# clovaai/assembled-cnn

Measured on AMD Instinct MI355X. Metric: images/sec Assemble-ResNet-50 224^2 bf16 train, higher is better.
Workload: dtype bf16; 1 GPU; Assemble-ResNet-50 (BigLittle + SK + anti_alias sconv k=3 + resnet_d) bf16 train; per_gpu_batch=256, global_batch=256, image=224x224x3, num_classes=1001, parallelism=dp1

## Files before the change

### assembled_cnn_amd/build.py

```python
from __future__ import annotations

import concurrent.futures
import os
import shutil
import subprocess
import sys

HERE = os.path.dirname(os.path.abspath(__file__))
CSRC = os.path.join(HERE, 'csrc')
OBJ_DIR = os.path.join(CSRC, '_obj')
LIB_PATH = os.path.join(HERE, 'libasm_hip.so')
SOURCES = ['conv_igemm.hip', 'conv_igemm8.hip', 'conv_gemm1.hip', 'conv_dgrad_s2.hip', 'conv_wgrad.hip', 'bn.hip', 'pool.hip', 'sk_se.hip', 'sk_fused.hip', 'dense_small.hip', 'misc.hip', 'extra.hip', 'input.hip', 'autoaugment.hip', 'jpeg.hip', 'plan.hip', 'tape.hip', 'collective.hip', 'retrieval.hip']
HEADERS = [os.path.join(CSRC, 'common.h'), os.path.join(CSRC, 'igemm_common.h'), os.path.join(CSRC, 'jpeg_entropy.h'), os.path.join(CSRC, 'jpeg_parallel.h'), os.path.join(HERE, '..', 'include', 'asm_hip.h'),
           os.path.join(HERE, '..', 'include', 'asm_hip_debug.h')]
ARCH = 'gfx950'
CFLAGS = ['--offload-arch=' + ARCH, '-O3', '-std=c++17', '-fPIC', '-fno-gpu-rdc', '-Wall', '-Wno-unused-function']


def _hipcc() -> str:
  exe = shutil.which('hipcc') or '/opt/rocm/bin/hipcc'
  if not os.path.exists(exe):
    raise RuntimeError('hipcc not found: cannot build libasm_hip.so')
  return exe


def _stale(target: str, deps) -> bool:
  if not os.path.exists(target):
    return True
  t = os.path.getmtime(target)
  return any(os.path.getmtime(d) > t for d in deps)


def _compile(src: str) -> str:
  obj = os.path.join(OBJ_DIR, os.path.splitext(src)[0] + '.o')
  path = os.path.join(CSRC, src)
  if _stale(obj, [path] + HEADERS):
    cmd = [_hipcc()] + CFLAGS + ['-c', path, '-o', obj]
    r = subprocess.run(cmd, capture_output=True, text=True)
    if r.returncode != 0:
      raise RuntimeError('hipcc failed for %s:\n%s\n%s' % (src, r.stdout, r.stderr))
  return obj


def build(force: bool = False, verbose: bool = False) -> str:
  os.makedirs(OBJ_DIR, exist_ok=True)
  if force:
    for f in os.listdir(OBJ_DIR):
      os.remove(os.path.join(OBJ_DIR, f))
  with concurrent.futures.ThreadPoolExecutor(max_workers=min(8, len(SOURCES))) as ex:
    objs = list(ex.map(_compile, SOURCES))
  if force or _stale(LIB_PATH, objs):
    tmp = LIB_PATH + '.tmp.%d' % os.getpid()
    cmd = [_hipcc(), '--offload-arch=' + ARCH, '-shared', '-fPIC', '-o', tmp] + objs
    r = subprocess.run(cmd, capture_output=True, text=True)
    if r.returncode != 0:
      if os.path.exists(tmp):
        os.remove(tmp)
      raise RuntimeError('link failed:\n%s\n%s' % (r.stdout, r.stderr))
    os.replace(tmp, LIB_PATH)
  if verbose:
    print('built', LIB_PATH)
  return LIB_PATH


if __name__ == '__main__':
  build(force='--force' in sys.argv, verbose=True)
```

### assembled_cnn_amd/csrc/bn.hip

```cpp
#include "common.h"
#include <stdlib.h>


#define BN_LD_RED(p) (*(p))
#define BN_ST_BWD(v, p) __builtin_nontemporal_store(v, p)
#define BN_ST_FWD(v, p) __builtin_nontemporal_store(v, p)

namespace {

struct RowTiling {
  int vcols;
  int vcb;
  int rpb;
  int rows_per_block;
  int blocks;
  int slices;
  int vc_slice;
};

RowTiling make_tiling(int M, int C) {
  RowTiling t;
  t.vcols = C / 8;
  const int want = 8;
  int sl = t.vcols / 8;
// ... 312 lines not shown
      const unsigned m = fd_div((unsigned)i, fd_vcols);
      body(i, m, (int)((unsigned)i - m * (unsigned)vcols), k);
    }
  } else {
    for (size_t i = i0; i < nvec; i += stride) {
      const unsigned m = fd_div((unsigned)i, fd_vcols);
      const int vc = (int)((unsigned)i - m * (unsigned)vcols);
      load_coef(vc);
      body(i, m, vc, k);
    }
  }
}

template <int RES, bool RELU>
__global__ __launch_bounds__(256) void bn_apply_kernel(size_t nvec, int C, FastDiv fd_vcols,
                                                       const bf16_t* __restrict__ x, bf16_t* __restrict__ y,
                                                       const float* __restrict__ scale,
                                                       const float* __restrict__ shift,
                                                       const bf16_t* __restrict__ res, FastDiv fd_w, FastDiv fd_h,
                                                       int H, int W, uint8_t* __restrict__ mask) {
  const float* const coef[2] = {scale, shift};
  for_each_vec<2>(nvec, C, fd_vcols, coef, [&](size_t i, unsigned m, int vc, const float (&k)[2][8]) {
    float f[8];
    unpack8(__builtin_nontemporal_load(reinterpret_cast<const u32x4*>(x + i * 8)), f);
#pragma unroll
    for (int e = 0; e < 8; ++e) f[e] = f[e] * k[0][e] + k[1][e];
    if (RES != 0) {
      size_t ri;
      if (RES == 1) {
        ri = i * 8;
      } else {
        const unsigned nh = fd_div(m, fd_w);
        const unsigned w = m - nh * (unsigned)W;
        const unsigned n = fd_div(nh, fd_h);
        const unsigned h = nh - n * (unsigned)H;
        ri = ((((size_t)n * (H >> 1) + (h >> 1)) * (W >> 1) + (w >> 1)) * (C >> 3) + vc) * 8;
      }
      float r[8];
      unpack8(*reinterpret_cast<const u32x4*>(res + ri), r);
#pragma unroll
      for (int e = 0; e < 8; ++e) f[e] += r[e];
    }
    if (RELU) {
      if (mask) mask[i] = (uint8_t)relu_mask8(f);
#pragma unroll
      for (int e = 0; e < 8; ++e) f[e] = fmaxf(f[e], 0.f);
    }
    BN_ST_FWD(pack8(f), reinterpret_cast<u32x4*>(y + i * 8));
  });
}

__device__ __forceinline__ float bwd_dx(float A, float dz, float B, float x, float C) {
  return __builtin_fmaf(A, dz, B * x) + C;
}

template <int RELU, bool WRITE_DZ>
__global__ __launch_bounds__(256) void bn_bwd_apply_kernel(size_t nvec, int C, FastDiv fd_vcols,
                                                           const bf16_t* __restrict__ dy, const bf16_t* __restrict__ x,
                                                           const bf16_t* __restrict__ yout, const float* __restrict__ cA,
                                                           const float* __restrict__ cB,
                                                           const float* __restrict__ cC, bf16_t* __restrict__ dx,
                                                           bf16_t* __restrict__ dz) {
  const float* const coef[3] = {cA, cB, cC};
  for_each_vec<3>(nvec, C, fd_vcols, coef, [&](size_t i, unsigned, int, const float (&k)[3][8]) {
    float g[8], fx[8];
    unpack8(__builtin_nontemporal_load(reinterpret_cast<const u32x4*>(dy + i * 8)), g);
    unpack8(__builtin_nontemporal_load(reinterpret_cast<const u32x4*>(x + i * 8)), fx);
    if (RELU == 1) {
      float fy[8];
      unpack8(*reinterpret_cast<const u32x4*>(yout + i * 8), fy);
#pragma unroll
      for (int e = 0; e < 8; ++e) g[e] = fy[e] > 0.f ? g[e] : 0.f;
    } else if (RELU == 2) {
      mask8(g, reinterpret_cast<const uint8_t*>(yout)[i]);
    }
    if (WRITE_DZ) *reinterpret_cast<u32x4*>(dz + i * 8) = pack8(g);
    float o[8];
#pragma unroll
    for (int e = 0; e < 8; ++e) o[e] = bwd_dx(k[0][e], g[e], k[1][e], fx[e], k[2][e]);
    BN_ST_BWD(pack8(o), reinterpret_cast<u32x4*>(dx + i * 8));
  });
}

struct BwdRow2 {
  const bf16_t* __restrict__ dy;
  const bf16_t* __restrict__ xa;
  const bf16_t* __restrict__ xb;
  const uint8_t* __restrict__ mask;
  const float* __restrict__ mean_a;
  const float* __restrict__ invstd_a;
  const float* __restrict__ mean_b;
  const float* __restrict__ invstd_b;
  float* __restrict__ pa;
  float* __restrict__ pb;
  int C;
  float ma[8], ia[8], mb[8], ib[8];
  struct Loaded { u32x4 vg, va, vb; unsigned mk; };
  __device__ __forceinline__ void setup(int vc) {
#pragma unroll
    for (int e = 0; e < 8; ++e) {
      ma[e] = mean_a[vc * 8 + e];
      ia[e] = invstd_a[vc * 8 + e];
      mb[e] = mean_b[vc * 8 + e];
      ib[e] = invstd_b[vc * 8 + e];
    }
  }
  __device__ __forceinline__ void load(Loaded& ld, size_t off, size_t mi) const {
    ld.vg = BN_LD_RED(reinterpret_cast<const u32x4*>(dy + off));
    ld.va = BN_LD_RED(reinterpret_cast<const u32x4*>(xa + off));
    ld.vb = BN_LD_RED(reinterpret_cast<const u32x4*>(xb + off));
    ld.mk = mask[mi];
  }
  __device__ __forceinline__ void accum(const Loaded& ld, float (&acc)[3][8]) const {
    float g[8], fa[8], fb[8];
    unpack8(ld.vg, g);
    unpack8(ld.va, fa);
    unpack8(ld.vb, fb);
    mask8(g, ld.mk);
#pragma unroll
    for (int e = 0; e < 8; ++e) {
      acc[0][e] += g[e];
      acc[1][e] += g[e] * ((fa[e] - ma[e]) * ia[e]);
      acc[2][e] += g[e] * ((fb[e] - mb[e]) * ib[e]);
    }
  }
  __device__ __forceinline__ void store(int rblk, int which, int ch, float v) const {
    if (which == 0) {
      pa[((size_t)rblk * 2 + 0) * C + ch] = v;
      pb[((size_t)rblk * 2 + 0) * C + ch] = v;
    } else if (which == 1) {
      pa[((size_t)rblk * 2 + 1) * C + ch] = v;
    } else {
      pb[((size_t)rblk * 2 + 1) * C + ch] = v;
    }
  }
};

__global__ __launch_bounds__(256) void bn_bwd_reduce2_kernel(const bf16_t* __restrict__ dy, const bf16_t* __restrict__ xa,
                                                             const bf16_t* __restrict__ xb, const uint8_t* __restrict__ mask,
                                                             int M, int C, const float* __restrict__ mean_a,
                                                             const float* __restrict__ invstd_a, const float* __restrict__ mean_b,
                                                             const float* __restrict__ invstd_b, RowTiling t,
                                                             float* __restrict__ pa, float* __restrict__ pb) {
  row_reduce<3>(BwdRow2{dy, xa, xb, mask, mean_a, invstd_a, mean_b, invstd_b, pa, pb, C}, M, C, t);
}

__global__ __launch_bounds__(256) void bn_bwd_apply2_kernel(size_t nvec, int C, FastDiv fd_vcols,
                                                            const bf16_t* __restrict__ dy, const bf16_t* __restrict__ xa,
                                                            const bf16_t* __restrict__ xb, const uint8_t* __restrict__ mask,
                                                            const float* __restrict__ co, bf16_t* __restrict__ dxa,
                                                            bf16_t* __restrict__ dxb) {
  const float* const coef[6] = {co, co + (size_t)C, co + (size_t)2 * C, co + (size_t)3 * C, co + (size_t)4 * C, co + (size_t)5 * C};
  for_each_vec<6>(nvec, C, fd_vcols, coef, [&](size_t i, unsigned, int, const float (&k)[6][8]) {
    float g[8], fa[8], fb[8];
    unpack8(__builtin_nontemporal_load(reinterpret_cast<const u32x4*>(dy + i * 8)), g);
    unpack8(__builtin_nontemporal_load(reinterpret_cast<const u32x4*>(xa + i * 8)), fa);
    unpack8(__builtin_nontemporal_load(reinterpret_cast<const u32x4*>(xb + i * 8)), fb);
    mask8(g, mask[i]);
    float oa[8], ob[8];
#pragma unroll
    for (int e = 0; e < 8; ++e) {
      oa[e] = bwd_dx(k[0][e], g[e], k[1][e], fa[e], k[2][e]);
      ob[e] = bwd_dx(k[3][e], g[e], k[4][e], fb[e], k[5][e]);
    }
    BN_ST_BWD(pack8(oa), reinterpret_cast<u32x4*>(dxa + i * 8));
    BN_ST_BWD(pack8(ob), reinterpret_cast<u32x4*>(dxb + i * 8));
// ... 267 lines not shown
  ASM_LAUNCH(bn_finalize_kernel, dim3(cdiv(C, 16)), dim3(16 * FL), 0, (hipStream_t)stream, stats_partial,
                     blocks, M, C, gamma, beta, eps, momentum, moving_mean, moving_var, mean, invstd, scale, shift);
  ASM_CHECK_LAUNCH("bn_finalize");
  return ASM_OK;
}

extern "C" int asm_bn_infer_coeffs(int C, const float* gamma, const float* beta, const float* moving_mean,
                                   const float* moving_var, float eps, float* scale, float* shift, void* stream) {
  ASM_REQUIRE(C > 0 && gamma && beta && moving_mean && moving_var && scale && shift, "bn_infer_coeffs: bad arguments");
  ASM_LAUNCH(bn_infer_coeffs_kernel, dim3(cdiv(C, 256)), dim3(256), 0, (hipStream_t)stream, C, gamma, beta,
                     moving_mean, moving_var, eps, scale, shift);
  ASM_CHECK_LAUNCH("bn_infer_coeffs");
  return ASM_OK;
}

extern "C" int asm_bn_apply(const void* x, void* y, int M, int C, const float* scale, const float* shift,
                            const void* residual, int res_mode, int relu, int H, int W, uint8_t* relu_mask_out,
                            void* stream) {
  ASM_REQUIRE(x && y && scale && shift && M > 0 && C > 0 && C % 8 == 0, "bn_apply: bad arguments");
  ASM_REQUIRE(res_mode >= 0 && res_mode <= 2 && (res_mode == 0 || residual), "bn_apply: bad residual mode");
  ASM_REQUIRE((size_t)M * (C / 8) < 0x7fffffffull, "bn_apply: tensor too large");
  if (res_mode == 2)
    ASM_REQUIRE(H > 0 && W > 0 && H % 2 == 0 && W % 2 == 0 && M % (H * W) == 0, "bn_apply: bad upsample geometry");
  const FastDiv fw = make_fastdiv((unsigned)(W > 0 ? W : 1)), fh = make_fastdiv((unsigned)(H > 0 ? H : 1));
  static constexpr decltype(&bn_apply_kernel<0, false>) kernels[3][2] = {
      {bn_apply_kernel<0, false>, bn_apply_kernel<0, true>},
      {bn_apply_kernel<1, false>, bn_apply_kernel<1, true>},
      {bn_apply_kernel<2, false>, bn_apply_kernel<2, true>}};
  launch_vecs(kernels[res_mode][relu != 0], stream, M, C, (const bf16_t*)x, (bf16_t*)y, scale, shift, (const bf16_t*)residual,
              fw, fh, H, W, relu_mask_out);
  ASM_CHECK_LAUNCH("bn_apply");
  return ASM_OK;
}

extern "C" int asm_bn_bwd_reduce(const void* dy, const void* x, const void* yout, int relu, int M, int C,
                                 const float* mean, const float* invstd, float* partial, void* stream) {
  ASM_REQUIRE(dy && x && mean && invstd && partial && M > 0 && C > 0 && C % 8 == 0, "bn_bwd_reduce: bad arguments");
  ASM_REQUIRE(relu >= 0 && relu <= 2 && (!relu || yout), "bn_bwd_reduce: relu mask needs the forward output / bitmask");
  RowTiling t = make_tiling(M, C);
  ASM_LAUNCH(bn_bwd_reduce_kernel, dim3(t.blocks * t.slices), dim3(256), 0, (hipStream_t)stream, (const bf16_t*)dy,
                     (const bf16_t*)x, (const bf16_t*)yout, relu, M, C, mean, invstd, t, partial);
  ASM_CHECK_LAUNCH("bn_bwd_reduce");
  return ASM_OK;
}

extern "C" int asm_bn_bwd_finalize(const float* partial, int blocks, int M, int C, const float* gamma,
                                   const float* mean, const float* invstd, float* dgamma, float* dbeta,
                                   float* coefA, float* coefB, float* coefC, void* stream) {
  ASM_REQUIRE(partial && gamma && mean && invstd && dgamma && dbeta && coefA && coefB && coefC && blocks > 0,
              "bn_bwd_finalize: bad arguments");
  ASM_LAUNCH(bn_bwd_finalize_kernel, dim3(cdiv(C, 16)), dim3(16 * FL), 0, (hipStream_t)stream, partial, blocks,
                     M, C, gamma, mean, invstd, dgamma, dbeta, coefA, coefB, coefC, 0);
  ASM_CHECK_LAUNCH("bn_bwd_finalize");
  return ASM_OK;
}

extern "C" int asm_bn_bwd_finalize_raw(const float* partial, int blocks, int M, int C, const float* gamma,
                                       const float* mean, const float* invstd, float* dgamma, float* dbeta,
                                       float* coefA, float* coefB, float* coefC, void* stream) {
  ASM_REQUIRE(partial && gamma && mean && invstd && dgamma && dbeta && coefA && coefB && coefC && blocks > 0,
              "bn_bwd_finalize_raw: bad arguments");
  ASM_LAUNCH(bn_bwd_finalize_kernel, dim3(cdiv(C, 16)), dim3(16 * FL), 0, (hipStream_t)stream, partial, blocks,
                     M, C, gamma, mean, invstd, dgamma, dbeta, coefA, coefB, coefC, 1);
  ASM_CHECK_LAUNCH("bn_bwd_finalize_raw");
  return ASM_OK;
}

extern "C" int asm_bn_bwd_apply(const void* dy, const void* x, const void* yout, int relu, int M, int C,
                                const float* coefA, const float* coefB, const float* coefC, void* dx,
                                void* dz_out, void* stream) {
  ASM_REQUIRE(dy && x && dx && coefA && coefB && coefC && M > 0 && C > 0 && C % 8 == 0, "bn_bwd_apply: bad arguments");
  ASM_REQUIRE(relu >= 0 && relu <= 2 && (!relu || yout), "bn_bwd_apply: relu mask needs the forward output / bitmask");
  ASM_REQUIRE((size_t)M * (C / 8) < 0x7fffffffull, "bn_bwd_apply: tensor too large");
  static constexpr decltype(&bn_bwd_apply_kernel<0, false>) kernels[3][2] = {
      {bn_bwd_apply_kernel<0, false>, bn_bwd_apply_kernel<0, true>},
      {bn_bwd_apply_kernel<1, false>, bn_bwd_apply_kernel<1, true>},
      {bn_bwd_apply_kernel<2, false>, bn_bwd_apply_kernel<2, true>}};
  launch_vecs(kernels[relu][dz_out != nullptr], stream, M, C, (const bf16_t*)dy, (const bf16_t*)x, (const bf16_t*)yout, coefA,
              coefB, coefC, (bf16_t*)dx, (bf16_t*)dz_out);
  ASM_CHECK_LAUNCH("bn_bwd_apply");
  return ASM_OK;
}

extern "C" int asm_bn_small_max_rows(void) { return SMALL_BN_MAX_ROWS; }

extern "C" int asm_bn_small_fwd(const void* x, void* y, int M, int C, const float* gamma, const float* beta, float eps,
                                float momentum, float* moving_mean, float* moving_var, float* mean, float* invstd,
                                int relu, uint8_t* relu_mask_out, void* stream) {
  ASM_REQUIRE(x && y && gamma && beta && mean && invstd && M > 0 && M <= SMALL_BN_MAX_ROWS && C > 0 && C % 8 == 0,
              "bn_small_fwd: bad arguments (M=%d C=%d)", M, C);
  ASM_REQUIRE((moving_mean == nullptr) == (moving_var == nullptr), "bn_small_fwd: moving stats must both be given");
  const dim3 grid(cdiv(C, 64)), block(256);
  if (relu)
    ASM_LAUNCH(bn_small_fwd_kernel<true>, grid, block, 0, (hipStream_t)stream, (const bf16_t*)x, (bf16_t*)y, M, C,
                       gamma, beta, eps, momentum, moving_mean, moving_var, mean, invstd, relu_mask_out);
  else
    ASM_LAUNCH(bn_small_fwd_kernel<false>, grid, block, 0, (hipStream_t)stream, (const bf16_t*)x, (bf16_t*)y, M, C,
                       gamma, beta, eps, momentum, moving_mean, moving_var, mean, invstd, nullptr);
  ASM_CHECK_LAUNCH("bn_small_fwd");
  return ASM_OK;
}

extern "C" int asm_bn_small_bwd(const void* dy, const void* x, const uint8_t* relu_mask, int M, int C,
                                const float* gamma, const float* mean, const float* invstd, float* dgamma,
                                float* dbeta, void* dx, void* stream) {
  ASM_REQUIRE(dy && x && gamma && mean && invstd && dgamma && dbeta && dx && M > 0 && M <= SMALL_BN_MAX_ROWS && C > 0 &&
                  C % 8 == 0, "bn_small_bwd: bad arguments (M=%d C=%d)", M, C);
  const dim3 grid(cdiv(C, 64)), block(256);
  if (relu_mask)
    ASM_LAUNCH(bn_small_bwd_kernel<2>, grid, block, 0, (hipStream_t)stream, (const bf16_t*)dy, (const bf16_t*)x,
                       relu_mask, M, C, gamma, mean, invstd, dgamma, dbeta, (bf16_t*)dx);
  else
    ASM_LAUNCH(bn_small_bwd_kernel<0>, grid, block, 0, (hipStream_t)stream, (const bf16_t*)dy, (const bf16_t*)x,
                       nullptr, M, C, gamma, mean, invstd, dgamma, dbeta, (bf16_t*)dx);
  ASM_CHECK_LAUNCH("bn_small_bwd");
  return ASM_OK;
}

extern "C" int asm_bn_bwd_reduce2(const void* dy, const void* xa, const void* xb, const uint8_t* relu_mask, int M, int C,
                                  const float* mean_a, const float* invstd_a, const float* mean_b, const float* invstd_b,
                                  float* partial_a, float* partial_b, void* stream) {
  ASM_REQUIRE(dy && xa && xb && relu_mask && mean_a && invstd_a && mean_b && invstd_b && partial_a && partial_b && M > 0 &&
                  C > 0 && C % 8 == 0, "bn_bwd_reduce2: bad arguments");
  RowTiling t = make_tiling(M, C);
  ASM_LAUNCH(bn_bwd_reduce2_kernel, dim3(t.blocks * t.slices), dim3(256), 0, (hipStream_t)stream, (const bf16_t*)dy,
                     (const bf16_t*)xa, (const bf16_t*)xb, relu_mask, M, C, mean_a, invstd_a, mean_b, invstd_b, t, partial_a,
                     partial_b);
  ASM_CHECK_LAUNCH("bn_bwd_reduce2");
  return ASM_OK;
}

extern "C" int asm_bn_bwd_apply2(const void* dy, const void* xa, const void* xb, const uint8_t* relu_mask, int M, int C,
                                 const float* coef6, void* dxa, void* dxb, void* stream) {
  ASM_REQUIRE(dy && xa && xb && relu_mask && coef6 && dxa && dxb && M > 0 && C > 0 && C % 8 == 0, "bn_bwd_apply2: bad arguments");
  ASM_REQUIRE((size_t)M * (C / 8) < 0x7fffffffull, "bn_bwd_apply2: tensor too large");
  launch_vecs(bn_bwd_apply2_kernel, stream, M, C, (const bf16_t*)dy, (const bf16_t*)xa, (const bf16_t*)xb, relu_mask, coef6,
              (bf16_t*)dxa, (bf16_t*)dxb);
  ASM_CHECK_LAUNCH("bn_bwd_apply2");
  return ASM_OK;
}

extern "C" int asm_bn_apply2(const void* xa, const void* xb, void* y, int M, int C, const float* scale_a,
                             const float* shift_a, const float* scale_b, const float* shift_b, int relu,
                             uint8_t* relu_mask_out, void* stream) {
  ASM_REQUIRE(xa && xb && y && scale_a && shift_a && scale_b && shift_b && M > 0 && C > 0 && C % 8 == 0, "bn_apply2: bad arguments");
  ASM_REQUIRE((size_t)M * (C / 8) < 0x7fffffffull, "bn_apply2: tensor too large");
  launch_vecs(relu ? bn_apply2_kernel<true> : bn_apply2_kernel<false>, stream, M, C, (const bf16_t*)xa, (const bf16_t*)xb,
              (bf16_t*)y, scale_a, shift_a, scale_b, shift_b, relu ? relu_mask_out : nullptr);
  ASM_CHECK_LAUNCH("bn_apply2");
  return ASM_OK;
}
```

### assembled_cnn_amd/csrc/pool.hip

```cpp
#include "common.h"

namespace {

inline unsigned grid_for(size_t nvec) {
  size_t b = cdivz(nvec, 256);
  return (unsigned)(b ? b : 1);
}

__device__ __forceinline__ u32x4 ldv(const bf16_t* p, size_t elem_off) {
  return *reinterpret_cast<const u32x4*>(p + elem_off);
}

struct Pix {
  int n, h, w, vc;
};
__device__ __forceinline__ Pix decode(size_t i64, int H, int W, int vcols) {
  const unsigned i = (unsigned)i64;
  Pix p;
  unsigned m = i / (unsigned)vcols;
  p.vc = (int)(i - m * (unsigned)vcols);
  unsigned q = m / (unsigned)W;
  p.w = (int)(m - q * (unsigned)W);
  const unsigned n = q / (unsigned)H;
  p.h = (int)(q - n * (unsigned)H);
  p.n = (int)n;
  return p;
}

__global__ __launch_bounds__(256) void maxpool_fwd_kernel(const bf16_t* __restrict__ x, bf16_t* __restrict__ y,
                                                          uint8_t* __restrict__ amax, int N, int H, int W, int C,
                                                          int Ho, int Wo, int pad_h, int pad_w) {
  const int vcols = C >> 3;
  const size_t nvec = (size_t)N * Ho * Wo * vcols;
  const size_t i = (size_t)blockIdx.x * 256 + threadIdx.x;
  if (i >= nvec) return;
  const Pix p = decode(i, Ho, Wo, vcols);
  float best[8];
  int bidx[8];
#pragma unroll
  for (int e = 0; e < 8; ++e) {
    best[e] = -INFINITY;
    bidx[e] = 0;
  }
  for (int r = 0; r < 3; ++r) {
    const int ih = p.h * 2 + r - pad_h;
    if ((unsigned)ih >= (unsigned)H) continue;
    for (int s = 0; s < 3; ++s) {
      const int iw = p.w * 2 + s - pad_w;
      if ((unsigned)iw >= (unsigned)W) continue;
      float f[8];
      unpack8(ldv(x, (((size_t)p.n * H + ih) * W + iw) * C + p.vc * 8), f);
#pragma unroll
      for (int e = 0; e < 8; ++e)
        if (f[e] > best[e]) {
          best[e] = f[e];
          bidx[e] = r * 3 + s;
        }
    }
  }
  *reinterpret_cast<u32x4*>(y + i * 8) = pack8(best);
  if (amax) {
    unsigned lo = 0, hi = 0;
#pragma unroll
    for (int e = 0; e < 4; ++e) {
      lo |= (unsigned)bidx[e] << (8 * e);
      hi |= (unsigned)bidx[e + 4] << (8 * e);
    }
    u32x2 v = {lo, hi};
    *reinterpret_cast<u32x2*>(amax + i * 8) = v;
  }
}

__global__ __launch_bounds__(256) void maxpool_bwd_kernel(const bf16_t* __restrict__ dy,
                                                          const uint8_t* __restrict__ amax, bf16_t* __restrict__ dx,
                                                          int N, int H, int W, int C, int Ho, int Wo, int pad_h,
                                                          int pad_w) {
  const int vcols = C >> 3;
  const size_t nvec = (size_t)N * H * W * vcols;
  const size_t i = (size_t)blockIdx.x * 256 + threadIdx.x;
  if (i >= nvec) return;
  const Pix p = decode(i, H, W, vcols);
  float acc[8];
#pragma unroll
// ... 48 lines not shown
      ++cnt;
    }
  }
  const float inv = 1.0f / (float)(count_valid ? cnt : k * k);
#pragma unroll
  for (int e = 0; e < 8; ++e) acc[e] *= inv;
  *reinterpret_cast<u32x4*>(y + i * 8) = pack8(acc);
}

__device__ __forceinline__ int valid_taps(int o, int stride, int pad, int k, int L) {
  int c = 0;
  for (int r = 0; r < k; ++r) c += ((unsigned)(o * stride + r - pad) < (unsigned)L);
  return c;
}

__global__ __launch_bounds__(256) void avgpool_bwd_kernel(const bf16_t* __restrict__ dy, bf16_t* dx,
                                                          int N, int H, int W, int C, int k, int stride, int pad,
                                                          int Ho, int Wo, int count_valid, const bf16_t* addend) {
  const int vcols = C >> 3;
  const size_t nvec = (size_t)N * H * W * vcols;
  const size_t i = (size_t)blockIdx.x * 256 + threadIdx.x;
  if (i >= nvec) return;
  const Pix p = decode(i, H, W, vcols);
  const int sh = stride >> 1, msk = stride - 1;
  const float inv_full = 1.0f / (float)(k * k);
  float acc[8];
#pragma unroll
  for (int e = 0; e < 8; ++e) acc[e] = 0.f;
  const bf16_t* src = dy + (size_t)p.n * Ho * Wo * C + p.vc * 8;
  for (int r = 0; r < k; ++r) {
    const int th = p.h + pad - r;
    const int ho = th >> sh;
    if (th < 0 || (th & msk) || ho >= Ho) continue;
    for (int s = 0; s < k; ++s) {
      const int tw = p.w + pad - s;
      const int wo = tw >> sh;
      if (tw < 0 || (tw & msk) || wo >= Wo) continue;
      float g[8];
      unpack8(ldv(src, (size_t)(ho * Wo + wo) * C), g);
      const float inv = count_valid
                            ? 1.0f / (float)(valid_taps(ho, stride, pad, k, H) * valid_taps(wo, stride, pad, k, W))
                            : inv_full;
#pragma unroll
      for (int e = 0; e < 8; ++e) acc[e] += g[e] * inv;
    }
  }
  if (addend) {
    float f[8];
    unpack8(ldv(addend, i * 8), f);
#pragma unroll
    for (int e = 0; e < 8; ++e) acc[e] += f[e];
  }
  *reinterpret_cast<u32x4*>(dx + i * 8) = pack8(acc);
}

template <bool MASKED>
__global__ __launch_bounds__(256) void upsample_bwd_kernel(const bf16_t* __restrict__ dy, const uint8_t* __restrict__ mask,
                                                           bf16_t* __restrict__ dx, int N, int Hs, int Ws, int C) {
  const int vcols = C >> 3;
  const size_t nvec = (size_t)N * Hs * Ws * vcols;
  const size_t i = (size_t)blockIdx.x * 256 + threadIdx.x;
  if (i >= nvec) return;
  const Pix p = decode(i, Hs, Ws, vcols);
  float acc[8];
#pragma unroll
  for (int e = 0; e < 8; ++e) acc[e] = 0.f;
  const int H = Hs * 2, W = Ws * 2;
#pragma unroll
  for (int r = 0; r < 2; ++r)
#pragma unroll
    for (int s = 0; s < 2; ++s) {
      float g[8];
      const size_t pix = ((size_t)p.n * H + p.h * 2 + r) * W + p.w * 2 + s;
      unpack8(ldv(dy, pix * C + p.vc * 8), g);
      if (MASKED) {
        const unsigned mk = mask[pix * vcols + p.vc];
#pragma unroll
        for (int e = 0; e < 8; ++e) g[e] = ((mk >> e) & 1u) ? g[e] : 0.f;
      }
#pragma unroll
      for (int e = 0; e < 8; ++e) acc[e] += g[e];
    }
  *reinterpret_cast<u32x4*>(dx + i * 8) = pack8(acc);
}

struct BlurCoef {
  float a[8];
};
inline BlurCoef blur_coef(int k) {
  static const int tri[8][7] = {{0}, {1}, {1, 1}, {1, 2, 1}, {1, 3, 3, 1}, {1, 4, 6, 4, 1}, {1, 5, 10, 10, 5, 1},
                                {1, 6, 15, 20, 15, 6, 1}};
  BlurCoef c;
  int sum = 0;
  for (int i = 0; i < k; ++i) sum += tri[k][i];
  for (int i = 0; i < 8; ++i) c.a[i] = i < k ? (float)tri[k][i] / (float)sum : 0.f;
  return c;
}
__device__ __forceinline__ int reflect(int i, int L) {
  if (i < 0) i = -i;
  if (i >= L) i = 2 * (L - 1) - i;
  return i;
}

__global__ __launch_bounds__(256) void blur_fwd_kernel(const bf16_t* __restrict__ x, bf16_t* __restrict__ y, int N,
                                                       int H, int W, int C, int k, int stride, int Ho, int Wo,
                                                       BlurCoef cf) {
  const int vcols = C >> 3;
  const size_t nvec = (size_t)N * Ho * Wo * vcols;
  const size_t i = (size_t)blockIdx.x * 256 + threadIdx.x;
  if (i >= nvec) return;
  const Pix p = decode(i, Ho, Wo, vcols);
  const int pad = (k - 1) / 2;
  float acc[8];
#pragma unroll
  for (int e = 0; e < 8; ++e) acc[e] = 0.f;
  for (int r = 0; r < k; ++r) {
    const int ih = reflect(p.h * stride + r - pad, H);
    for (int s = 0; s < k; ++s) {
      const int iw = reflect(p.w * stride + s - pad, W);
      float f[8];
      unpack8(ldv(x, (((size_t)p.n * H + ih) * W + iw) * C + p.vc * 8), f);
      const float wgt = cf.a[r] * cf.a[s];
#pragma unroll
      for (int e = 0; e < 8; ++e) acc[e] += f[e] * wgt;
    }
  }
  *reinterpret_cast<u32x4*>(y + i * 8) = pack8(acc);
}

__device__ __forceinline__ int padded_sources(int h, int L, int pad, int* hp) {
  int n = 0;
  hp[n++] = h + pad;
  if (h >= 1 && h <= pad) hp[n++] = pad - h;
  if (h <= L - 2 && h >= L - 1 - pad) hp[n++] = pad + 2 * (L - 1) - h;
  return n;
}

__global__ __launch_bounds__(256) void blur_bwd_kernel(const bf16_t* __restrict__ dy, bf16_t* __restrict__ dx, int N,
                                                       int H, int W, int C, int k, int stride, int Ho, int Wo,
                                                       BlurCoef cf) {
  const int vcols = C >> 3;
  const size_t nvec = (size_t)N * H * W * vcols;
  const size_t i = (size_t)blockIdx.x * 256 + threadIdx.x;
  if (i >= nvec) return;
  const Pix p = decode(i, H, W, vcols);
  const int pad = (k - 1) / 2;
  float acc[8];
#pragma unroll
  for (int e = 0; e < 8; ++e) acc[e] = 0.f;
  int hps[3], wps[3];
  const int nh = padded_sources(p.h, H, pad, hps);
  const int nw = padded_sources(p.w, W, pad, wps);
  for (int a = 0; a < nh; ++a)
    for (int r = 0; r < k; ++r) {
      const int th = hps[a] - r;
      if (th < 0 || th % stride) continue;
      const int ho = th / stride;
      if (ho >= Ho) continue;
      for (int b = 0; b < nw; ++b)
        for (int s = 0; s < k; ++s) {
          const int tw = wps[b] - s;
          if (tw < 0 || tw % stride) continue;
          const int wo = tw / stride;
          if (wo >= Wo) continue;
          float g[8];
          unpack8(ldv(dy, (((size_t)p.n * Ho + ho) * Wo + wo) * C + p.vc * 8), g);
          const float wgt = cf.a[r] * cf.a[s];
#pragma unroll
          for (int e = 0; e < 8; ++e) acc[e] += g[e] * wgt;
        }
    }
  *reinterpret_cast<u32x4*>(dx + i * 8) = pack8(acc);
}

__global__ __launch_bounds__(256) void blur3s2_bwd_kernel(const bf16_t* __restrict__ dy, bf16_t* __restrict__ dx, int N,
                                                          int Hh, int Wh, int C, float a0, float a1, float a2) {
  const int vcols = C >> 3;
  const size_t nq = (size_t)N * Hh * Wh * vcols;
  const size_t q = (size_t)blockIdx.x * 256 + threadIdx.x;
  if (q >= nq) return;
  const Pix p = decode(q, Hh, Wh, vcols);
  const bool hv = p.h + 1 < Hh, wv = p.w + 1 < Wh;
  float g[2][2][8];
#pragma unroll
  for (int a = 0; a < 2; ++a)
#pragma unroll
    for (int b = 0; b < 2; ++b) {
      const bool ok = (a == 0 || hv) && (b == 0 || wv);
      const size_t off = (((size_t)p.n * Hh + p.h + (ok ? a : 0)) * Wh + p.w + (ok ? b : 0)) * C + p.vc * 8;
      unpack8(ldv(dy, off), g[a][b]);
    }
  const int src_odd[3] = {1, 0, 0};
  const float wgt_odd[3] = {a0, a2, a0};
  const bool okh[3] = {hv, true, p.h == 0}, okw[3] = {wv, true, p.w == 0};
  const int W2 = 2 * Wh;
#pragma unroll
  for (int u = 0; u < 2; ++u)
#pragma unroll
    for (int v = 0; v < 2; ++v) {
      float acc[8];
#pragma unroll
      for (int e = 0; e < 8; ++e) acc[e] = 0.f;
#pragma unroll
      for (int th = 0; th < (u ? 3 : 1); ++th) {
        const int sh = u ? src_odd[th] : 0;
        const float wh = u ? wgt_odd[th] : a1;
        if (u && !okh[th]) continue;
#pragma unroll
        for (int tw = 0; tw < (v ? 3 : 1); ++tw) {
          const int sw = v ? src_odd[tw] : 0;
          const float ww = v ? wgt_odd[tw] : a1;
          if (v && !okw[tw]) continue;
          const float wgt = wh * ww;
#pragma unroll
          for (int e = 0; e < 8; ++e) acc[e] += g[sh][sw][e] * wgt;
        }
      }
      const size_t off = (((size_t)p.n * 2 * Hh + 2 * p.h + u) * W2 + 2 * p.w + v) * C + p.vc * 8;
      *reinterpret_cast<u32x4*>(dx + off) = pack8(acc);
    }
}

template <bool TWO_BRANCH, int NT>
__global__ __launch_bounds__(NT) void gap_fwd_kernel(const bf16_t* __restrict__ x, bf16_t* __restrict__ y, int HW,
                                                     int Cin, int Cout, int vcb) {
  __shared__ float red[NT][9];
  const int vcols = Cout >> 3;
  const int vcl = threadIdx.x % vcb;
  const int rl = threadIdx.x / vcb;
  const int nrl = NT / vcb;
  const int vc = blockIdx.x * vcb + vcl;
  const int n = blockIdx.y;
  float acc[8];
#pragma unroll
  for (int e = 0; e < 8; ++e) acc[e] = 0.f;
  if (vc < vcols && rl < nrl) {
    constexpr int U = 4;
    const bf16_t* base = x + (size_t)n * HW * Cin + vc * 8;
    int r = rl;
    for (; r + (U - 1) * nrl < HW; r += U * nrl) {
      u32x4 v[U], w[U];
#pragma unroll
      for (int u = 0; u < U; ++u) {
        const size_t off = (size_t)(r + u * nrl) * Cin;
        v[u] = ldv(base, off);
        if (TWO_BRANCH) w[u] = ldv(base, off + Cout);
      }
#pragma unroll
      for (int u = 0; u < U; ++u) {
        float f[8];
        unpack8(v[u], f);
#pragma unroll
        for (int e = 0; e < 8; ++e) acc[e] += f[e];
        if (TWO_BRANCH) {
          unpack8(w[u], f);
#pragma unroll
          for (int e = 0; e < 8; ++e) acc[e] += f[e];
        }
      }
    }
    for (; r < HW; r += nrl) {
      const size_t off = (size_t)r * Cin;
      float f[8];
      unpack8(ldv(base, off), f);
#pragma unroll
      for (int e = 0; e < 8; ++e) acc[e] += f[e];
      if (TWO_BRANCH) {
        unpack8(ldv(base, off + Cout), f);
#pragma unroll
        for (int e = 0; e < 8; ++e) acc[e] += f[e];
      }
    }
  }
#pragma unroll
  for (int e = 0; e < 8; ++e) red[threadIdx.x][e] = acc[e];
  __syncthreads();
  if (rl == 0 && vc < vcols) {
    float o[8];
    const float inv = 1.0f / (float)HW;
#pragma unroll
    for (int e = 0; e < 8; ++e) {
      float t = 0.f;
      for (int r = 0; r < nrl; ++r) t += red[r * vcb + vcl][e];
      o[e] = t * inv;
    }
    *reinterpret_cast<u32x4*>(y + (size_t)n * Cout + vc * 8) = pack8(o);
  }
}

__global__ __launch_bounds__(256) void gap_bwd_kernel(const bf16_t* __restrict__ dy, bf16_t* __restrict__ dx, int N,
                                                      int HW, int C) {
  const int vcols = C >> 3;
  const size_t nvec = (size_t)N * HW * vcols;
  const size_t i = (size_t)blockIdx.x * 256 + threadIdx.x;
  if (i >= nvec) return;
  const unsigned iu = (unsigned)i;
  const int vc = (int)(iu % (unsigned)vcols);
  const int n = (int)(iu / ((unsigned)HW * (unsigned)vcols));
  float g[8];
  unpack8(ldv(dy, (size_t)n * C + vc * 8), g);
// ... 163 lines not shown
```

### assembled_cnn_amd/csrc/sk_fused.hip

```cpp
#include "common.h"

namespace {

__device__ __forceinline__ u32x4 ldv(const bf16_t* p, size_t off) { return *reinterpret_cast<const u32x4*>(p + off); }
__device__ __forceinline__ float rbf(float x) { return bf2f(f2bf(x)); }

struct Coef8 {
  float sc[8], sh[8];
};
__device__ __forceinline__ void load_coef(const float* __restrict__ scale, const float* __restrict__ shift, int ch0, Coef8& k) {
  const f32x4 s0 = *reinterpret_cast<const f32x4*>(scale + ch0), s1 = *reinterpret_cast<const f32x4*>(scale + ch0 + 4);
  const f32x4 h0 = *reinterpret_cast<const f32x4*>(shift + ch0), h1 = *reinterpret_cast<const f32x4*>(shift + ch0 + 4);
#pragma unroll
  for (int e = 0; e < 4; ++e) {
    k.sc[e] = s0[e]; k.sc[e + 4] = s1[e];
    k.sh[e] = h0[e]; k.sh[e + 4] = h1[e];
  }
}
__device__ __forceinline__ void bnrelu8(const u32x4& vy, const Coef8& k, float* f) {
  float y[8];
  unpack8(vy, y);
#pragma unroll
  for (int e = 0; e < 8; ++e) f[e] = rbf(fmaxf(y[e] * k.sc[e] + k.sh[e], 0.f));
}

__device__ __forceinline__ void gate8(const float* __restrict__ att, int n, int F, int c0, float* a0) {
#pragma unroll
  for (int e = 0; e < 8; ++e) {
    const float l0 = att[(size_t)n * 2 * F + c0 + e];
    const float l1 = att[(size_t)n * 2 * F + F + c0 + e];
    a0[e] = 1.0f / (1.0f + __expf(l1 - l0));
  }
}

template <int NT>
__device__ __forceinline__ void lane_sum8(float (*red)[9], const float* v, float* out, int vcb, int vcl, int nrl, bool leader) {
  if ((vcb & (vcb - 1)) == 0 && vcb <= 64) {
    float w[8];
#pragma unroll
    for (int e = 0; e < 8; ++e) w[e] = v[e];
    for (int off = vcb; off < 64; off <<= 1) {
#pragma unroll
      for (int e = 0; e < 8; ++e) w[e] += __shfl_xor(w[e], off, 64);
    }
    const int wave = threadIdx.x >> 6, lane = threadIdx.x & 63;
    __syncthreads();
    if (lane < vcb) {
#pragma unroll
      for (int e = 0; e < 8; ++e) red[wave * vcb + lane][e] = w[e];
    }
    __syncthreads();
    if (leader) {
#pragma unroll
      for (int e = 0; e < 8; ++e) {
        float t = 0.f;
#pragma unroll
        for (int r = 0; r < NT / 64; ++r) t += red[r * vcb + vcl][e];
        out[e] = t;
      }
    }
    return;
  }
  __syncthreads();
#pragma unroll
  for (int e = 0; e < 8; ++e) red[threadIdx.x][e] = v[e];
  __syncthreads();
  if (leader) {
#pragma unroll
    for (int e = 0; e < 8; ++e) {
      float t = 0.f;
      for (int r = 0; r < nrl; ++r) t += red[r * vcb + vcl][e];
      out[e] = t;
    }
  }
}

__device__ __forceinline__ void bnrelu8m(const u32x4& vy, const Coef8& k, float* f, float* m, float* my) {
  float y[8];
  unpack8(vy, y);
#pragma unroll
  for (int e = 0; e < 8; ++e) {
    const float t = y[e] * k.sc[e] + k.sh[e];
    f[e] = rbf(fmaxf(t, 0.f));
    m[e] = t > 0.f ? 1.f : 0.f;
    my[e] = t > 0.f ? y[e] : 0.f;
  }
}

template <int NT, bool ST>
__global__ __launch_bounds__(NT, NT == 256 ? 4 : 1) void sk_gap_bn_kernel(const bf16_t* __restrict__ y, const float* __restrict__ scale,
                                                       const float* __restrict__ shift, bf16_t* __restrict__ s, int HW,
                                                       int F, int vcb, const float* __restrict__ mean,
                                                       const float* __restrict__ invstd, float* __restrict__ stats) {
  __shared__ float red[NT][9];
  const int vcols = F >> 3;
  const int vcl = threadIdx.x % vcb, rl = threadIdx.x / vcb, nrl = NT / vcb;
  const int vc = blockIdx.x * vcb + vcl;
  const int n = blockIdx.y;
  float acc[8], c0[8], x0[8], c1[8], x1[8];
#pragma unroll
  for (int e = 0; e < 8; ++e) acc[e] = c0[e] = x0[e] = c1[e] = x1[e] = 0.f;
  if (vc < vcols && rl < nrl) {
    Coef8 k0, k1;
    load_coef(scale, shift, vc * 8, k0);
    load_coef(scale, shift, F + vc * 8, k1);
    auto consume = [&](const u32x4& v, const u32x4& w) {
      if (ST) {
        float f[8], m[8], my[8];
        bnrelu8m(v, k0, f, m, my);
#pragma unroll
        for (int e = 0; e < 8; ++e) { acc[e] += f[e]; c0[e] += m[e]; x0[e] += my[e]; }
        bnrelu8m(w, k1, f, m, my);
#pragma unroll
        for (int e = 0; e < 8; ++e) { acc[e] += f[e]; c1[e] += m[e]; x1[e] += my[e]; }
      } else {
        float f0[8], f1[8];
        bnrelu8(v, k0, f0);
        bnrelu8(w, k1, f1);
#pragma unroll
        for (int e = 0; e < 8; ++e) acc[e] += f0[e] + f1[e];
      }
    };
    constexpr int U = ST ? 2 : 4;
    const bf16_t* base = y + (size_t)n * HW * 2 * F + vc * 8;
    int r = rl;
    for (; r + (U - 1) * nrl < HW; r += U * nrl) {
      u32x4 v[U], w[U];
#pragma unroll
      for (int u = 0; u < U; ++u) {
        const size_t off = (size_t)(r + u * nrl) * 2 * F;
        v[u] = ldv(base, off);
        w[u] = ldv(base, off + F);
      }
#pragma unroll
      for (int u = 0; u < U; ++u) consume(v[u], w[u]);
    }
    for (; r < HW; r += nrl) {
      const size_t off = (size_t)r * 2 * F;
      consume(ldv(base, off), ldv(base, off + F));
    }
  }
  const bool leader = rl == 0 && vc < vcols;
  float o[8];
  lane_sum8<NT>(red, acc, o, vcb, vcl, nrl, leader);
  if (leader) {
    const float inv = 1.0f / (float)HW;
#pragma unroll
    for (int e = 0; e < 8; ++e) o[e] *= inv;
    *reinterpret_cast<u32x4*>(s + (size_t)n * F + vc * 8) = pack8(o);
  }
  if (ST) {
    float* st = stats + (size_t)n * 4 * F;
    const float* src[4] = {c0, c1, x0, x1};
#pragma unroll
    for (int q = 0; q < 4; ++q) {
      lane_sum8<NT>(red, src[q], o, vcb, vcl, nrl, leader);
      if (leader) {
        float* dst = st + (q >> 1) * 2 * F + (q & 1) * F + vc * 8;
        *reinterpret_cast<f32x4*>(dst) = f32x4{o[0], o[1], o[2], o[3]};
        *reinterpret_cast<f32x4*>(dst + 4) = f32x4{o[4], o[5], o[6], o[7]};
      }
    }
  }
}

__global__ __launch_bounds__(256) void sk_select_bn_fwd_kernel(const bf16_t* __restrict__ y, const float* __restrict__ scale,
                                                               const float* __restrict__ shift,
                                                               const float* __restrict__ att, bf16_t* __restrict__ v,
                                                               int HW, int F, int rpb, int rows_per_chunk) {
  const int fv = F >> 3;
  const int vc = threadIdx.x % fv, rr = threadIdx.x / fv;
  if (rr >= rpb) return;
  const int n = blockIdx.y;
  Coef8 k0, k1;
  load_coef(scale, shift, vc * 8, k0);
  load_coef(scale, shift, F + vc * 8, k1);
  float a0[8];
  gate8(att, n, F, vc * 8, a0);
  const int r_begin = blockIdx.x * rows_per_chunk;
  const int r_end = min(HW, r_begin + rows_per_chunk);
  constexpr int U = 2;
  for (int r = r_begin + rr; r < r_end; r += U * rpb) {
    u32x4 y0[U], y1[U];
#pragma unroll
    for (int q = 0; q < U; ++q) {
      const int rq = r + q * rpb;
      const size_t m = (size_t)n * HW + (rq < r_end ? rq : r);
      y0[q] = ldv(y, m * 2 * F + vc * 8);
      y1[q] = ldv(y, m * 2 * F + F + vc * 8);
    }
#pragma unroll
    for (int q = 0; q < U; ++q) {
      const int rq = r + q * rpb;
      if (rq >= r_end) break;
      float f0[8], f1[8], o[8];
      bnrelu8(y0[q], k0, f0);
      bnrelu8(y1[q], k1, f1);
#pragma unroll
      for (int e = 0; e < 8; ++e) o[e] = a0[e] * f0[e] + (1.0f - a0[e]) * f1[e];
      *reinterpret_cast<u32x4*>(v + ((size_t)n * HW + rq) * F + vc * 8) = pack8(o);
    }
  }
}

template <int NT, bool ST>
__global__ __launch_bounds__(NT, NT == 256 ? 4 : 1) void sk_bn_bwd_att_kernel(const bf16_t* __restrict__ y, const float* __restrict__ scale,
                                                           const float* __restrict__ shift, const bf16_t* __restrict__ dv,
                                                           const float* __restrict__ att, bf16_t* __restrict__ datt,
                                                           int HW, int F, int vcb, const float* __restrict__ mean,
                                                           const float* __restrict__ invstd, float* __restrict__ stats) {
  __shared__ float red[NT][9];
  const int vcols = F >> 3;
  const int vcl = threadIdx.x % vcb, rl = threadIdx.x / vcb, nrl = NT / vcb;
  const int vc = blockIdx.x * vcb + vcl;
  const int n = blockIdx.y;
  float acc[8], g0[8], x0[8], g1[8], x1[8];
#pragma unroll
  for (int e = 0; e < 8; ++e) acc[e] = g0[e] = x0[e] = g1[e] = x1[e] = 0.f;
  if (vc < vcols && rl < nrl) {
    Coef8 k0, k1;
    load_coef(scale, shift, vc * 8, k0);
    load_coef(scale, shift, F + vc * 8, k1);
    auto consume = [&](const u32x4& v0, const u32x4& v1, const u32x4& vg) {
      float g[8];
      unpack8(vg, g);
      if (ST) {
        float f[8], m[8], my[8];
        bnrelu8m(v0, k0, f, m, my);
#pragma unroll
        for (int e = 0; e < 8; ++e) { acc[e] += f[e] * g[e]; g0[e] += m[e] * g[e]; x0[e] += my[e] * g[e]; }
        bnrelu8m(v1, k1, f, m, my);
#pragma unroll
        for (int e = 0; e < 8; ++e) { acc[e] -= f[e] * g[e]; g1[e] += m[e] * g[e]; x1[e] += my[e] * g[e]; }
      } else {
        float f0[8], f1[8];
        bnrelu8(v0, k0, f0);
        bnrelu8(v1, k1, f1);
#pragma unroll
        for (int e = 0; e < 8; ++e) acc[e] += (f0[e] - f1[e]) * g[e];
      }
    };
    constexpr int U = ST ? 1 : 2;
    int r = rl;
    for (; r + (U - 1) * nrl < HW; r += U * nrl) {
      u32x4 v0[U], v1[U], vg[U];
#pragma unroll
      for (int u = 0; u < U; ++u) {
        const size_t m = (size_t)n * HW + r + u * nrl;
        v0[u] = ldv(y, m * 2 * F + vc * 8);
        v1[u] = ldv(y, m * 2 * F + F + vc * 8);
        vg[u] = ldv(dv, m * F + vc * 8);
      }
#pragma unroll
      for (int u = 0; u < U; ++u) consume(v0[u], v1[u], vg[u]);
    }
    for (; r < HW; r += nrl) {
      const size_t m = (size_t)n * HW + r;
      consume(ldv(y, m * 2 * F + vc * 8), ldv(y, m * 2 * F + F + vc * 8), ldv(dv, m * F + vc * 8));
    }
  }
  const bool leader = rl == 0 && vc < vcols;
  float o[8];
  lane_sum8<NT>(red, acc, o, vcb, vcl, nrl, leader);
  if (leader) {
    float a0[8], d0[8], d1[8];
    gate8(att, n, F, vc * 8, a0);
#pragma unroll
    for (int e = 0; e < 8; ++e) {
      d0[e] = a0[e] * (1.0f - a0[e]) * o[e];
      d1[e] = -d0[e];
    }
    *reinterpret_cast<u32x4*>(datt + (size_t)n * 2 * F + vc * 8) = pack8(d0);
    *reinterpret_cast<u32x4*>(datt + (size_t)n * 2 * F + F + vc * 8) = pack8(d1);
  }
  if (ST) {
    float* st = stats + (size_t)n * 4 * F;
    const float* src[4] = {g0, g1, x0, x1};
#pragma unroll
    for (int q = 0; q < 4; ++q) {
      lane_sum8<NT>(red, src[q], o, vcb, vcl, nrl, leader);
      if (leader) {
        float* dst = st + (q >> 1) * 2 * F + (q & 1) * F + vc * 8;
        *reinterpret_cast<f32x4*>(dst) = f32x4{o[0], o[1], o[2], o[3]};
        *reinterpret_cast<f32x4*>(dst + 4) = f32x4{o[4], o[5], o[6], o[7]};
      }
    }
  }
}

struct SkBnGeom {
  int HW, F, vcols, rpb, rows_per_chunk, chunks;
};

__device__ __forceinline__ void sk_thread_setup(const SkBnGeom& g, int n, int vc, const float* __restrict__ att,
                                                const bf16_t* __restrict__ ds, float* ab, float* u) {
  const int fv = g.F >> 3;
  const int b = vc >= fv ? 1 : 0;
  const int c0 = (vc - b * fv) * 8;
  float a0[8], q[8];
  gate8(att, n, g.F, c0, a0);
  unpack8(ldv(ds, (size_t)n * g.F + c0), q);
  const float inv = 1.0f / (float)g.HW;
#pragma unroll
  for (int e = 0; e < 8; ++e) {
    ab[e] = b ? (1.0f - a0[e]) : a0[e];
    u[e] = q[e] * inv;
  }
}

__global__ __launch_bounds__(256) void sk_bn_bwd_reduce_kernel(const bf16_t* __restrict__ dv, const float* __restrict__ att,
                                                               const bf16_t* __restrict__ ds, const bf16_t* __restrict__ y,
                                                               const float* __restrict__ scale,
                                                               const float* __restrict__ shift,
                                                               const float* __restrict__ mean,
                                                               const float* __restrict__ invstd, SkBnGeom g,
                                                               float* __restrict__ partial) {
  __shared__ float red[4096];
  const int tid = threadIdx.x;
  const int vc = tid % g.vcols;
  const int rr = tid / g.vcols;
  const bool active = rr < g.rpb;
  const int n = blockIdx.y;
  const int C2 = 2 * g.F;
  const int fv = g.F >> 3;
  const int cv = vc >= fv ? vc - fv : vc;
  float acc[2][8];
#pragma unroll
  for (int e = 0; e < 8; ++e) acc[0][e] = acc[1][e] = 0.f;
  if (active) {
    Coef8 k;
    load_coef(scale, shift, vc * 8, k);
    float mu[8], is[8], ab[8], u[8];
#pragma unroll
    for (int e = 0; e < 8; ++e) {
      mu[e] = mean[vc * 8 + e];
      is[e] = invstd[vc * 8 + e];
    }
    sk_thread_setup(g, n, vc, att, ds, ab, u);
    const int r_begin = blockIdx.x * g.rows_per_chunk;
    const int r_end = min(g.HW, r_begin + g.rows_per_chunk);
    constexpr int U = 2;
    for (int r = r_begin + rr; r < r_end; r += U * g.rpb) {
      u32x4 vy[U], vg[U];
#pragma unroll
      for (int q = 0; q < U; ++q) {
        const int rq = r + q * g.rpb;
        const size_t m = (size_t)n * g.HW + (rq < r_end ? rq : r);
        vy[q] = *reinterpret_cast<const u32x4*>(y + m * C2 + vc * 8);
        vg[q] = ldv(dv, m * g.F + cv * 8);
      }
#pragma unroll
      for (int q = 0; q < U; ++q) {
        if (r + q * g.rpb >= r_end) break;
        float fy[8], fg[8];
        unpack8(vy[q], fy);
        unpack8(vg[q], fg);
#pragma unroll
        for (int e = 0; e < 8; ++e) {
          const float dz = (fy[e] * k.sc[e] + k.sh[e] > 0.f) ? (ab[e] * fg[e] + u[e]) : 0.f;
          acc[0][e] += dz;
          acc[1][e] += dz * ((fy[e] - mu[e]) * is[e]);
        }
      }
    }
  }
  const size_t prow = (size_t)n * g.chunks + blockIdx.x;
  row_lanes_sum<2>(red, acc, active, vc, rr, g.rpb, g.vcols * 8,
                   [&](int which, int col, float v) { partial[(prow * 2 + which) * C2 + col] = v; });
}

__global__ __launch_bounds__(1024) void sk_bn_bwd_finalize_kernel(const float* __restrict__ gst, const float* __restrict__ mst,
                                                                  const float* __restrict__ att, const bf16_t* __restrict__ ds,
                                                                  int N, int HW, int F, const float* __restrict__ gamma,
                                                                  const float* __restrict__ mean,
                                                                  const float* __restrict__ invstd, float* dgamma,
                                                                  float* dbeta, float* coefA, float* coefB, float* coefC) {
  __shared__ double red[2][64][16];
  const int cx = threadIdx.x & 15, ry = threadIdx.x >> 4;
  const int C2 = 2 * F;
  const int ch = blockIdx.x * 16 + cx;
  double s0 = 0.0, s1 = 0.0;
  if (ch < C2) {
    const int b = ch >= F ? 1 : 0, c = ch - b * F;
    const float inv = 1.0f / (float)HW;
    for (int n = ry; n < N; n += 64) {
      const float l0 = att[(size_t)n * C2 + c], l1 = att[(size_t)n * C2 + F + c];
      const float a0 = 1.0f / (1.0f + __expf(l1 - l0));
      const float ab = b ? (1.0f - a0) : a0;
      const float u = bf2f(ds[(size_t)n * F + c]) * inv;
      const float* gs = gst + (size_t)n * 2 * C2;
      const float* ms = mst + (size_t)n * 2 * C2;
      const double g0 = gs[ch], m0 = ms[ch];
      const double w = (double)ab * g0 + (double)u * m0;
      s0 += w;
      s1 += (double)ab * (double)gs[C2 + ch] + (double)u * (double)ms[C2 + ch];
      s1 -= (double)mean[ch] * w;
    }
    s1 *= (double)invstd[ch];
  }
  fl_stage(red, ry, cx, s0, s1);
  if (ry == 0 && ch < C2) {
    double db, dg;
    fl_sum2(red, cx, db, dg);
    dbeta[ch] = (float)db;
    dgamma[ch] = (float)dg;
    bn_bwd_coefs(gamma[ch], invstd[ch], mean[ch], db, dg, (double)N * (double)HW, coefA[ch], coefB[ch], coefC[ch]);
  }
}

__global__ __launch_bounds__(256) void sk_bn_bwd_apply_kernel(const bf16_t* __restrict__ dv, const float* __restrict__ att,
                                                              const bf16_t* __restrict__ ds, const bf16_t* __restrict__ y,
                                                              const float* __restrict__ scale,
                                                              const float* __restrict__ shift, const float* __restrict__ cA,
                                                              const float* __restrict__ cB, const float* __restrict__ cC,
                                                              bf16_t* __restrict__ dy, SkBnGeom g) {
  const int tid = threadIdx.x;
  const int vc = tid % g.vcols;
  const int rr = tid / g.vcols;
  if (rr >= g.rpb) return;
  const int n = blockIdx.y;
  const int C2 = 2 * g.F;
  const int fv = g.F >> 3;
  const int cv = vc >= fv ? vc - fv : vc;
  Coef8 k;
  load_coef(scale, shift, vc * 8, k);
  float ab[8], u[8], kA[8], kB[8], kC[8];
#pragma unroll
  for (int e = 0; e < 8; ++e) {
    kA[e] = cA[vc * 8 + e];
    kB[e] = cB[vc * 8 + e];
    kC[e] = cC[vc * 8 + e];
  }
  sk_thread_setup(g, n, vc, att, ds, ab, u);
  const int r_begin = blockIdx.x * g.rows_per_chunk;
  const int r_end = min(g.HW, r_begin + g.rows_per_chunk);
  constexpr int U = 2;
  for (int r = r_begin + rr; r < r_end; r += U * g.rpb) {
    u32x4 vy[U], vg[U];
#pragma unroll
    for (int q = 0; q < U; ++q) {
      const int rq = r + q * g.rpb;
      const size_t m = (size_t)n * g.HW + (rq < r_end ? rq : r);
      vy[q] = __builtin_nontemporal_load(reinterpret_cast<const u32x4*>(y + m * C2 + vc * 8));
      vg[q] = ldv(dv, m * g.F + cv * 8);
    }
#pragma unroll
    for (int q = 0; q < U; ++q) {
      const int rq = r + q * g.rpb;
      if (rq >= r_end) break;
      float fy[8], fg[8], o[8];
      unpack8(vy[q], fy);
      unpack8(vg[q], fg);
#pragma unroll
      for (int e = 0; e < 8; ++e) {
        const float dz = (fy[e] * k.sc[e] + k.sh[e] > 0.f) ? (ab[e] * fg[e] + u[e]) : 0.f;
        o[e] = kA[e] * dz + kB[e] * fy[e] + kC[e];
      }
      const size_t m = (size_t)n * g.HW + rq;
      __builtin_nontemporal_store(pack8(o), reinterpret_cast<u32x4*>(dy + m * C2 + vc * 8));
    }
  }
}

int image_pass_vcb(int N, int F) {
  const int vcols = F / 8;
  int groups = cdiv(1024, N > 0 ? N : 1);
  if (groups < 1) groups = 1;
  int vcb = 32;
  while (vcb > 8 && cdiv(vcols, vcb) < groups) vcb >>= 1;
  return vcols < vcb ? vcols : vcb;
}

SkBnGeom make_geom(int N, int HW, int F) {
  SkBnGeom g;
  g.HW = HW;
  g.F = F;
  g.vcols = 2 * F / 8;
  g.rpb = 256 / g.vcols;
  int chunks = 1024 / N;
  if (chunks < 1) chunks = 1;
  int rows = cdiv(HW, chunks);
  rows = cdiv(rows, g.rpb) * g.rpb;
  if (rows < g.rpb * 4) rows = g.rpb * 4;
  g.rows_per_chunk = rows;
  g.chunks = cdiv(HW, rows);
  return g;
}

}

#define SKF_OK(name)                                                                                        \
  ASM_REQUIRE(N > 0 && HW > 0 && F > 0 && F % 8 == 0 && 2 * F / 8 <= 256, name ": bad shape (N=%d HW=%d F=%d)", N, HW, F); \
  ASM_REQUIRE((size_t)N * HW * (2 * F / 8) < 0x7fffffffull, name ": tensor too large for 32-bit indexing")

static int sk_gap_bn_impl(const void* y, const float* scale, const float* shift, void* s, int N, int HW, int F,
                          const float* mean, const float* invstd, float* stats, void* stream) {
  SKF_OK("sk_gap_bn");
  ASM_REQUIRE(y && scale && shift && s, "sk_gap_bn: null pointer");
  const int vcb = image_pass_vcb(N, F);
  const dim3 grid(cdiv(F / 8, vcb), N);
  hipStream_t st = (hipStream_t)stream;
#define LAUNCH_GAP(NT, ST)                                                                                       \
  ASM_LAUNCH((sk_gap_bn_kernel<NT, ST>), grid, dim3(NT), 0, st, (const bf16_t*)y, scale, shift, (bf16_t*)s, HW, F, \
                     vcb, mean, invstd, stats)
  if (stats) { if (HW >= 512) LAUNCH_GAP(1024, true); else LAUNCH_GAP(256, true); }
  else { if (HW >= 512) LAUNCH_GAP(1024, false); else LAUNCH_GAP(256, false); }
#undef LAUNCH_GAP
  ASM_CHECK_LAUNCH("sk_gap_bn");
  return ASM_OK;
}

extern "C" int asm_sk_gap_bn(const void* y, const float* scale, const float* shift, void* s, int N, int HW, int F,
                             void* stream) {
  return sk_gap_bn_impl(y, scale, shift, s, N, HW, F, nullptr, nullptr, nullptr, stream);
}

extern "C" int asm_sk_gap_bn_stats(const void* y, const float* scale, const float* shift, const float* mean,
                                   const float* invstd, void* s, float* mask_stats, int N, int HW, int F, void* stream) {
  ASM_REQUIRE(mean && invstd && mask_stats, "sk_gap_bn_stats: null pointer");
  return sk_gap_bn_impl(y, scale, shift, s, N, HW, F, mean, invstd, mask_stats, stream);
}

extern "C" int asm_sk_select_bn_fwd(const void* y, const float* scale, const float* shift, const float* att, void* v,
                                    int N, int HW, int F, void* stream) {
  SKF_OK("sk_select_bn_fwd");
  ASM_REQUIRE(y && scale && shift && att && v, "sk_select_bn_fwd: null pointer");
  const int fv = F / 8, rpb = 256 / fv;
  int chunks = 2048 / N;
  if (chunks < 1) chunks = 1;
  int rows = cdiv(HW, chunks);
  rows = cdiv(rows, rpb) * rpb;
  if (rows < rpb * 4) rows = rpb * 4;
  ASM_LAUNCH(sk_select_bn_fwd_kernel, dim3(cdiv(HW, rows), N), dim3(256), 0, (hipStream_t)stream,
                     (const bf16_t*)y, scale, shift, att, (bf16_t*)v, HW, F, rpb, rows);
  ASM_CHECK_LAUNCH("sk_select_bn_fwd");
  return ASM_OK;
}

static int sk_att_impl(const void* y, const float* scale, const float* shift, const void* dv, const float* att, void* datt,
                       int N, int HW, int F, const float* mean, const float* invstd, float* stats, void* stream) {
  SKF_OK("sk_select_bn_bwd_att");
  ASM_REQUIRE(y && scale && shift && dv && att && datt, "sk_select_bn_bwd_att: null pointer");
  const int vcb = image_pass_vcb(N, F);
  const dim3 grid(cdiv(F / 8, vcb), N);
  hipStream_t st = (hipStream_t)stream;
#define LAUNCH_ATT(NT, ST)                                                                                          \
  ASM_LAUNCH((sk_bn_bwd_att_kernel<NT, ST>), grid, dim3(NT), 0, st, (const bf16_t*)y, scale, shift, (const bf16_t*)dv, \
                     att, (bf16_t*)datt, HW, F, vcb, mean, invstd, stats)
  if (stats) { if (HW >= 512) LAUNCH_ATT(1024, true); else LAUNCH_ATT(256, true); }
  else { if (HW >= 512) LAUNCH_ATT(1024, false); else LAUNCH_ATT(256, false); }
#undef LAUNCH_ATT
  ASM_CHECK_LAUNCH("sk_select_bn_bwd_att");
  return ASM_OK;
}

extern "C" int asm_sk_select_bn_bwd_att(const void* y, const float* scale, const float* shift, const void* dv,
                                        const float* att, void* datt, int N, int HW, int F, void* stream) {
  return sk_att_impl(y, scale, shift, dv, att, datt, N, HW, F, nullptr, nullptr, nullptr, stream);
}

extern "C" int asm_sk_select_bn_bwd_att_stats(const void* y, const float* scale, const float* shift, const float* mean,
                                              const float* invstd, const void* dv, const float* att, void* datt,
                                              float* grad_stats, int N, int HW, int F, void* stream) {
  ASM_REQUIRE(mean && invstd && grad_stats, "sk_select_bn_bwd_att_stats: null pointer");
  return sk_att_impl(y, scale, shift, dv, att, datt, N, HW, F, mean, invstd, grad_stats, stream);
}

extern "C" int asm_sk_bn_bwd_finalize(const float* grad_stats, const float* mask_stats, const float* att, const void* ds,
                                      int N, int HW, int F, const float* gamma, const float* mean, const float* invstd,
                                      float* dgamma, float* dbeta, float* coefA, float* coefB, float* coefC, void* stream) {
  SKF_OK("sk_bn_bwd_finalize");
  ASM_REQUIRE(grad_stats && mask_stats && att && ds && gamma && mean && invstd && dgamma && dbeta && coefA && coefB && coefC,
              "sk_bn_bwd_finalize: null pointer");
  ASM_LAUNCH(sk_bn_bwd_finalize_kernel, dim3(cdiv(2 * F, 16)), dim3(1024), 0, (hipStream_t)stream, grad_stats,
                     mask_stats, att, (const bf16_t*)ds, N, HW, F, gamma, mean, invstd, dgamma, dbeta, coefA, coefB, coefC);
  ASM_CHECK_LAUNCH("sk_bn_bwd_finalize");
  return ASM_OK;
}

extern "C" int asm_sk_bn_bwd_blocks(int N, int HW, int F) {
  if (N <= 0 || HW <= 0 || F <= 0 || F % 8 || 2 * F / 8 > 256) return ASM_EINVAL;
  return N * make_geom(N, HW, F).chunks;
}

extern "C" int asm_sk_bn_bwd_reduce(const void* dv, const float* att, const void* ds, const void* y, const float* scale,
                                    const float* shift, const float* mean, const float* invstd, int N, int HW, int F,
                                    float* partial, void* stream) {
  SKF_OK("sk_bn_bwd_reduce");
  ASM_REQUIRE(dv && att && ds && y && scale && shift && mean && invstd && partial, "sk_bn_bwd_reduce: null pointer");
  const SkBnGeom g = make_geom(N, HW, F);
  ASM_LAUNCH(sk_bn_bwd_reduce_kernel, dim3(g.chunks, N), dim3(256), 0, (hipStream_t)stream, (const bf16_t*)dv, att,
                     (const bf16_t*)ds, (const bf16_t*)y, scale, shift, mean, invstd, g, partial);
  ASM_CHECK_LAUNCH("sk_bn_bwd_reduce");
  return ASM_OK;
}

extern "C" int asm_sk_bn_bwd_apply(const void* dv, const float* att, const void* ds, const void* y, const float* scale,
                                   const float* shift, const float* coefA, const float* coefB, const float* coefC,
                                   void* dy, int N, int HW, int F, void* stream) {
  SKF_OK("sk_bn_bwd_apply");
  ASM_REQUIRE(dv && att && ds && y && scale && shift && coefA && coefB && coefC && dy, "sk_bn_bwd_apply: null pointer");
  const SkBnGeom g = make_geom(N, HW, F);
  ASM_LAUNCH(sk_bn_bwd_apply_kernel, dim3(g.chunks, N), dim3(256), 0, (hipStream_t)stream,
                     (const bf16_t*)dv, att, (const bf16_t*)ds, (const bf16_t*)y, scale, shift, coefA, coefB, coefC,
                     (bf16_t*)dy, g);
  ASM_CHECK_LAUNCH("sk_bn_bwd_apply");
  return ASM_OK;
}
```

### assembled_cnn_amd/lib.py

```python
from __future__ import annotations

import ctypes as C
import os

HERE = os.path.dirname(os.path.abspath(__file__))
LIB_PATH = os.environ.get('ASM_HIP_LIB') or os.path.join(HERE, 'libasm_hip.so')

ASM_OK, ASM_EINVAL, ASM_ENOTSUP, ASM_EHIP = 0, -1, -2, -3
ABI_VERSION = 11


class AsmError(RuntimeError):
  pass


class ImageDesc(C.Structure):
  _fields_ = [('src_offset', C.c_int64), ('Hs', C.c_int32), ('Ws', C.c_int32),
              ('crop_y', C.c_int32), ('crop_x', C.c_int32), ('crop_h', C.c_int32), ('crop_w', C.c_int32),
              ('resize_h', C.c_int32), ('resize_w', C.c_int32), ('out_y', C.c_int32), ('out_x', C.c_int32),
              ('flip', C.c_int32), ('reserved', C.c_int32)]


assert C.sizeof(ImageDesc) == 56

# ... 66 lines not shown
  _fields_ = [('n_entries', C.c_int32), ('trainable_tensors', C.c_int32), ('trainable_elems', C.c_int64),
              ('forward_macs_per_image', C.c_int64), ('wgrad_workspace_bytes', C.c_int64)]


class Tuning(C.Structure):
  _fields_ = [(n, C.c_int32) for n in (
      'igemm_mode', 'igemm_tile', 'igemm_pfa', 'dgrad_parity', 'wgrad_halo', 'wgrad_big', 'wgrad_splits', 'bn_rows', 'igemm3',
      'gemm1', 'wgrad_ring', 'igemm8', 'dense_small')]


TUNING_ENV = {'ASM_IGEMM_MODE': 'igemm_mode', 'ASM_IGEMM_TILE': 'igemm_tile', 'ASM_IGEMM_PFA': 'igemm_pfa',
              'ASM_DGRAD_PARITY': 'dgrad_parity', 'ASM_WGRAD_HALO': 'wgrad_halo', 'ASM_WGRAD_BIG': 'wgrad_big',
              'ASM_WGRAD_SPLITS': 'wgrad_splits', 'ASM_BN_ROWS': 'bn_rows', 'ASM_IGEMM3': 'igemm3', 'ASM_GEMM1': 'gemm1',
              'ASM_WGRAD_RING': 'wgrad_ring', 'ASM_IGEMM8': 'igemm8', 'ASM_DENSE_SMALL': 'dense_small'}


def apply_env_tuning(lib) -> 'Tuning':
  t = Tuning()
  lib.asm_tuning_defaults(C.byref(t))
  for env, field in TUNING_ENV.items():
    v = os.environ.get(env)
    if v not in (None, ''):
      setattr(t, field, int(v))
  check_code = lib.asm_set_tuning(C.byref(t))
  if check_code != ASM_OK:
    raise ValueError('asm_set_tuning rejected the ASM_* overrides: %s' % (lib.asm_last_error() or b'').decode())
  return t


ASM_F32, ASM_BF16, ASM_F16 = 0, 1, 2
ASM_DGRAD_MASKED, ASM_DGRAD_POOLED, ASM_DGRAD_BNRED = 1, 2, 4
CONV_DGRAD_S2 = 5
CONV_DENSE = 6
ASM_AA_SCONV, ASM_AA_PROJ = 1, 2
POOL_TYPES = {'gap': 0, 'gem': 1, 'flatten': 2}
(PLAN_CONV, PLAN_BN, PLAN_DENSE, PLAN_MAXPOOL, PLAN_AVGPOOL, PLAN_BLURPOOL, PLAN_GAP, PLAN_GEM, PLAN_FLATTEN, PLAN_SK_GAP,
 PLAN_SK_SELECT, PLAN_SE_SCALE, PLAN_ADD) = range(13)

_P, _I, _F, _Z = C.c_void_p, C.c_int, C.c_float, C.c_size_t
_D = C.POINTER(ConvDesc)

SIGNATURES = {
    'asm_last_error': (C.c_char_p, []),
    'asm_abi_version': (_I, []),
    'asm_launch_count': (C.c_ulonglong, []),
    'asm_stream_join': (_I, [_P, _P]),
    'asm_memcpy_async': (_I, [_P, _P, _Z, _P]),
    'asm_allreduce_bucket': (_I, [_P, _Z, _I, _P, _P, _P]),
    'asm_tape_begin': (_I, []),
    'asm_tape_mark': (_I, []),
    'asm_tape_end': (_I, []),
    'asm_tape_info': (_I, [_I, C.POINTER(C.c_int64 * 6)]),
    'asm_tape_replay': (_I, [_I, _I]),
    'asm_tape_free': (_I, [_I]),
    'asm_tuning_defaults': (None, [C.POINTER(Tuning)]),
    'asm_set_tuning': (_I, [C.POINTER(Tuning)]),
    'asm_get_tuning': (None, [C.POINTER(Tuning)]),
    'asm_conv2d_fprop': (_I, [_D, _P, _P, _P, _P, _P]),
    'asm_conv2d_stats_blocks': (_I, [_D]),
    'asm_conv2d_dgrad': (_I, [_D, _P, _P, _P, _P, _P]),
    'asm_conv2d_dgrad_masked': (_I, [_D, _P, _P, _P, _P, _P, _P]),
    'asm_conv2d_dgrad_pooled': (_I, [_D, _P, _P, _P, _P, _P, _I, _I, _I, _I, _I, _I, _P, _P]),
    'asm_conv2d_dgrad_bnred_blocks': (_I, [_D]),
    'asm_conv2d_dgrad_bnred': (_I, [_D, _P, _P, _P, _P, _P, _P, _P, _P, _P]),
    'asm_conv2d_dgrad_kernel': (_I, [_D, _I]),
    'asm_conv2d_wgrad_workspace_bytes': (_Z, [_D]),
    'asm_conv2d_wgrad': (_I, [_D, _P, _P, _P, _P, _Z, _P]),
    'asm_filter_transpose': (_I, [_P, _P, _I, _I, _I, _I, _I, _P]),
    'asm_filter_transpose_batched': (_I, [_P, _P, _P, _I, C.c_longlong, _P]),
    'asm_filter_transpose_tiled': (_I, [_P, _P, _P, _I, _I, _P]),
    'asm_stem_pack_filter': (_I, [_P, _P, _I, _I, _P]),
    'asm_stem_unpack_grad': (_I, [_P, _P, _I, _I, _P]),
    'asm_stem_pad_input': (_I, [_P, _I, _P, _I, _I, _I, _P]),
    'asm_bn_stats_blocks': (_I, [_I, _I]),
    'asm_bn_stats': (_I, [_P, _I, _I, _P, _P]),
    'asm_bn_partials_compact': (_I, [_P, _I, _I, _P, _I, _P]),
    'asm_bn_finalize': (_I, [_P, _I, _I, _I, _P, _P, _F, _F, _P, _P, _P, _P, _P, _P, _P]),
    'asm_bn_infer_coeffs': (_I, [_I, _P, _P, _P, _P, _F, _P, _P, _P]),
    'asm_bn_apply': (_I, [_P, _P, _I, _I, _P, _P, _P, _I, _I, _I, _I, _P, _P]),
    'asm_bn_bwd_reduce': (_I, [_P, _P, _P, _I, _I, _I, _P, _P, _P, _P]),
    'asm_bn_bwd_finalize': (_I, [_P, _I, _I, _I, _P, _P, _P, _P, _P, _P, _P, _P, _P]),
    'asm_bn_bwd_finalize_raw': (_I, [_P, _I, _I, _I, _P, _P, _P, _P, _P, _P, _P, _P, _P]),
    'asm_bn_bwd_apply': (_I, [_P, _P, _P, _I, _I, _I, _P, _P, _P, _P, _P, _P]),
    'asm_maxpool3x3s2_fwd': (_I, [_P, _P, _P, _I, _I, _I, _I, _P]),
    'asm_maxpool3x3s2_bwd': (_I, [_P, _P, _P, _I, _I, _I, _I, _P]),
    'asm_avgpool_fwd': (_I, [_P, _P, _I, _I, _I, _I, _I, _I, _I, _I, _I, _I, _P]),
    'asm_avgpool_bwd': (_I, [_P, _P, _I, _I, _I, _I, _I, _I, _I, _I, _I, _I, _P, _P]),
    'asm_upsample2x_bwd': (_I, [_P, _P, _I, _I, _I, _I, _P]),
    'asm_upsample2x_bwd_masked': (_I, [_P, _P, _P, _I, _I, _I, _I, _P]),
    'asm_blurpool_fwd': (_I, [_P, _P, _I, _I, _I, _I, _I, _I, _P]),
    'asm_blurpool_bwd': (_I, [_P, _P, _I, _I, _I, _I, _I, _I, _P]),
    'asm_gap_fwd': (_I, [_P, _P, _I, _I, _I, _P]),
    'asm_gap_bwd': (_I, [_P, _P, _I, _I, _I, _P]),
    'asm_sk_gap': (_I, [_P, _P, _I, _I, _I, _P]),
    'asm_sk_select_fwd': (_I, [_P, _P, _P, _I, _I, _I, _P]),
    'asm_sk_select_bwd_att': (_I, [_P, _P, _P, _P, _I, _I, _I, _P]),
    'asm_sk_select_bwd_f': (_I, [_P, _P, _P, _P, _I, _I, _I, _P]),
    'asm_sk_gap_bn': (_I, [_P, _P, _P, _P, _I, _I, _I, _P]),
    'asm_sk_select_bn_fwd': (_I, [_P, _P, _P, _P, _P, _I, _I, _I, _P]),
    'asm_sk_select_bn_bwd_att': (_I, [_P, _P, _P, _P, _P, _P, _I, _I, _I, _P]),
    'asm_sk_bn_bwd_blocks': (_I, [_I, _I, _I]),
    'asm_sk_bn_bwd_reduce': (_I, [_P, _P, _P, _P, _P, _P, _P, _P, _I, _I, _I, _P, _P]),
    'asm_sk_bn_bwd_apply': (_I, [_P, _P, _P, _P, _P, _P, _P, _P, _P, _P, _I, _I, _I, _P]),
    'asm_sk_gap_bn_stats': (_I, [_P, _P, _P, _P, _P, _P, _P, _I, _I, _I, _P]),
    'asm_sk_select_bn_bwd_att_stats': (_I, [_P, _P, _P, _P, _P, _P, _P, _P, _P, _I, _I, _I, _P]),
    'asm_sk_bn_bwd_finalize': (_I, [_P, _P, _P, _P, _I, _I, _I, _P, _P, _P, _P, _P, _P, _P, _P, _P]),
    'asm_se_scale_fwd': (_I, [_P, _P, _P, _I, _I, _I, _P]),
    'asm_se_scale_bwd_e': (_I, [_P, _P, _P, _P, _I, _I, _I, _P]),
    'asm_se_scale_bwd_x': (_I, [_P, _P, _P, _P, _I, _I, _I, _P]),
    'asm_relu_fwd': (_I, [_P, _P, _Z, _P]),
    'asm_relu_bwd': (_I, [_P, _P, _P, _Z, _P]),
    'asm_add_bf16': (_I, [_P, _P, _P, _Z, _P]),
    'asm_mask_apply': (_I, [_P, _P, _P, _Z, _P]),
    'asm_bias_add_f32': (_I, [_P, _P, _I, _I, _I, _P]),
    'asm_bias_grad_bf16': (_I, [_P, _I, _I, _I, _P, _P]),
    'asm_cast_f32_to_bf16': (_I, [_P, _P, _Z, _P]),
    'asm_cast_bf16_to_f32': (_I, [_P, _P, _Z, _P]),
    'asm_softmax_ce': (_I, [_P, _I, _P, _P, _I, _I, _F, _F, _F, _P, _P, _I, _P]),
    'asm_onehot': (_I, [_P, _P, _I, _I, _P]),
    'asm_softmax_rows': (_I, [_P, _P, _I, _I, _F, _P]),
    'asm_mean_f32': (_I, [_P, _I, _P, _P]),
    'asm_mixup_meansub': (_I, [_P, _I, _I, _I, _I, _I, _P, _P, _P, _P]),
    'asm_mixup_labels': (_I, [_P, _I, _I, _I, _P, _P, _P, _P]),
    'asm_sigmoid_ce': (_I, [_P, _I, _P, _I, _I, _F, _P, _P, _P, _I, _P]),
    'asm_gem_fwd': (_I, [_P, _P, _P, _I, _I, _I, _F, _P]),
    'asm_gem_bwd': (_I, [_P, _P, _P, _P, _I, _I, _I, _F, _P]),
    'asm_dropblock_mask': (_I, [_P, _F, _I, _I, _I, _I, _P, _P, _P]),
    'asm_dropblock_mask_dev': (_I, [_P, _P, _I, _I, _I, _I, _P, _P, _P]),
    'asm_dropblock_apply': (_I, [_P, _P, _P, _P, _I, _P, _I, _I, _P]),
    'asm_eval_rows': (_I, [_P, _I, _P, _I, _I, _P, _P, _P, _P, _P]),
    'asm_eval_accumulate': (_I, [_P, _P, _P, _I, _P, _P]),
    'asm_embed_sqnorm': (_I, [_P, _I, _I, _I, _P, _P]),
    'asm_retrieval_topk_workspace_bytes': (_Z, [_I, _I, _I]),
    'asm_retrieval_topk': (_I, [_P, _I, _P, _I, _P, _P, _I, _I, _I, _I, _I, _I, _P, _P, _P, _Z, _P]),
    'asm_topk_merge': (_I, [_P, _P, _I, _I, _I, _P, _P, _P]),
    'asm_retrieval_topk_wide_workspace_bytes': (_Z, [_I, _I, _I]),
    'asm_retrieval_topk_wide': (_I, [_P, _I, _P, _I, _P, _P, _I, _I, _I, _I, _I, _I, _P, _P, _P, _Z, _P]),
    'asm_topk_merge_wide': (_I, [_P, _P, _I, _I, _I, _P, _P, _P]),
    'asm_recall_accumulate': (_I, [_P, _I, _I, _P, _P, _I, _I, _P, _I, _P, _P]),
    'asm_sgd_momentum': (_I, [_P, _P, _P, _P, _Z, _F, _F, _F, _F, _P]),
    'asm_conv2d_fprop_bn': (_I, [_P, _P, _P, _P, _P, _P, _P, _I, _P]),
    'asm_bn_apply2': (_I, [_P, _P, _P, _I, _I, _P, _P, _P, _P, _I, _P, _P]),
    'asm_bn_bwd_reduce2': (_I, [_P, _P, _P, _P, _I, _I, _P, _P, _P, _P, _P, _P, _P]),
    'asm_bn_bwd_apply2': (_I, [_P, _P, _P, _P, _I, _I, _P, _P, _P, _P]),
    'asm_bn_small_max_rows': (_I, []),
    'asm_bn_small_fwd': (_I, [_P, _P, _I, _I, _P, _P, _F, _F, _P, _P, _P, _P, _I, _P, _P]),
    'asm_bn_small_bwd': (_I, [_P, _P, _P, _I, _I, _P, _P, _P, _P, _P, _P, _P]),
    'asm_dense_small': (_I, [_P, _I, _P, _I, _I, _I, _I, _P, _I, _I, _P, _P]),
    'asm_dense_small_wgrad': (_I, [_P, _I, _P, _I, _I, _I, _I, _P, _I, _P]),
    'asm_resize_crop_flip': (_I, [_P, C.c_int64, _P, _I, _I, _I, _I, _P, _P]),
    'asm_autoaugment_workspace_bytes': (_I, [_I, _I, _I, C.POINTER(C.c_int64)]),
    'asm_autoaugment': (_I, [_P, _P, _I, _I, _I, _I, _P, _P, C.c_int64, _P]),
    'asm_jpeg_decode_workspace_bytes': (_I, [C.c_int64, C.POINTER(C.c_int64)]),
    'asm_jpeg_decode': (_I, [_P, C.c_int64, _P, _P, _P, _I, _I, C.c_int64, _I, _I, _P, C.c_int64, _P, _P, C.c_int64, _I, _P]),
    'asm_jpeg_decode_parallel_workspace_bytes': (_I, [C.c_int64, C.c_int64, C.POINTER(C.c_int64)]),
    'asm_jpeg_decode_parallel': (_I, [_P, C.c_int64, _P, _P, _P, _P, _I, _I, C.c_int64, _I, C.c_int64, _I, _I, _P, C.c_int64, _P,
                                      _P, _P, C.c_int64, _I, _P]),
    'asm_jpeg_decode_progressive': (_I, [_P, C.c_int64, _P, _P, _P, _P, _P, _I, _I, _I, _I, C.c_int64, _I, _I, _P, C.c_int64, _P,
                                         _P, C.c_int64, _I, _P]),
    'asm_model_plan': (_I, [C.POINTER(ModelCfg), _I, _I, _I, C.POINTER(PlanEntry), _I, C.POINTER(PlanSummary)]),
}

DEBUG_SIGNATURES = {
    'asm_conv2d_fprop_naive': (_I, [_D, _P, _P, _P, _P]),
    'asm_conv2d_dgrad_naive': (_I, [_D, _P, _P, _P, _P]),
    'asm_conv2d_wgrad_naive': (_I, [_D, _P, _P, _P, _P]),
    'asm_debug_tr_probe': (_I, [_P, _P]),
    'asm_conv2d_wgrad_plan': (_I, [_D, C.POINTER(C.c_int32 * 6)]),
    'asm_debug_last_conv_kernel': (_I, []),
    'asm_debug_retrieval_topk_wide_counted': (_I, [_P, _I, _P, _I, _P, _P, _I, _I, _I, _I, _I, _I, _P, _P, _P, _Z, _P, _P]),
}

_lib = None


def load(path: str = LIB_PATH) -> C.CDLL:
  global _lib
  if _lib is not None:
    return _lib
  if not os.path.exists(path):
    raise AsmError('%s not found -- build it with `python -m assembled_cnn_amd.build` '
                   '(there is no CPU fallback)' % path)
  import torch
  lib = C.CDLL(path)
  ver = getattr(lib, 'asm_abi_version', None)
  if ver is None:
    raise AsmError('%s does not export asm_abi_version: not a libasm_hip.so' % path)
  ver.restype, ver.argtypes = C.c_int, []
# ... 27 lines not shown
```

### assembled_cnn_amd/nn.py

```python
from __future__ import annotations

import math
from collections import OrderedDict
from typing import Callable, Dict, List, NamedTuple, Optional, Tuple

import numpy as np
import torch

from . import ops

BN_EPS = 1e-5


def dual_bn_on() -> bool:
  return ops.knob('ASM_BN_DUAL', '1') != '0'


def lazy_dz_on() -> bool:
  return ops.knob('ASM_LAZY_DZ', '1') != '0'


def defer_bn_on() -> bool:
  return ops.knob('ASM_BN_DEFER', '1') != '0'

# ... 172 lines not shown
    self.finalized = True
    self.refresh_shadows()

  def _view(self, arena, name):
    sp = self.specs[name]
    return arena[sp.offset:sp.offset + sp.numel].view(sp.shape)

  def w(self, name):
    return self._view(self.w32, name)

  def g(self, name):
    return self._view(self.g32, name)

  def m(self, name):
    return self._view(self.m32, name)

  def wb(self, name):
    return self._view(self.w16, name)

  def st(self, name):
    shape, _, off = self.state_specs[name]
    n = int(np.prod(shape))
    return self.state[off:off + n].view(shape)

  def refresh_shadows(self):
    ops.cast_f32_to_bf16(self.w32, self.w16)
    self.refresh_derived()

  def alloc_wt(self, name, K, RS, Cn, ldk) -> dict:
    ws = dict(name=name, K=K, RS=RS, C=Cn, ldk=ldk, offset=-1)
    self.wt_specs.append(ws)
    return ws

  def wt_view(self, ws) -> torch.Tensor:
    n = ws['C'] * ws['RS'] * ws['ldk']
    return self.wt16[ws['offset']:ws['offset'] + n]

  def refresh_derived(self):
    if self.wt_specs:
      ops.filter_transpose_tiled(self.w16, self.wt16, self._wt_table, len(self.wt_specs), self._wt_tiles)
    for fn in self.derived:
      fn()

  def num_params(self) -> int:
    return sum(sp.numel for sp in self.specs.values())


def variance_scaling_init(shape_krsc):
  k, r, s, c = shape_krsc
  std = math.sqrt(1.0 / (r * s * c)) / .87962566103423978

  def init(rng):
    out = rng.standard_normal(size=shape_krsc)
    bad = np.abs(out) > 2.0
    while bad.any():
      out[bad] = rng.standard_normal(size=int(bad.sum()))
      bad = np.abs(out) > 2.0
    return out * std
  return init


def glorot_uniform_init(shape_kc):
  k, c = shape_kc
  limit = math.sqrt(6.0 / (k + c))
  return lambda rng: rng.uniform(-limit, limit, size=shape_kc)


def const_init(shape, value):
  return lambda rng: np.full(shape, value, dtype=np.float32)


class SavedBN(NamedTuple):
  y: torch.Tensor
  M: int
  C: int
  gamma: torch.Tensor
  mean: torch.Tensor
  invstd: torch.Tensor
  bn: "BatchNorm"
  scale: torch.Tensor
  shift: torch.Tensor


class RedCtx(NamedTuple):
  y: torch.Tensor
  mask: Optional[torch.Tensor]


class Var(object):
  __slots__ = ('_data', 'shape', '_grad', 'grad_mask', 'grad_owned', 'needs_grad', 'deferred', 'bn_ctx', 'red_ctx', 'red',
               'pre_dy', 'pool_grad')

  def __init__(self, data, shape=None, needs_grad=True):
    self._data = data
    self.shape = tuple(data.shape) if data is not None else tuple(shape)
    self.needs_grad = needs_grad
    self._grad = self.grad_mask = self.pool_grad = self.red = self.pre_dy = None
    self.grad_owned = False
    self.deferred = self.bn_ctx = self.red_ctx = None

  @property
  def data(self):
    if self.bn_pending():
      s = self.deferred
      self._data = ops.bn_apply(s.y, s.M, s.C, s.scale, s.shift, None, 0, False)
    return self._data

  def bn_pending(self) -> bool:
    return self._data is None and self.deferred is not None

  @data.setter
  def data(self, t):
    self._data = t

  @property
  def grad(self):
    if self.grad_mask is not None:
      self.set_grad(ops.mask_apply(self._grad, self.grad_mask), True)
    if self.pool_grad is not None:
      pg, self.pool_grad = self.pool_grad, None
      self._add_scattered(*pg)
    return self._grad

  @grad.setter
  def grad(self, g):
    self.set_grad(g, False)

  def set_grad(self, g, owned: bool, red_part=None):
    self._grad, self.grad_mask, self.grad_owned = g, None, owned
    self.red = (red_part, g) if red_part is not None else None

  def add_grad(self, g, owned: bool, mask=None):
    self.red = None
    if mask is not None:
      if self._grad is None:
        self._grad, self.grad_mask, self.grad_owned = g, mask, False
        return
      g, owned = ops.mask_apply(g, mask), True
    cur = self.grad
    if cur is None:
      self.set_grad(g, owned)
    elif self.grad_owned:
      ops.add_bf16(cur, g, out=cur)
    else:
      self.set_grad(ops.add_bf16(cur, g), True)

  def add_pooled_grad(self, dp, k, stride, pad, count_valid, keep_pooled: bool):
    self.red = None
    if keep_pooled and self.pool_grad is None:
      self.pool_grad = (dp, k, stride, pad, count_valid)
    else:
      self.grad
      self._add_scattered(dp, k, stride, pad, count_valid)

  def _add_scattered(self, dp, k, stride, pad, count_valid):
    self.red = None
    if self._grad is None:
      self._grad = ops.avgpool_bwd(dp, self.shape, k, stride, pad, count_valid)
    elif self.grad_owned:
      ops.avgpool_bwd(dp, self.shape, k, stride, pad, count_valid, addend=self._grad)
    else:
      self._grad = ops.add_bf16(self._grad, ops.avgpool_bwd(dp, self.shape, k, stride, pad, count_valid))
    self.grad_owned = True

  def take_masked_grad(self):
    if self.pool_grad is not None:
      self.grad
    return self._grad, self.grad_mask

  def take_pool_grad(self, d):
    if self.pool_grad is None or not ops.dgrad_pool_ok(d):
      return None
    pg, self.pool_grad = self.pool_grad, None
    return pg

  def take_red(self, g, relu_mask):
    red, self.red = self.red, None
    ok = red is not None and red[1] is g and self.red_ctx is not None and self.red_ctx.mask is relu_mask
    return red[0] if ok else None

  def park_dy(self, dy):
    self.pre_dy = dy

  def take_dy(self):
    dy, self.pre_dy = self.pre_dy, None
    return dy

  def no_grad_yet(self) -> bool:
    return self._grad is None and self.pre_dy is None

  def held(self):
    return self._grad, self.grad_mask, self.pre_dy, self.pool_grad


def accum_grad(v: Var, g: torch.Tensor, owned: bool, mask: Optional[torch.Tensor] = None):
  if v.needs_grad:
    v.add_grad(g, owned, mask)


class Ctx(object):

  def __init__(self, arena: ParamArena, training: bool, dry: bool, bn_momentum: float, device,
               record_tape: bool, layers: Optional[list] = None):
    self.arena = arena
    self.layers = layers if layers is not None else []
    self._cursor = 0
    self.dlogits = None
    self.uniforms = None
    self.db_static = None
    self.rng = None
    self.training = training
    self.dry = dry
    self.bn_momentum = bn_momentum
    self.device = device
    self.tape: Optional[List[Callable[[], None]]] = [] if (record_tape and not dry) else None
    self.taps: "OrderedDict[str, torch.Tensor]" = OrderedDict()
    self._scope: List[str] = []
    self._counters: Dict[Tuple[str, str], int] = {}

  def next_uniform(self, shape):
    if self.uniforms is not None:
      u = next(self.uniforms)
      if tuple(u.shape) != tuple(shape):
        raise ValueError('dropblock uniform has shape %s, expected %s' % (tuple(u.shape), tuple(shape)))
      return u.contiguous()
    return torch.rand(shape, generator=self.rng, device=self.device, dtype=torch.float32)

  def layer(self, factory):
    if self.dry:
      obj = factory()
      self.layers.append(obj)
      return obj
    obj = self.layers[self._cursor]
    self._cursor += 1
    return obj

  def unique(self, base: str) -> str:
    key = ('/'.join(self._scope), base)
    n = self._counters.get(key, 0)
    self._counters[key] = n + 1
    return base if n == 0 else '%s_%d' % (base, n)

  def push_scope(self, default_name: str):
    self._scope.append(self.unique(default_name))

  def pop_scope(self):
    self._scope.pop()

  def full_name(self, layer: str, var: str) -> str:
    return '/'.join(['resnet_model'] + self._scope + [layer, var])

  def record(self, fn: Callable[[], None]):
    if self.tape is not None:
      self.tape.append(fn)

  def tap(self, name: str, v: Var):
    if not self.dry:
      self.taps[name] = v.data

  def backward(self):
    for fn in reversed(self.tape):
      fn()
    self.tape = []


class ConvKernel(object):

  def __init__(self, ctx: Ctx, k: int, cin: int, cout: int, layer_name: Optional[str] = None,
               dense: bool = False, stem: bool = False, need_dgrad: bool = True):
    layer = ctx.unique('dense' if dense else 'conv2d') if layer_name is None else layer_name
    self.name = ctx.full_name(layer, 'kernel')
    self.k, self.cin, self.cout = k, cin, cout
    self.stem = stem
    self.stem_len = _round_up(4 * k, 8)
# ... 161 lines not shown
  out_shape = (N, d.Ho, d.Wo, conv.cout)
  if ctx.dry:
    return Var(None, out_shape)
  a = ctx.arena
  M = N * d.Ho * d.Wo
  Cn = conv.cout
  gamma, beta = a.w(bn.gamma), a.w(bn.beta)
  rm = res_mode if residual is not None else 0
  form = conv_bn_form(ctx, conv, d, M, relu, residual, rm, tap_pre)
  small = form.stats == 'small'
  res_t = residual.data if (residual is not None and form.apply != 'dual') else None
  out_t = mask_t = mean = invstd = None
  if small:
    y, _ = conv.fprop(d, x.data, False)
    out_t, mask_t, mean, invstd = ops.bn_small_fwd(y, M, Cn, gamma, beta, BN_EPS, ctx.bn_momentum, a.st(bn.mm),
                                                   a.st(bn.mv), relu, want_mask=form.want_mask)
  elif form.stats == 'batch':
    y, part = conv.fprop(d, x.data, True)
    mean, invstd, scale, shift = ops.bn_finalize(part, M, Cn, gamma, beta, BN_EPS, ctx.bn_momentum,
                                                 a.st(bn.mm), a.st(bn.mv))
  elif form.fold:
    scale, shift = ops.bn_infer_coeffs(Cn, gamma, beta, a.st(bn.mm), a.st(bn.mv), BN_EPS)
    return Var(conv.fprop_bn(d, x.data, scale, shift, res_t if rm == 1 else None, relu))
  else:
    y, _ = conv.fprop(d, x.data, False)
    scale, shift = ops.bn_infer_coeffs(Cn, gamma, beta, a.st(bn.mm), a.st(bn.mv), BN_EPS)
  if tap_pre is not None:
    ctx.taps[tap_pre] = y
  if form.apply == 'dual':
    sc = residual.deferred
    out_t, mask_t = _with_mask(ops.bn_apply_dual(y, sc.y, M, Cn, scale, shift, sc.scale, sc.shift, relu,
                                                 want_mask=form.want_mask), form.want_mask)
  elif form.apply == 'own':
    out_t, mask_t = _with_mask(ops.bn_apply(y, M, Cn, scale, shift, res_t, rm, relu, d.Ho, d.Wo, want_mask=form.want_mask),
                               form.want_mask)
  out = Var(out_t, out_shape)
  if form.apply == 'defer' or form.save_bn:
    saved = SavedBN(y, M, Cn, gamma, mean, invstd, bn, scale, shift)
    if form.apply == 'defer':
      out.deferred = saved
    if form.save_bn:
      out.bn_ctx = saved
  if form.offer_red:
    out.red_ctx = RedCtx(y, mask_t)

  if ctx.tape is not None:
    x_t = x.data

    def bwd():
      dy = out.take_dy()
      if dy is not None:
        a.notify_grad(bn.gamma)
        conv_input_grad(conv, d, x, x_t, dy, want_red=False)
        return
      dout, in_mask = out.take_masked_grad()
      if dout is None:
        raise RuntimeError('conv_bn backward: no gradient reached this layer')
      bmask, brelu = mask_t, relu
      if in_mask is not None:
        if relu or small or residual is not None:
          dout = out.grad
        else:
          bmask, brelu = in_mask, True
      sc = residual.bn_ctx if (residual is not None and rm == 1) else None
      if residual is None:
        route = 'none'
      elif not relu:
        route = 'dout'
      elif not (lazy_dz_on() and (residual.needs_grad if rm == 1 else rm == 2)):
        route = 'dz'
      elif sc is not None and residual.no_grad_yet() and sc.M == M and sc.C == Cn and dual_bn_on():
        route = 'dual'
      else:
        route = 'lazy'
      dz = None
      if small:
        dy = ops.bn_small_bwd(dout, y, bmask, M, Cn, gamma, mean, invstd, a.g(bn.gamma), a.g(bn.beta))
      elif route == 'dual':
        dy, dy_sc = ops.bn_bwd_dual(dout, y, sc.y, mask_t, M, Cn,
                                    (gamma, mean, invstd, a.g(bn.gamma), a.g(bn.beta)),
                                    (sc.gamma, sc.mean, sc.invstd, a.g(sc.bn.gamma), a.g(sc.bn.beta)))
        residual.park_dy(dy_sc)
      else:
        dy, dz = ops.bn_bwd(dout, y, bmask, brelu, M, Cn, gamma, mean, invstd, a.g(bn.gamma), a.g(bn.beta),
                            route == 'dz', raw_part=out.take_red(dout, bmask))
      a.notify_grad(bn.gamma)
      if route in ('lazy', 'dz', 'dout'):
        g, g_mask, owned = (dout, mask_t, False) if route == 'lazy' else (dz, None, True) if route == 'dz' else (dout, None, False)
        if rm == 2:
          g, g_mask, owned = ops.upsample2x_bwd(g, g_mask), None, True
        accum_grad(residual, g, owned, mask=g_mask)
      conv_input_grad(conv, d, x, x_t, dy)
      out.grad = None
    bwd.relu_mask = mask_t
    ctx.record(bwd)
  return out


def conv_input_grad(conv: ConvKernel, d, x: Var, x_t: torch.Tensor, dy: torch.Tensor, want_red: bool = True):
  pool = x.take_pool_grad(d) if (conv.kpad == conv.cout and x.needs_grad) else None
  xg, xmask = x.take_masked_grad()
  dx, part = conv.backward_red(d, x_t, dy, x.needs_grad, xg, xmask, pool, x.red_ctx if want_red else None)
  if dx is not None:
    x.set_grad(dx, True, part)


def conv_plain(ctx: Ctx, x: Var, conv: ConvKernel, out_f32: bool, ldy: int = 0):
  N, H, W, _ = x.shape
  d = conv.desc(N, H, W, 1, out_f32=out_f32, ldy=ldy)
  if ctx.dry:
    return None, None, (N, d.Ho, d.Wo, ldy if ldy else conv.cout)
  y, _ = conv.fprop(d, x.data, False)
  x_t = x.data

  def bwd(dy: torch.Tensor):
    dd = ops.make_conv_desc(d.N, d.H, d.W, d.C, d.K, d.R, d.S, d.stride, pad=d.pad, Ho=d.Ho, Wo=d.Wo,
                            ldy=ldy if (ldy and ldy != conv.cout) else 0)
    conv_input_grad(conv, dd, x, x_t, dy, want_red=False)
  return y, bwd, tuple(y.shape)


class SKUnit(object):

  def __init__(self, ctx: Ctx, cin: int, filters: int, r: int = 2, L: int = 32):
    self.filters = filters
    self.conv = ConvKernel(ctx, 3, cin, filters * 2)
    self.bn = BatchNorm(ctx, filters * 2)
    self.d = max(int(filters / r), L)
    ctx.push_scope('sk_block')
    self.fc1 = ConvKernel(ctx, 1, filters, self.d, layer_name='sk_fc_1')
    self.bn1 = BatchNorm(ctx, self.d)
    self.fc2 = ConvKernel(ctx, 1, self.d, filters * 2, layer_name='sk_fc_2')
    ctx.pop_scope()

  def __call__(self, ctx: Ctx, x: Var, stride: int) -> Var:
    if ctx.training and not ctx.dry and 2 * self.filters <= 2048 and ops.knob('ASM_SK_FUSED', '1') != '0':
      return self._call_fused(ctx, x, stride)
    F_ = self.filters
    f = conv_bn(ctx, x, self.conv, self.bn, stride, relu=True)
    N, H, W, _ = f.shape
    if ctx.dry:
      return Var(None, (N, H, W, F_))
    s = Var(ops.sk_gap(f.data, F_))
    z = conv_bn(ctx, s, self.fc1, self.bn1, 1, relu=True)
    att, fc2_bwd, _ = conv_plain(ctx, z, self.fc2, out_f32=True)
    v_t = ops.sk_select_fwd(f.data, att, F_)
    v = Var(v_t)
    if ctx.tape is not None:
      bwd_z = ctx.tape.pop()
      bwd_f = ctx.tape.pop()
      f_t = f.data

      def bwd():
        dv = v.grad
        datt = ops.sk_select_bwd_att(f_t, dv, att, F_)
        fc2_bwd(datt)
        bwd_z()
        df = ops.sk_select_bwd_f(dv, att, s.grad, F_)
        s.grad = None
        accum_grad(f, df, True)
        bwd_f()
        v.grad = None
      ctx.record(bwd)
    return v


  def _call_fused(self, ctx: Ctx, x: Var, stride: int) -> Var:
    F_ = self.filters
    conv, bn, a = self.conv, self.bn, ctx.arena
    N, H, W, _ = x.shape
    d = conv.desc(N, H, W, stride)
    M, C2 = N * d.Ho * d.Wo, 2 * F_
    gamma, beta = a.w(bn.gamma), a.w(bn.beta)
    y, part = conv.fprop(d, x.data, True)
    mean, invstd, scale, shift = ops.bn_finalize(part, M, C2, gamma, beta, BN_EPS, ctx.bn_momentum, a.st(bn.mm),
                                                 a.st(bn.mv))
    factor = ctx.tape is not None and ops.knob('ASM_SK_FACTOR', '1') == '1'
    if factor:
      s_t, mask_stats = ops.sk_gap_bn(y, scale, shift, F_, mean, invstd)
      s = Var(s_t)
    else:
      s = Var(ops.sk_gap_bn(y, scale, shift, F_))
    z = conv_bn(ctx, s, self.fc1, self.bn1, 1, relu=True)
    att, fc2_bwd, _ = conv_plain(ctx, z, self.fc2, out_f32=True)
    v = Var(ops.sk_select_bn_fwd(y, scale, shift, att, F_))
    if ctx.tape is not None:
      bwd_z = ctx.tape.pop()
      x_t = x.data

      def bwd():
        dv = v.grad
        if dv is None:
          raise RuntimeError('sk unit backward: no gradient reached this layer')
        if factor:
          datt, grad_stats = ops.sk_select_bn_bwd_att(y, scale, shift, dv, att, F_, mean, invstd)
        else:
          datt, grad_stats = ops.sk_select_bn_bwd_att(y, scale, shift, dv, att, F_), None
        fc2_bwd(datt)
        bwd_z()
        dy = ops.sk_bn_bwd(dv, att, s.grad, y, scale, shift, gamma, mean, invstd, a.g(bn.gamma), a.g(bn.beta), F_,
                           grad_stats, mask_stats if factor else None)
        s.grad = None
        a.notify_grad(bn.gamma)
        conv_input_grad(conv, d, x, x_t, dy)
        v.grad = None
      ctx.record(bwd)
    return v


class SEUnit(object):

  def __init__(self, ctx: Ctx, c: int, ratio: int = 16):
    self.c = c
    ctx.push_scope('se_block')
    self.fc1 = ConvKernel(ctx, 1, c, c // ratio, layer_name='seblock_dense_1')
    self.fc2 = ConvKernel(ctx, 1, c // ratio, c, layer_name='seblock_dense_2')
    ctx.pop_scope()

  def __call__(self, ctx: Ctx, x: Var) -> Var:
    if ctx.dry:
      return Var(None, x.shape)
    sq = Var(ops.gap_fwd(x.data))
    e1_t, fc1_bwd, _ = conv_plain(ctx, sq, self.fc1, out_f32=False)
    e1r = Var(ops.relu_fwd(e1_t))
    e_t, fc2_bwd, _ = conv_plain(ctx, e1r, self.fc2, out_f32=True)
    y = Var(ops.se_scale_fwd(x.data, e_t))
    if ctx.tape is not None:
      x_t = x.data

      def bwd():
        dy = y.grad
        de = ops.se_scale_bwd_e(x_t, dy, e_t)
        fc2_bwd(de)
        fc1_bwd(ops.relu_bwd(e1r.grad, e1r.data))
        accum_grad(x, ops.se_scale_bwd_x(dy, e_t, sq.grad), True)
        e1r.grad = sq.grad = y.grad = None
      ctx.record(bwd)
    return y


def max_pool_3x3_s2_same(ctx: Ctx, x: Var) -> Var:
  N, H, W, Cn = x.shape
  if ctx.dry:
    return Var(None, (N, (H + 1) // 2, (W + 1) // 2, Cn))
  y_t, am = ops.maxpool3x3s2_fwd(x.data)
  y = Var(y_t)
  if ctx.tape is not None:
    def bwd():
      accum_grad(x, ops.maxpool3x3s2_bwd(y.grad, am, x.shape), True)
      y.grad = None
    ctx.record(bwd)
  return y


def avg_pool(ctx: Ctx, x: Var, k: int, stride: int, pad: int, count_valid: bool) -> Var:
  N, H, W, Cn = x.shape
  if count_valid:
    Ho, Wo = H, W
  else:
    Ho, Wo = (H + (k - 1) - k) // stride + 1, (W + (k - 1) - k) // stride + 1
  if ctx.dry:
    return Var(None, (N, Ho, Wo, Cn))
  y = Var(ops.avgpool_fwd(x.data, k, stride, pad, Ho, Wo, count_valid))
  if ctx.tape is not None:
    def bwd():
      if y.grad is None:
        raise RuntimeError('avg_pool backward: no gradient reached this layer')
      if x.needs_grad:
        x.add_pooled_grad(y.grad, k, stride, pad, count_valid,
                          stride in (1, 2) and stride <= k <= 2 * stride and ops.knob('ASM_POOL_FUSE', '1') != '0')
      y.grad = None
    ctx.record(bwd)
  return y


def blur_pool(ctx: Ctx, x: Var, k: int, stride: int) -> Var:
  N, H, W, Cn = x.shape
  if k == 1:
    raise NotImplementedError('anti_alias_filter_size=1 hard-codes NCHW slicing in the reference (blocks.py:79-84)')
  if ctx.dry:
    return Var(None, (N, ops.blur_out_size(H, k, stride), ops.blur_out_size(W, k, stride), Cn))
  y = Var(ops.blurpool_fwd(x.data, k, stride))
  if ctx.tape is not None:
    def bwd():
      accum_grad(x, ops.blurpool_bwd(y.grad, x.shape, k, stride), True)
      y.grad = None
    ctx.record(bwd)
  return y


def global_avg_pool(ctx: Ctx, x: Var) -> Var:
  N, H, W, Cn = x.shape
  if ctx.dry:
    return Var(None, (N, 1, 1, Cn))
  y = Var(ops.gap_fwd(x.data))
  if ctx.tape is not None:
    def bwd():
      accum_grad(x, ops.gap_bwd(y.grad, x.shape), True)
      y.grad = None
    ctx.record(bwd)
  return y


def gem_pool(ctx: Ctx, x: Var, p: float = 3.0) -> Var:
  N, H, W, Cn = x.shape
  if ctx.dry:
    return Var(None, (N, 1, 1, Cn))
  y_t, ssum = ops.gem_fwd(x.data, p)
  y = Var(y_t)
  if ctx.tape is not None:
    x_t = x.data

    def bwd():
      accum_grad(x, ops.gem_bwd(x_t, y.grad, ssum, p), True)
      y.grad = None
    ctx.record(bwd)
  return y


def flatten_pool(ctx: Ctx, x: Var) -> Var:
  N, H, W, Cn = x.shape
  if ctx.dry:
    return Var(None, (N, 1, 1, H * W * Cn))
  y = Var(x.data.view(N, 1, 1, H * W * Cn))
  if ctx.tape is not None:
    def bwd():
      accum_grad(x, y.grad.view(N, H, W, Cn), False)
      y.grad = None
    ctx.record(bwd)
  return y


DROPBLOCK_SIZE = 7


def dropblock_gamma(gamma_scale: float, keep_prob: float, H: int, W: int) -> float:
  bs = DROPBLOCK_SIZE
  return gamma_scale * (1. - keep_prob) * (W * H) / (bs ** 2) / ((W - bs + 1) * (H - bs + 1))


class DropBlockState(object):
  CAP = 256
  RING = 16

  def __init__(self, device):
    self.device = torch.device(device)
    self.slots = []
    self.gamma = torch.zeros((self.CAP,), dtype=torch.float32, device=self.device)
    self.known = False
    self._i = 0
    self._kp = 1.0
    self._pin = None
    self._pin_ev = None
    self._k = 0

  def begin(self, keep_prob: float, uniforms, rng):
    self._i = 0
    self._kp = float(keep_prob)
    self._given = list(uniforms) if uniforms is not None else None
    self._rng = rng
    if not self.known:
      self.slots = []
      return
    n = len(self.slots)
# ... 89 lines not shown
```

### assembled_cnn_amd/ops.py

```python
from __future__ import annotations

import ctypes as C
import os
from typing import Optional, Tuple

import torch

from . import lib as _lib
from .lib import ConvDesc, check

_L = None
_IS_DOUBLE = False


def set_library(obj, is_double: bool = False):
  global _L, _IS_DOUBLE
  _L = obj
  _IS_DOUBLE = is_double


def L():
  global _L
  if _L is None:
    _L = _lib.load()
# ... 301 lines not shown


def filter_transpose_tiled(w_arena, wt_arena, table, nlayers, total_tiles):
  check(L().asm_filter_transpose_tiled(_ptr(w_arena), _ptr(wt_arena), _ptr(table), nlayers, total_tiles, _stream()),
        'filter_transpose_tiled')


def stem_pack_filter(w32: torch.Tensor, wp: torch.Tensor, K: int, ksize: int):
  check(L().asm_stem_pack_filter(_ptr(w32), _ptr(wp), K, ksize, _stream()), 'stem_pack_filter')


def stem_unpack_grad(dwp: torch.Tensor, dw: torch.Tensor, K: int, ksize: int):
  check(L().asm_stem_unpack_grad(_ptr(dwp), _ptr(dw), K, ksize, _stream()), 'stem_unpack_grad')


def stem_pad_input(x: torch.Tensor) -> torch.Tensor:
  N, H, W, c = x.shape
  if c != 3:
    raise ValueError('stem input must have 3 channels')
  if x.dtype not in (F32, BF16):
    raise ValueError('stem input dtype must be float32 or bfloat16')
  xp = empty((N, H + 6, W + 6, 4), BF16, x)
  check(L().asm_stem_pad_input(_ptr(x), 1 if x.dtype == F32 else 0, _ptr(xp), N, H, W, _stream()), 'stem_pad_input')
  return xp


def bn_stats(x2d: torch.Tensor, M: int, Cn: int) -> torch.Tensor:
  blocks = L().asm_bn_stats_blocks(M, Cn)
  if blocks <= 0:
    raise ValueError('bn_stats: bad shape')
  part = empty((blocks, 2, Cn), F32, x2d)
  check(L().asm_bn_stats(_ptr(x2d), M, Cn, _ptr(part), _stream()), 'bn_stats')
  return part


def _compact(part: torch.Tensor, Cn: int) -> torch.Tensor:
  blocks = part.shape[0]
  if blocks <= 1024:
    return part
  per = -(-blocks // 32)
  groups = -(-blocks // per)
  out = empty((groups, 2, Cn), F32, part)
  check(L().asm_bn_partials_compact(_ptr(part), blocks, Cn, _ptr(out), groups, _stream()), 'bn_partials_compact')
  return out


def bn_finalize(part, M, Cn, gamma, beta, eps, momentum, mm, mv):
  ev = _bn_ev(part.numel() * 4.0)
  part = _compact(part, Cn)
  co = empty((4, Cn), F32, part)
  check(L().asm_bn_finalize(_ptr(part), part.shape[0], M, Cn, _ptr(gamma), _ptr(beta), eps, momentum,
                            _ptr(mm), _ptr(mv), _ptr(co[0]), _ptr(co[1]), _ptr(co[2]), _ptr(co[3]),
                            _stream()), 'bn_finalize')
  if ev is not None:
    ev.record()
  return co[0], co[1], co[2], co[3]


def bn_infer_coeffs(Cn, gamma, beta, mm, mv, eps):
  co = empty((2, Cn), F32, gamma)
  check(L().asm_bn_infer_coeffs(Cn, _ptr(gamma), _ptr(beta), _ptr(mm), _ptr(mv), eps, _ptr(co[0]), _ptr(co[1]),
                                _stream()), 'bn_infer_coeffs')
  return co[0], co[1]


def bn_apply(x, M, Cn, scale, shift, residual=None, res_mode=0, relu=False, H=0, W=0, want_mask=False):
  y = torch.empty_like(x)
  mask = empty((M, Cn // 8), torch.uint8, x) if (want_mask and relu) else None
  ev = _bn_ev(M * Cn * (4.0 + (2.0 if res_mode == 1 else 0.5 if res_mode == 2 else 0.0) + (0.125 if mask is not None else 0.0)))
  check(L().asm_bn_apply(_ptr(x), _ptr(y), M, Cn, _ptr(scale), _ptr(shift), _ptr(residual), res_mode,
                         1 if relu else 0, H, W, _ptr(mask), _stream()), 'bn_apply')
  if ev is not None:
    ev.record()
  return (y, mask) if want_mask else y


def _bn_bwd_coeffs(part, M, Cn, gamma, mean, invstd, dgamma, dbeta, co, raw=False):
  part = _compact(part, Cn)
  fin, what = (L().asm_bn_bwd_finalize_raw, 'bn_bwd_finalize_raw') if raw else (L().asm_bn_bwd_finalize, 'bn_bwd_finalize')
  check(fin(_ptr(part), part.shape[0], M, Cn, _ptr(gamma), _ptr(mean), _ptr(invstd), _ptr(dgamma), _ptr(dbeta),
            _ptr(co[0]), _ptr(co[1]), _ptr(co[2]), _stream()), what)


def bn_bwd(dy, x, yout, relu, M, Cn, gamma, mean, invstd, dgamma, dbeta, want_dz, raw_part=None):
  rk = 0 if not relu else (2 if yout.dtype == torch.uint8 else 1)
  red_bytes = 0.0 if raw_part is not None else (4.0 + (0.125 if rk == 2 else 2.0 if rk == 1 else 0.0))
  ev = _bn_ev(M * Cn * (red_bytes + 4.0 + 2.0 + (2.0 if want_dz else 0.0) + (0.125 if rk == 2 else 2.0 if rk == 1 else 0.0)))
  co = empty((3, Cn), F32, dy)
  part = raw_part
  if part is None:
    part = empty((L().asm_bn_stats_blocks(M, Cn), 2, Cn), F32, dy)
    check(L().asm_bn_bwd_reduce(_ptr(dy), _ptr(x), _ptr(yout if relu else None), rk, M, Cn,
                                _ptr(mean), _ptr(invstd), _ptr(part), _stream()), 'bn_bwd_reduce')
  _bn_bwd_coeffs(part, M, Cn, gamma, mean, invstd, dgamma, dbeta, co, raw=raw_part is not None)
  dx = torch.empty_like(x)
  dz = torch.empty_like(x) if want_dz else None
  check(L().asm_bn_bwd_apply(_ptr(dy), _ptr(x), _ptr(yout if relu else None), rk, M, Cn,
                             _ptr(co[0]), _ptr(co[1]), _ptr(co[2]), _ptr(dx), _ptr(dz), _stream()), 'bn_bwd_apply')
  if ev is not None:
    ev.record()
  return dx, dz


def bn_apply_dual(xa, xb, M, Cn, scale_a, shift_a, scale_b, shift_b, relu, want_mask=False):
  y = torch.empty_like(xa)
  mask = empty((M, Cn // 8), torch.uint8, xa) if (want_mask and relu) else None
  ev = _bn_ev(M * Cn * (6.0 + (0.125 if mask is not None else 0.0)))
  check(L().asm_bn_apply2(_ptr(xa), _ptr(xb), _ptr(y), M, Cn, _ptr(scale_a), _ptr(shift_a), _ptr(scale_b), _ptr(shift_b),
                          1 if relu else 0, _ptr(mask), _stream()), 'bn_apply2')
  if ev is not None:
    ev.record()
  return (y, mask) if want_mask else y


def bn_bwd_dual(dy, xa, xb, mask, M, Cn, bn_a, bn_b):
  ev = _bn_ev(M * Cn * (2 * 6.0 + 4.0 + 2 * 0.125))
  blocks = L().asm_bn_stats_blocks(M, Cn)
  pa, pb = empty((blocks, 2, Cn), F32, dy), empty((blocks, 2, Cn), F32, dy)
  check(L().asm_bn_bwd_reduce2(_ptr(dy), _ptr(xa), _ptr(xb), _ptr(mask), M, Cn, _ptr(bn_a[1]), _ptr(bn_a[2]),
                               _ptr(bn_b[1]), _ptr(bn_b[2]), _ptr(pa), _ptr(pb), _stream()), 'bn_bwd_reduce2')
  co = empty((6, Cn), F32, dy)
  for i, (part, (gamma, mean, invstd, dgamma, dbeta)) in enumerate(((pa, bn_a), (pb, bn_b))):
    _bn_bwd_coeffs(part, M, Cn, gamma, mean, invstd, dgamma, dbeta, co[3 * i:3 * i + 3])
  dxa, dxb = torch.empty_like(xa), torch.empty_like(xb)
  check(L().asm_bn_bwd_apply2(_ptr(dy), _ptr(xa), _ptr(xb), _ptr(mask), M, Cn, _ptr(co), _ptr(dxa), _ptr(dxb), _stream()),
        'bn_bwd_apply2')
  if ev is not None:
    ev.record()
  return dxa, dxb


_SMALL_BN_ROWS = None


def bn_small_ok(M: int) -> bool:
  global _SMALL_BN_ROWS
  if _SMALL_BN_ROWS is None:
    _SMALL_BN_ROWS = int(L().asm_bn_small_max_rows())
  return M <= _SMALL_BN_ROWS


def bn_small_fwd(x, M, Cn, gamma, beta, eps, momentum, mm, mv, relu, want_mask):
  y = torch.empty_like(x)
  co = empty((2, Cn), F32, x)
  mask = empty((M, Cn // 8), torch.uint8, x) if (want_mask and relu) else None
  check(L().asm_bn_small_fwd(_ptr(x), _ptr(y), M, Cn, _ptr(gamma), _ptr(beta), eps, momentum, _ptr(mm), _ptr(mv),
                             _ptr(co[0]), _ptr(co[1]), 1 if relu else 0, _ptr(mask), _stream()), 'bn_small_fwd')
  return y, mask, co[0], co[1]


def bn_small_bwd(dy, x, mask, M, Cn, gamma, mean, invstd, dgamma, dbeta):
  dx = torch.empty_like(x)
  check(L().asm_bn_small_bwd(_ptr(dy), _ptr(x), _ptr(mask), M, Cn, _ptr(gamma), _ptr(mean), _ptr(invstd),
                             _ptr(dgamma), _ptr(dbeta), _ptr(dx), _stream()), 'bn_small_bwd')
  return dx


def maxpool3x3s2_fwd(x):
  N, H, W, Cn = x.shape
  Ho, Wo = (H + 1) // 2, (W + 1) // 2
  y = empty((N, Ho, Wo, Cn), BF16, x)
  am = empty((N, Ho, Wo, Cn), torch.uint8, x)
  check(L().asm_maxpool3x3s2_fwd(_ptr(x), _ptr(y), _ptr(am), N, H, W, Cn, _stream()), 'maxpool_fwd')
  return y, am


def maxpool3x3s2_bwd(dy, am, in_shape):
  N, H, W, Cn = in_shape
  dx = empty(in_shape, BF16, dy)
  check(L().asm_maxpool3x3s2_bwd(_ptr(dy), _ptr(am), _ptr(dx), N, H, W, Cn, _stream()), 'maxpool_bwd')
  return dx


def avgpool_fwd(x, k, stride, pad, Ho, Wo, count_valid):
  N, H, W, Cn = x.shape
  y = empty((N, Ho, Wo, Cn), BF16, x)
  check(L().asm_avgpool_fwd(_ptr(x), _ptr(y), N, H, W, Cn, k, stride, pad, Ho, Wo, 1 if count_valid else 0,
                            _stream()), 'avgpool_fwd')
# ... 20 lines not shown


def blur_out_size(n, k, stride):
  return (n + 2 * ((k - 1) // 2) - k) // stride + 1


def blurpool_fwd(x, k, stride):
  N, H, W, Cn = x.shape
  y = empty((N, blur_out_size(H, k, stride), blur_out_size(W, k, stride), Cn), BF16, x)
  check(L().asm_blurpool_fwd(_ptr(x), _ptr(y), N, H, W, Cn, k, stride, _stream()), 'blurpool_fwd')
  return y


def blurpool_bwd(dy, in_shape, k, stride):
  N, H, W, Cn = in_shape
  dx = empty(in_shape, BF16, dy)
  check(L().asm_blurpool_bwd(_ptr(dy), _ptr(dx), N, H, W, Cn, k, stride, _stream()), 'blurpool_bwd')
  return dx


def gap_fwd(x):
  N, H, W, Cn = x.shape
  y = empty((N, 1, 1, Cn), BF16, x)
  check(L().asm_gap_fwd(_ptr(x), _ptr(y), N, H * W, Cn, _stream()), 'gap_fwd')
  return y


def gap_bwd(dy, in_shape):
  N, H, W, Cn = in_shape
  dx = empty(in_shape, BF16, dy)
  check(L().asm_gap_bwd(_ptr(dy), _ptr(dx), N, H * W, Cn, _stream()), 'gap_bwd')
  return dx


def sk_gap(f, F_):
  N, H, W, _ = f.shape
  s = empty((N, 1, 1, F_), BF16, f)
  check(L().asm_sk_gap(_ptr(f), _ptr(s), N, H * W, F_, _stream()), 'sk_gap')
  return s


def sk_select_fwd(f, att, F_):
  N, H, W, _ = f.shape
  v = empty((N, H, W, F_), BF16, f)
  check(L().asm_sk_select_fwd(_ptr(f), _ptr(att), _ptr(v), N, H * W, F_, _stream()), 'sk_select_fwd')
  return v


def sk_select_bwd_att(f, dv, att, F_):
  N, H, W, _ = f.shape
  datt = empty((N, 1, 1, 2 * F_), BF16, f)
  check(L().asm_sk_select_bwd_att(_ptr(f), _ptr(dv), _ptr(att), _ptr(datt), N, H * W, F_, _stream()),
        'sk_select_bwd_att')
  return datt


def sk_select_bwd_f(dv, att, ds, F_):
  N, H, W, _ = dv.shape
  df = empty((N, H, W, 2 * F_), BF16, dv)
  check(L().asm_sk_select_bwd_f(_ptr(dv), _ptr(att), _ptr(ds), _ptr(df), N, H * W, F_, _stream()), 'sk_select_bwd_f')
  return df


def sk_gap_bn(y, scale, shift, F_, mean=None, invstd=None):
  N, H, W, _ = y.shape
  s = empty((N, 1, 1, F_), BF16, y)
  if mean is not None:
    st = empty((N, 2, 2 * F_), F32, y)
    check(L().asm_sk_gap_bn_stats(_ptr(y), _ptr(scale), _ptr(shift), _ptr(mean), _ptr(invstd), _ptr(s), _ptr(st), N, H * W,
                                  F_, _stream()), 'sk_gap_bn_stats')
    return s, st
  check(L().asm_sk_gap_bn(_ptr(y), _ptr(scale), _ptr(shift), _ptr(s), N, H * W, F_, _stream()), 'sk_gap_bn')
  return s


def sk_select_bn_fwd(y, scale, shift, att, F_):
  N, H, W, _ = y.shape
  v = empty((N, H, W, F_), BF16, y)
  check(L().asm_sk_select_bn_fwd(_ptr(y), _ptr(scale), _ptr(shift), _ptr(att), _ptr(v), N, H * W, F_, _stream()),
        'sk_select_bn_fwd')
  return v


def sk_select_bn_bwd_att(y, scale, shift, dv, att, F_, mean=None, invstd=None):
  N, H, W, _ = y.shape
  datt = empty((N, 1, 1, 2 * F_), BF16, y)
  if mean is not None:
    st = empty((N, 2, 2 * F_), F32, y)
    check(L().asm_sk_select_bn_bwd_att_stats(_ptr(y), _ptr(scale), _ptr(shift), _ptr(mean), _ptr(invstd), _ptr(dv), _ptr(att),
                                             _ptr(datt), _ptr(st), N, H * W, F_, _stream()), 'sk_select_bn_bwd_att_stats')
    return datt, st
  check(L().asm_sk_select_bn_bwd_att(_ptr(y), _ptr(scale), _ptr(shift), _ptr(dv), _ptr(att), _ptr(datt), N, H * W, F_,
                                     _stream()), 'sk_select_bn_bwd_att')
  return datt


def sk_bn_bwd(dv, att, ds, y, scale, shift, gamma, mean, invstd, dgamma, dbeta, F_, grad_stats=None, mask_stats=None):
  N, H, W, C2 = y.shape
  HW, M = H * W, N * H * W
  co = empty((3, C2), F32, y)
  if grad_stats is not None and mask_stats is not None:
    ev = _bn_ev(M * (2.0 * C2 + 2.0 * F_ + 2.0 * C2))
    check(L().asm_sk_bn_bwd_finalize(_ptr(grad_stats), _ptr(mask_stats), _ptr(att), _ptr(ds), N, HW, F_, _ptr(gamma),
                                     _ptr(mean), _ptr(invstd), _ptr(dgamma), _ptr(dbeta), _ptr(co[0]), _ptr(co[1]),
                                     _ptr(co[2]), _stream()), 'sk_bn_bwd_finalize')
  else:
    blocks = L().asm_sk_bn_bwd_blocks(N, HW, F_)
    if blocks <= 0:
      raise ValueError('sk_bn_bwd: bad shape')
    ev = _bn_ev(M * (2 * (2.0 * C2 + 2.0 * F_) + 2.0 * C2))
    part = empty((blocks, 2, C2), F32, y)
    check(L().asm_sk_bn_bwd_reduce(_ptr(dv), _ptr(att), _ptr(ds), _ptr(y), _ptr(scale), _ptr(shift), _ptr(mean),
                                   _ptr(invstd), N, HW, F_, _ptr(part), _stream()), 'sk_bn_bwd_reduce')
    _bn_bwd_coeffs(part, M, C2, gamma, mean, invstd, dgamma, dbeta, co)
  dy = torch.empty_like(y)
  check(L().asm_sk_bn_bwd_apply(_ptr(dv), _ptr(att), _ptr(ds), _ptr(y), _ptr(scale), _ptr(shift), _ptr(co[0]),
                                _ptr(co[1]), _ptr(co[2]), _ptr(dy), N, HW, F_, _stream()), 'sk_bn_bwd_apply')
  if ev is not None:
    ev.record()
  return dy


def se_scale_fwd(x, e):
  N, H, W, Cn = x.shape
  y = torch.empty_like(x)
  check(L().asm_se_scale_fwd(_ptr(x), _ptr(e), _ptr(y), N, H * W, Cn, _stream()), 'se_scale_fwd')
  return y


def se_scale_bwd_e(x, dy, e):
  N, H, W, Cn = x.shape
  de = empty((N, 1, 1, Cn), BF16, x)
  check(L().asm_se_scale_bwd_e(_ptr(x), _ptr(dy), _ptr(e), _ptr(de), N, H * W, Cn, _stream()), 'se_scale_bwd_e')
  return de


def se_scale_bwd_x(dy, e, dsq):
  N, H, W, Cn = dy.shape
  dx = torch.empty_like(dy)
  check(L().asm_se_scale_bwd_x(_ptr(dy), _ptr(e), _ptr(dsq), _ptr(dx), N, H * W, Cn, _stream()), 'se_scale_bwd_x')
  return dx


def relu_fwd(x):
  y = torch.empty_like(x)
  check(L().asm_relu_fwd(_ptr(x), _ptr(y), x.numel(), _stream()), 'relu_fwd')
  return y


def relu_bwd(dy, y):
  dx = torch.empty_like(dy)
  check(L().asm_relu_bwd(_ptr(dy), _ptr(y), _ptr(dx), dy.numel(), _stream()), 'relu_bwd')
  return dx


def mask_apply(dy, mask):
  dx = torch.empty_like(dy)
  check(L().asm_mask_apply(_ptr(dy), _ptr(mask), _ptr(dx), dy.numel(), _stream()), 'mask_apply')
  return dx


def add_bf16(a, b, out=None):
  if out is None:
    out = torch.empty_like(a)
  check(L().asm_add_bf16(_ptr(a), _ptr(b), _ptr(out), a.numel(), _stream()), 'add_bf16')
  return out


def bias_add_f32(y, bias, M, Cn, ldy):
  check(L().asm_bias_add_f32(_ptr(y), _ptr(bias), M, Cn, ldy, _stream()), 'bias_add')


def bias_grad_bf16(dz, M, Cn, ld, dbias):
  check(L().asm_bias_grad_bf16(_ptr(dz), M, Cn, ld, _ptr(dbias), _stream()), 'bias_grad')


def cast_f32_to_bf16(x, y):
  check(L().asm_cast_f32_to_bf16(_ptr(x), _ptr(y), x.numel(), _stream()), 'cast')


def cast_bf16_to_f32(x, y):
  check(L().asm_cast_bf16_to_f32(_ptr(x), _ptr(y), x.numel(), _stream()), 'cast_bf16_to_f32')


def softmax_ce(logits, ld, targets, teacher, B, Cn, label_smoothing, kd_temp, loss_scale, ld_out, want_grad=True):
  loss_rows = empty((B,), F32, logits)
  dlogits = empty((B, 1, 1, ld_out), BF16, logits) if want_grad else None
  check(L().asm_softmax_ce(_ptr(logits), ld, _ptr(targets), _ptr(teacher), B, Cn, label_smoothing, kd_temp,
                           loss_scale, _ptr(loss_rows), _ptr(dlogits), ld_out, _stream()), 'softmax_ce')
  return loss_rows, dlogits


def onehot(labels_i32, B, Cn):
  out = empty((B, Cn), F32, labels_i32)
  check(L().asm_onehot(_ptr(labels_i32), _ptr(out), B, Cn, _stream()), 'onehot')
  return out


# ... 275 lines not shown
```

### include/asm_hip.h

```cpp
#ifndef ASM_HIP_H_
#define ASM_HIP_H_

#include <stddef.h>
#include <stdint.h>

#ifdef __cplusplus
extern "C" {
#endif

#define ASM_OK 0
#define ASM_EINVAL (-1)
#define ASM_ENOTSUP (-2)
#define ASM_EHIP (-3)

#define ASM_ABI_VERSION 11

const char* asm_last_error(void);
int asm_abi_version(void);
unsigned long long asm_launch_count(void);

int asm_stream_join(void* dst_stream, void* src_stream);
int asm_memcpy_async(void* dst, const void* src, size_t bytes, void* stream);

int asm_allreduce_bucket(void* buf, size_t count, int dtype, void* nccl_comm, void* comm_stream, void* producer_stream);
// ... 19 lines not shown
  int32_t igemm8;
  int32_t dense_small;
} asm_tuning;
void asm_tuning_defaults(asm_tuning* t);
int asm_set_tuning(const asm_tuning* t);
void asm_get_tuning(asm_tuning* t);

typedef struct asm_conv_desc {
  int32_t N, H, W, C;
  int32_t K, R, S;
  int32_t stride, pad;
  int32_t Ho, Wo;
  int64_t x_img_pitch;
  int32_t x_row_pitch;
  int32_t x_pix_pitch;
  int32_t ldy;
  int32_t out_f32;
} asm_conv_desc;

int asm_conv2d_fprop(const asm_conv_desc* d, const void* x, const void* w, void* y,
                     float* stats_partial, void* stream);
int asm_conv2d_stats_blocks(const asm_conv_desc* d);

int asm_conv2d_fprop_bn(const asm_conv_desc* d, const void* x, const void* w, void* y, const float* scale,
                        const float* shift, const void* residual, int relu, void* stream);

int asm_conv2d_dgrad(const asm_conv_desc* d, const void* dy, const void* wt, const void* addend, void* dx,
                     void* stream);

int asm_conv2d_dgrad_masked(const asm_conv_desc* d, const void* dy, const void* wt, const void* addend,
                            const uint8_t* addend_mask, void* dx, void* stream);
int asm_conv2d_dgrad_pooled(const asm_conv_desc* d, const void* dy, const void* wt, const void* addend,
                            const uint8_t* addend_mask, const void* pool_dy, int pool_k, int pool_stride, int pool_pad,
                            int pool_Ho, int pool_Wo, int count_valid, void* dx, void* stream);

int asm_conv2d_dgrad_bnred_blocks(const asm_conv_desc* d);
int asm_conv2d_dgrad_bnred(const asm_conv_desc* d, const void* dy, const void* wt, const void* addend,
                           const uint8_t* addend_mask, const void* bn_y, const uint8_t* bn_relu_mask, float* partial,
                           void* dx, void* stream);

#define ASM_DGRAD_MASKED 1
#define ASM_DGRAD_POOLED 2
#define ASM_DGRAD_BNRED 4
int asm_conv2d_dgrad_kernel(const asm_conv_desc* d, int variant);

size_t asm_conv2d_wgrad_workspace_bytes(const asm_conv_desc* d);
int asm_conv2d_wgrad(const asm_conv_desc* d, const void* x, const void* dy, float* dw,
                     void* workspace, size_t workspace_bytes, void* stream);

int asm_filter_transpose(const void* w_krsc, void* w_crsk, int K, int R, int S, int C, int ldk, void* stream);

int asm_filter_transpose_batched(const void* w_arena, void* wt_arena, const int32_t* table, int nlayers,
                                 long long total_elems, void* stream);
int asm_filter_transpose_tiled(const void* w_arena, void* wt_arena, const int32_t* table, int nlayers,
                               int total_tiles, void* stream);

int asm_stem_pack_filter(const float* w_krsc3, void* w_packed, int K, int ksize, void* stream);
int asm_stem_unpack_grad(const float* dw_packed, float* dw_krsc3, int K, int ksize, void* stream);
int asm_stem_pad_input(const void* x, int x_is_f32, void* xp, int N, int H, int W, void* stream);

int asm_bn_stats_blocks(int M, int C);
int asm_bn_stats(const void* x, int M, int C, float* stats_partial, void* stream);
int asm_bn_partials_compact(const float* partial, int blocks, int C, float* out, int groups, void* stream);
int asm_bn_finalize(const float* stats_partial, int blocks, int M, int C, const float* gamma,
                    const float* beta, float eps, float momentum, float* moving_mean,
                    float* moving_var, float* mean, float* invstd, float* scale, float* shift,
                    void* stream);
int asm_bn_infer_coeffs(int C, const float* gamma, const float* beta, const float* moving_mean,
                        const float* moving_var, float eps, float* scale, float* shift, void* stream);
int asm_bn_apply(const void* x, void* y, int M, int C, const float* scale, const float* shift,
                 const void* residual, int res_mode, int relu, int H, int W, uint8_t* relu_mask_out,
                 void* stream);
int asm_bn_bwd_reduce(const void* dy, const void* x, const void* yout, int relu, int M, int C,
                      const float* mean, const float* invstd, float* partial, void* stream);
int asm_bn_bwd_finalize(const float* partial, int blocks, int M, int C, const float* gamma,
                        const float* mean, const float* invstd, float* dgamma, float* dbeta,
                        float* coefA, float* coefB, float* coefC, void* stream);
int asm_bn_bwd_finalize_raw(const float* partial, int blocks, int M, int C, const float* gamma,
                            const float* mean, const float* invstd, float* dgamma, float* dbeta,
                            float* coefA, float* coefB, float* coefC, void* stream);
int asm_bn_bwd_apply(const void* dy, const void* x, const void* yout, int relu, int M, int C,
                     const float* coefA, const float* coefB, const float* coefC, void* dx,
                     void* dz_out, void* stream);

int asm_bn_apply2(const void* xa, const void* xb, void* y, int M, int C, const float* scale_a, const float* shift_a,
                  const float* scale_b, const float* shift_b, int relu, uint8_t* relu_mask_out, void* stream);
int asm_bn_bwd_reduce2(const void* dy, const void* xa, const void* xb, const uint8_t* relu_mask, int M, int C,
                       const float* mean_a, const float* invstd_a, const float* mean_b, const float* invstd_b,
                       float* partial_a, float* partial_b, void* stream);
int asm_bn_bwd_apply2(const void* dy, const void* xa, const void* xb, const uint8_t* relu_mask, int M, int C,
                      const float* coef6, void* dxa, void* dxb, void* stream);

int asm_bn_small_max_rows(void);
int asm_bn_small_fwd(const void* x, void* y, int M, int C, const float* gamma, const float* beta, float eps,
                     float momentum, float* moving_mean, float* moving_var, float* mean, float* invstd, int relu,
                     uint8_t* relu_mask_out, void* stream);
int asm_bn_small_bwd(const void* dy, const void* x, const uint8_t* relu_mask, int M, int C, const float* gamma,
                     const float* mean, const float* invstd, float* dgamma, float* dbeta, void* dx, void* stream);

int asm_dense_small(const void* p, int ldp, const void* q, int ldq, int M, int N, int K, void* out, int ldo,
                    int out_f32, const void* addend, void* stream);
int asm_dense_small_wgrad(const void* x, int ldx, const void* dy, int ldy, int M, int Cin, int Cout, float* dw, int ldw,
                          void* stream);

int asm_maxpool3x3s2_fwd(const void* x, void* y, uint8_t* argmax, int N, int H, int W, int C, void* stream);
int asm_maxpool3x3s2_bwd(const void* dy, const uint8_t* argmax, void* dx, int N, int H, int W, int C, void* stream);
int asm_avgpool_fwd(const void* x, void* y, int N, int H, int W, int C, int k, int stride, int pad,
                    int Ho, int Wo, int count_valid, void* stream);
int asm_avgpool_bwd(const void* dy, void* dx, int N, int H, int W, int C, int k, int stride, int pad,
                    int Ho, int Wo, int count_valid, const void* addend, void* stream);
int asm_upsample2x_bwd(const void* dy, void* dx, int N, int Hs, int Ws, int C, void* stream);
int asm_upsample2x_bwd_masked(const void* dy, const uint8_t* relu_mask, void* dx, int N, int Hs, int Ws, int C,
                              void* stream);
int asm_blurpool_fwd(const void* x, void* y, int N, int H, int W, int C, int k, int stride, void* stream);
int asm_blurpool_bwd(const void* dy, void* dx, int N, int H, int W, int C, int k, int stride, void* stream);
int asm_gap_fwd(const void* x, void* y, int N, int HW, int C, void* stream);
int asm_gap_bwd(const void* dy, void* dx, int N, int HW, int C, void* stream);

int asm_sk_gap(const void* f, void* s, int N, int HW, int F, void* stream);
int asm_sk_select_fwd(const void* f, const float* att, void* v, int N, int HW, int F, void* stream);
int asm_sk_select_bwd_att(const void* f, const void* dv, const float* att, void* datt, int N, int HW, int F, void* stream);
int asm_sk_select_bwd_f(const void* dv, const float* att, const void* ds, void* df, int N, int HW, int F, void* stream);
int asm_sk_gap_bn(const void* y, const float* scale, const float* shift, void* s, int N, int HW, int F, void* stream);
int asm_sk_select_bn_fwd(const void* y, const float* scale, const float* shift, const float* att, void* v, int N,
                         int HW, int F, void* stream);
int asm_sk_select_bn_bwd_att(const void* y, const float* scale, const float* shift, const void* dv, const float* att,
                             void* datt, int N, int HW, int F, void* stream);
int asm_sk_bn_bwd_blocks(int N, int HW, int F);
int asm_sk_bn_bwd_reduce(const void* dv, const float* att, const void* ds, const void* y, const float* scale,
                         const float* shift, const float* mean, const float* invstd, int N, int HW, int F,
                         float* partial, void* stream);
int asm_sk_bn_bwd_apply(const void* dv, const float* att, const void* ds, const void* y, const float* scale,
                        const float* shift, const float* coefA, const float* coefB, const float* coefC, void* dy,
                        int N, int HW, int F, void* stream);
int asm_sk_gap_bn_stats(const void* y, const float* scale, const float* shift, const float* mean, const float* invstd,
                        void* s, float* mask_stats, int N, int HW, int F, void* stream);
int asm_sk_select_bn_bwd_att_stats(const void* y, const float* scale, const float* shift, const float* mean,
                                   const float* invstd, const void* dv, const float* att, void* datt, float* grad_stats,
                                   int N, int HW, int F, void* stream);
int asm_sk_bn_bwd_finalize(const float* grad_stats, const float* mask_stats, const float* att, const void* ds, int N,
                           int HW, int F, const float* gamma, const float* mean, const float* invstd, float* dgamma,
                           float* dbeta, float* coefA, float* coefB, float* coefC, void* stream);
int asm_se_scale_fwd(const void* x, const float* e, void* y, int N, int HW, int C, void* stream);
int asm_se_scale_bwd_e(const void* x, const void* dy, const float* e, void* de, int N, int HW, int C, void* stream);
int asm_se_scale_bwd_x(const void* dy, const float* e, const void* dsq, void* dx, int N, int HW, int C, void* stream);

int asm_relu_fwd(const void* x, void* y, size_t n, void* stream);
int asm_relu_bwd(const void* dy, const void* y, void* dx, size_t n, void* stream);
int asm_add_bf16(const void* a, const void* b, void* out, size_t n, void* stream);
int asm_mask_apply(const void* dy, const uint8_t* mask, void* dx, size_t n, void* stream);
int asm_bias_add_f32(float* y, const float* bias, int M, int C, int ldy, void* stream);
int asm_bias_grad_bf16(const void* dz, int M, int C, int ld, float* dbias, void* stream);
int asm_cast_f32_to_bf16(const float* x, void* y, size_t n, void* stream);
int asm_cast_bf16_to_f32(const void* x, float* y, size_t n, void* stream);

int asm_softmax_ce(const float* logits, int ld, const float* targets, const float* teacher, int B,
                   int C, float label_smoothing, float kd_temp, float loss_scale, float* loss_rows,
                   void* dlogits, int ld_out, void* stream);
int asm_onehot(const int32_t* labels, float* out, int B, int C, void* stream);
int asm_softmax_rows(const float* x, float* y, int B, int C, float inv_temp, void* stream);
int asm_mean_f32(const float* x, int n, float* out, void* stream);

int asm_mixup_meansub(const void* images, int is_u8, int Bin, int H, int W, int mixup_type,
                      const float* lam1, const float* lam2, void* out, void* stream);
int asm_mixup_labels(const float* y, int Bin, int C, int mixup_type, const float* lam1,
                     const float* lam2, float* out, void* stream);

int asm_sgd_momentum(float* w, float* accum, const float* grad, void* w_bf16, size_t n, float lr,
                     float momentum, float weight_decay, float grad_scale, void* stream);

int asm_sigmoid_ce(const float* logits, int ld, const float* targets, int B, int C, float loss_scale,
                   float* rows_ws, float* loss_out, void* dlogits, int ld_out, void* stream);
int asm_gem_fwd(const void* x, void* y, float* ssum, int N, int HW, int C, float p, void* stream);
int asm_gem_bwd(const void* x, const void* dy, const float* ssum, void* dx, int N, int HW, int C, float p,
                void* stream);
int asm_dropblock_mask(const float* uniform, float gamma, int H, int W, int C, int block_size, float* keep,
                       float* scale, void* stream);
int asm_dropblock_mask_dev(const float* uniform, const float* gamma_dev, int H, int W, int C, int block_size, float* keep,
                           float* scale, void* stream);
int asm_dropblock_apply(const void* x, const float* keep, const float* scale, const void* relu_mask_from, int relu,
                        void* y, int N, int HWC, void* stream);
int asm_eval_rows(const float* logits, int ld, const int32_t* labels, int B, int C, int32_t* pred, float* conf,
                  float* top1, float* top5, void* stream);
int asm_eval_accumulate(const float* conf, const float* top1, const float* top5, int B, float* state33,
                        void* stream);

int asm_embed_sqnorm(const void* x, int N, int D, int ld, float* sq, void* stream);
size_t asm_retrieval_topk_workspace_bytes(int Q, int N, int K);
int asm_retrieval_topk(const void* queries, int ldq, const void* index, int ldi, const float* sq_queries,
                       const float* sq_index, int Q, int N, int D, int similarity, int K, int index_base,
                       float* top_val, int32_t* top_idx, void* workspace, size_t workspace_bytes, void* stream);
int asm_topk_merge(const float* in_val, const int32_t* in_idx, int rows, int P, int K, float* out_val, int32_t* out_idx,
                   void* stream);
#define ASM_TOPK_WIDE_MAX 1024
size_t asm_retrieval_topk_wide_workspace_bytes(int Q, int N, int K);
int asm_retrieval_topk_wide(const void* queries, int ldq, const void* index, int ldi, const float* sq_queries,
                            const float* sq_index, int Q, int N, int D, int similarity, int K, int index_base,
                            float* top_val, int32_t* top_idx, void* workspace, size_t workspace_bytes, void* stream);
int asm_topk_merge_wide(const float* in_val, const int32_t* in_idx, int rows, int P, int K, float* out_val, int32_t* out_idx,
                        void* stream);
int asm_recall_accumulate(const int32_t* top_idx, int Q, int K, const int32_t* query_labels, const int32_t* index_labels,
                          int N, int query_base, const int32_t* k_list, int nk, int32_t* hits, void* stream);

typedef struct asm_image_desc {
  int64_t src_offset;
  int32_t Hs, Ws;
  int32_t crop_y, crop_x, crop_h, crop_w;
  int32_t resize_h, resize_w;
  int32_t out_y, out_x;
  int32_t flip;
  int32_t reserved;
} asm_image_desc;
int asm_resize_crop_flip(const uint8_t* src, int64_t src_bytes, const asm_image_desc* descs, int N,
                         int out_h, int out_w, int subtract_mean, float* out, void* stream);

typedef struct asm_augment_op {
  int32_t op, a, b, reserved;
  float f[6];
} asm_augment_op;
typedef struct asm_augment_desc {
  asm_augment_op slot[2];
} asm_augment_desc;
int asm_autoaugment_workspace_bytes(int N, int H, int W, int64_t* bytes);
int asm_autoaugment(const float* in, const asm_augment_desc* descs, int N, int H, int W, int subtract_mean, float* out,
                    void* workspace, int64_t workspace_bytes, void* stream);
// ... 125 lines not shown
```

Before: 10650 images/sec.

## Fuse SK select and anti-alias blur-pool, and fuse BN backward with block-sum

Adds a kernel that computes the SK branch select (BN+ReLU+attention mix) directly into an LDS band and applies the 3x3 stride-2 blur in the same pass, so the full-resolution selected tensor is never written. In backward, the SK attention/BN kernels recompute the full-resolution gradient on the fly from the pooled gradient instead of reading a materialised one. A second fused kernel emits the BN backward dx together with the 2x2 block sum of the masked gradient, removing a separate pooling-backward read. The change adds recomputation, LDS usage and more index math, and relies on lazy tape plumbing in the Python layer.

```diff
diff --git a/assembled_cnn_amd/build.py b/assembled_cnn_amd/build.py
--- a/assembled_cnn_amd/build.py
+++ b/assembled_cnn_amd/build.py
@@ -11,7 +11,7 @@
 OBJ_DIR = os.path.join(CSRC, '_obj')
 LIB_PATH = os.path.join(HERE, 'libasm_hip.so')
 SOURCES = ['conv_igemm.hip', 'conv_igemm8.hip', 'conv_gemm1.hip', 'conv_dgrad_s2.hip', 'conv_wgrad.hip', 'bn.hip', 'pool.hip', 'sk_se.hip', 'sk_fused.hip', 'dense_small.hip', 'misc.hip', 'extra.hip', 'input.hip', 'autoaugment.hip', 'jpeg.hip', 'plan.hip', 'tape.hip', 'collective.hip', 'retrieval.hip']
-HEADERS = [os.path.join(CSRC, 'common.h'), os.path.join(CSRC, 'igemm_common.h'), os.path.join(CSRC, 'jpeg_entropy.h'), os.path.join(CSRC, 'jpeg_parallel.h'), os.path.join(HERE, '..', 'include', 'asm_hip.h'),
+HEADERS = [os.path.join(CSRC, 'common.h'), os.path.join(CSRC, 'igemm_common.h'), os.path.join(CSRC, 'blur3s2.h'), os.path.join(CSRC, 'jpeg_entropy.h'), os.path.join(CSRC, 'jpeg_parallel.h'), os.path.join(HERE, '..', 'include', 'asm_hip.h'),
            os.path.join(HERE, '..', 'include', 'asm_hip_debug.h')]
 ARCH = 'gfx950'
 CFLAGS = ['--offload-arch=' + ARCH, '-O3', '-std=c++17', '-fPIC', '-fno-gpu-rdc', '-Wall', '-Wno-unused-function']
diff --git a/assembled_cnn_amd/csrc/blur3s2.h b/assembled_cnn_amd/csrc/blur3s2.h
--- /dev/null
+++ b/assembled_cnn_amd/csrc/blur3s2.h
@@ -0,0 +1,43 @@
+#pragma once
+#include "common.h"
+
+struct BlurCoef {
+  float a[8];
+};
+inline BlurCoef blur_coef(int k) {
+  static const int tri[8][7] = {{0}, {1}, {1, 1}, {1, 2, 1}, {1, 3, 3, 1}, {1, 4, 6, 4, 1}, {1, 5, 10, 10, 5, 1},
+                                {1, 6, 15, 20, 15, 6, 1}};
+  BlurCoef c;
+  int sum = 0;
+  for (int i = 0; i < k; ++i) sum += tri[k][i];
+  for (int i = 0; i < 8; ++i) c.a[i] = i < k ? (float)tri[k][i] / (float)sum : 0.f;
+  return c;
+}
+__device__ __forceinline__ int reflect(int i, int L) {
+  if (i < 0) i = -i;
+  if (i >= L) i = 2 * (L - 1) - i;
+  return i;
+}
+
+template <class Get>
+__device__ __forceinline__ void blur3s2_bwd_pixel(Get get, bool u, bool v, bool hv, bool wv, bool h0, bool w0, float a0,
+                                                  float a1, float a2, float* acc) {
+  const int src[3] = {1, 0, 0};
+  const float wh[3] = {a0, u ? a2 : a1, a0}, ww[3] = {a0, v ? a2 : a1, a0};
+  const bool okh[3] = {u && hv, true, u && h0}, okw[3] = {v && wv, true, v && w0};
+#pragma unroll
+  for (int e = 0; e < 8; ++e) acc[e] = 0.f;
+#pragma unroll
+  for (int th = 0; th < 3; ++th) {
+    if (!okh[th]) continue;
+#pragma unroll
+    for (int tw = 0; tw < 3; ++tw) {
+      if (!okw[tw]) continue;
+      const float wgt = wh[th] * ww[tw];
+      float t[8];
+      get(src[th], src[tw], t);
+#pragma unroll
+      for (int e = 0; e < 8; ++e) acc[e] += t[e] * wgt;
+    }
+  }
+}
diff --git a/assembled_cnn_amd/csrc/bn.hip b/assembled_cnn_amd/csrc/bn.hip
--- a/assembled_cnn_amd/csrc/bn.hip
+++ b/assembled_cnn_amd/csrc/bn.hip
@@ -418,6 +418,50 @@
   });
 }
 
+__global__ __launch_bounds__(256) void bn_bwd_apply_bsum_kernel(size_t nquad, int C, FastDiv fd_vcols,
+                                                                const bf16_t* __restrict__ dy, const bf16_t* __restrict__ x,
+                                                                const uint8_t* __restrict__ mask, const float* __restrict__ cA,
+                                                                const float* __restrict__ cB, const float* __restrict__ cC,
+                                                                bf16_t* __restrict__ dx, bf16_t* __restrict__ bsum,
+                                                                FastDiv fd_ws, FastDiv fd_hs, int Hs, int Ws) {
+  const float* const coef[3] = {cA, cB, cC};
+  const unsigned vcols = (unsigned)(C >> 3);
+  for_each_vec<3>(nquad, C, fd_vcols, coef, [&](size_t i, unsigned m, int vc, const float (&k)[3][8]) {
+    const unsigned nh = fd_div(m, fd_ws);
+    const unsigned j = m - nh * (unsigned)Ws;
+    const unsigned n = fd_div(nh, fd_hs);
+    const unsigned h = nh - n * (unsigned)Hs;
+    const unsigned p00 = (n * 2u * (unsigned)Hs + 2u * h) * (2u * (unsigned)Ws) + 2u * j;
+    size_t idx[4];
+    u32x4 vg[4], vx[4];
+    unsigned mk[4];
+#pragma unroll
+    for (int q = 0; q < 4; ++q) {
+      idx[q] = (size_t)((p00 + (unsigned)(q >> 1) * 2u * (unsigned)Ws + (unsigned)(q & 1)) * vcols + (unsigned)vc);
+      vg[q] = __builtin_nontemporal_load(reinterpret_cast<const u32x4*>(dy + idx[q] * 8));
+      vx[q] = __builtin_nontemporal_load(reinterpret_cast<const u32x4*>(x + idx[q] * 8));
+      mk[q] = mask[idx[q]];
+    }
+    float acc[8];
+#pragma unroll
+    for (int e = 0; e < 8; ++e) acc[e] = 0.f;
+#pragma unroll
+    for (int q = 0; q < 4; ++q) {
+      float g[8], fx[8], o[8];
+      unpack8(vg[q], g);
+      unpack8(vx[q], fx);
+      mask8(g, mk[q]);
+#pragma unroll
+      for (int e = 0; e < 8; ++e) {
+        acc[e] += g[e];
+        o[e] = bwd_dx(k[0][e], g[e], k[1][e], fx[e], k[2][e]);
+      }
+      BN_ST_BWD(pack8(o), reinterpret_cast<u32x4*>(dx + idx[q] * 8));
+    }
+    *reinterpret_cast<u32x4*>(bsum + i * 8) = pack8(acc);
+  });
+}
+
 struct BwdRow2 {
   const bf16_t* __restrict__ dy;
   const bf16_t* __restrict__ xa;
@@ -851,6 +895,20 @@
   return ASM_OK;
 }
 
+extern "C" int asm_bn_bwd_apply_blocksum(const void* dy, const void* x, const uint8_t* relu_mask, int N, int H, int W, int C,
+                                         const float* coefA, const float* coefB, const float* coefC, void* dx,
+                                         void* block_sum, void* stream) {
+  ASM_REQUIRE(dy && x && relu_mask && dx && block_sum && coefA && coefB && coefC, "bn_bwd_apply_blocksum: null pointer");
+  ASM_REQUIRE(N > 0 && H > 0 && W > 0 && H % 2 == 0 && W % 2 == 0 && C > 0 && C % 8 == 0,
+              "bn_bwd_apply_blocksum: bad shape (N=%d H=%d W=%d C=%d; H and W must be even)", N, H, W, C);
+  ASM_REQUIRE((size_t)N * H * W * (C / 8) < 0x7fffffffull, "bn_bwd_apply_blocksum: tensor too large");
+  const int Hs = H / 2, Ws = W / 2;
+  launch_vecs(bn_bwd_apply_bsum_kernel, stream, N * Hs * Ws, C, (const bf16_t*)dy, (const bf16_t*)x, relu_mask, coefA, coefB,
+              coefC, (bf16_t*)dx, (bf16_t*)block_sum, make_fastdiv((unsigned)Ws), make_fastdiv((unsigned)Hs), Hs, Ws);
+  ASM_CHECK_LAUNCH("bn_bwd_apply_blocksum");
+  return ASM_OK;
+}
+
 extern "C" int asm_bn_small_max_rows(void) { return SMALL_BN_MAX_ROWS; }
 
 extern "C" int asm_bn_small_fwd(const void* x, void* y, int M, int C, const float* gamma, const float* beta, float eps,
diff --git a/assembled_cnn_amd/csrc/pool.hip b/assembled_cnn_amd/csrc/pool.hip
--- a/assembled_cnn_amd/csrc/pool.hip
+++ b/assembled_cnn_amd/csrc/pool.hip
@@ -1,4 +1,5 @@
 #include "common.h"
+#include "blur3s2.h"
 
 namespace {
 
@@ -213,24 +214,6 @@
       for (int e = 0; e < 8; ++e) acc[e] += g[e];
     }
   *reinterpret_cast<u32x4*>(dx + i * 8) = pack8(acc);
-}
-
-struct BlurCoef {
-  float a[8];
-};
-inline BlurCoef blur_coef(int k) {
-  static const int tri[8][7] = {{0}, {1}, {1, 1}, {1, 2, 1}, {1, 3, 3, 1}, {1, 4, 6, 4, 1}, {1, 5, 10, 10, 5, 1},
-                                {1, 6, 15, 20, 15, 6, 1}};
-  BlurCoef c;
-  int sum = 0;
-  for (int i = 0; i < k; ++i) sum += tri[k][i];
-  for (int i = 0; i < 8; ++i) c.a[i] = i < k ? (float)tri[k][i] / (float)sum : 0.f;
-  return c;
-}
-__device__ __forceinline__ int reflect(int i, int L) {
-  if (i < 0) i = -i;
-  if (i >= L) i = 2 * (L - 1) - i;
-  return i;
 }
 
 __global__ __launch_bounds__(256) void blur_fwd_kernel(const bf16_t* __restrict__ x, bf16_t* __restrict__ y, int N,
@@ -321,32 +304,16 @@
       const size_t off = (((size_t)p.n * Hh + p.h + (ok ? a : 0)) * Wh + p.w + (ok ? b : 0)) * C + p.vc * 8;
       unpack8(ldv(dy, off), g[a][b]);
     }
-  const int src_odd[3] = {1, 0, 0};
-  const float wgt_odd[3] = {a0, a2, a0};
-  const bool okh[3] = {hv, true, p.h == 0}, okw[3] = {wv, true, p.w == 0};
   const int W2 = 2 * Wh;
 #pragma unroll
   for (int u = 0; u < 2; ++u)
 #pragma unroll
     for (int v = 0; v < 2; ++v) {
       float acc[8];
-#pragma unroll
-      for (int e = 0; e < 8; ++e) acc[e] = 0.f;
-#pragma unroll
-      for (int th = 0; th < (u ? 3 : 1); ++th) {
-        const int sh = u ? src_odd[th] : 0;
-        const float wh = u ? wgt_odd[th] : a1;
-        if (u && !okh[th]) continue;
-#pragma unroll
-        for (int tw = 0; tw < (v ? 3 : 1); ++tw) {
-          const int sw = v ? src_odd[tw] : 0;
-          const float ww = v ? wgt_odd[tw] : a1;
-          if (v && !okw[tw]) continue;
-          const float wgt = wh * ww;
-#pragma unroll
-          for (int e = 0; e < 8; ++e) acc[e] += g[sh][sw][e] * wgt;
-        }
-      }
+      blur3s2_bwd_pixel([&](int a, int b, float* t) {
+#pragma unroll
+        for (int e = 0; e < 8; ++e) t[e] = g[a][b][e];
+      }, u != 0, v != 0, hv, wv, p.h == 0, p.w == 0, a0, a1, a2, acc);
       const size_t off = (((size_t)p.n * 2 * Hh + 2 * p.h + u) * W2 + 2 * p.w + v) * C + p.vc * 8;
       *reinterpret_cast<u32x4*>(dx + off) = pack8(acc);
     }
diff --git a/assembled_cnn_amd/csrc/sk_fused.hip b/assembled_cnn_amd/csrc/sk_fused.hip
--- a/assembled_cnn_amd/csrc/sk_fused.hip
+++ b/assembled_cnn_amd/csrc/sk_fused.hip
@@ -1,4 +1,5 @@
 #include "common.h"
+#include "blur3s2.h"
 
 namespace {
 
@@ -17,7 +18,8 @@
     k.sh[e] = h0[e]; k.sh[e + 4] = h1[e];
   }
 }
-__device__ __forceinline__ void bnrelu8(const u32x4& vy, const Coef8& k, float* f) {
+template <class K>
+__device__ __forceinline__ void bnrelu8(const u32x4& vy, const K& k, float* f) {
   float y[8];
   unpack8(vy, y);
 #pragma unroll
@@ -75,7 +77,12 @@
   }
 }
 
-__device__ __forceinline__ void bnrelu8m(const u32x4& vy, const Coef8& k, float* f, float* m, float* my) {
+struct CoefLds {
+  const float* sc;
+  const float* sh;
+};
+template <class K>
+__device__ __forceinline__ void bnrelu8m(const u32x4& vy, const K& k, float* f, float* m, float* my) {
   float y[8];
   unpack8(vy, y);
 #pragma unroll
@@ -160,6 +167,106 @@
         *reinterpret_cast<f32x4*>(dst) = f32x4{o[0], o[1], o[2], o[3]};
         *reinterpret_cast<f32x4*>(dst + 4) = f32x4{o[4], o[5], o[6], o[7]};
       }
+    }
+  }
+}
+
+struct PoolGeom {
+  int W, Hh, Wh;
+  FastDiv fd_w;
+  float a0, a1, a2;
+};
+
+__device__ __forceinline__ u32x4 dv_from_pooled(const bf16_t* __restrict__ gimg, const PoolGeom& pg, int F, int r) {
+  const int h = (int)fd_div((unsigned)r, pg.fd_w), w = r - h * pg.W;
+  const int i = h >> 1, j = w >> 1;
+  const bool u = h & 1, v = w & 1;
+  const bool hv = i + 1 < pg.Hh, wv = j + 1 < pg.Wh;
+  u32x4 g[2][2];
+#pragma unroll
+  for (int a = 0; a < 2; ++a)
+#pragma unroll
+    for (int b = 0; b < 2; ++b) {
+      const bool ok = (a == 0 || (u && hv)) && (b == 0 || (v && wv));
+      g[a][b] = ldv(gimg, ((size_t)(i + (ok ? a : 0)) * pg.Wh + j + (ok ? b : 0)) * F);
+    }
+  float acc[8];
+  blur3s2_bwd_pixel([&](int a, int b, float* t) { unpack8(g[a][b], t); }, u, v, hv, wv, i == 0, j == 0, pg.a0, pg.a1, pg.a2,
+                    acc);
+  return pack8(acc);
+}
+
+__global__ __launch_bounds__(256) void sk_select_blur_fwd_kernel(const bf16_t* __restrict__ y, const float* __restrict__ scale,
+                                                                 const float* __restrict__ shift,
+                                                                 const float* __restrict__ att, bf16_t* __restrict__ out,
+                                                                 int H, int W, int F, int fvb, int rpb, int bh,
+                                                                 FastDiv fd_wo, float b0, float b1, float b2) {
+  extern __shared__ u32x4 vband[];
+  const int fv = F >> 3;
+  const int vcl = threadIdx.x % fvb, rr = threadIdx.x / fvb;
+  const int vc = blockIdx.z * fvb + vcl;
+  const int n = blockIdx.y;
+  const bool live = rr < rpb && vc < fv;
+  const int Ho = H >> 1, Wo = W >> 1;
+  const int ho0 = blockIdx.x * bh;
+  const int nbh = min(bh, Ho - ho0);
+  if (live) {
+    Coef8 k0, k1;
+    load_coef(scale, shift, vc * 8, k0);
+    load_coef(scale, shift, F + vc * 8, k1);
+    float a0[8];
+    gate8(att, n, F, vc * 8, a0);
+    const bf16_t* yn = y + (size_t)n * H * W * 2 * F + vc * 8;
+    const int npix = (2 * nbh + 1) * W;
+    const int first = (2 * ho0 - 1) * W;
+    constexpr int U = 2;
+    for (int p = rr; p < npix; p += U * rpb) {
+      u32x4 y0[U], y1[U];
+#pragma unroll
+      for (int q = 0; q < U; ++q) {
+        const int pq = p + q * rpb;
+        int gp = first + (pq < npix ? pq : p);
+        if (gp < 0) gp += 2 * W;
+        y0[q] = ldv(yn, (size_t)gp * 2 * F);
+        y1[q] = ldv(yn, (size_t)gp * 2 * F + F);
+      }
+#pragma unroll
+      for (int q = 0; q < U; ++q) {
+        const int pq = p + q * rpb;
+        if (pq >= npix) break;
+        float f0[8], f1[8], o[8];
+        bnrelu8(y0[q], k0, f0);
+        bnrelu8(y1[q], k1, f1);
+#pragma unroll
+        for (int e = 0; e < 8; ++e) o[e] = a0[e] * f0[e] + (1.0f - a0[e]) * f1[e];
+        vband[pq * fvb + vcl] = pack8(o);
+      }
+    }
+  }
+  __syncthreads();
+  if (live) {
+    const float bw[3] = {b0, b1, b2};
+    const int nout = nbh * Wo;
+    for (int q = rr; q < nout; q += rpb) {
+      const int oh = (int)fd_div((unsigned)q, fd_wo), ow = q - oh * Wo;
+      float acc[8];
+#pragma unroll
+      for (int e = 0; e < 8; ++e) acc[e] = 0.f;
+#pragma unroll
+      for (int r = 0; r < 3; ++r) {
+        const int lr = 2 * oh + r;
+#pragma unroll
+        for (int t = 0; t < 3; ++t) {
+          int iw = 2 * ow + t - 1;
+          if (iw < 0) iw = 1;
+          float f[8];
+          unpack8(vband[(lr * W + iw) * fvb + vcl], f);
+          const float wgt = bw[r] * bw[t];
+#pragma unroll
+          for (int e = 0; e < 8; ++e) acc[e] += f[e] * wgt;
+        }
+      }
+      *reinterpret_cast<u32x4*>(out + (((size_t)n * Ho + ho0 + oh) * Wo + ow) * F + vc * 8) = pack8(acc);
     }
   }
 }
@@ -203,13 +310,15 @@
   }
 }
 
-template <int NT, bool ST>
+template <int NT, bool ST, bool PG>
 __global__ __launch_bounds__(NT, NT == 256 ? 4 : 1) void sk_bn_bwd_att_kernel(const bf16_t* __restrict__ y, const float* __restrict__ scale,
                                                            const float* __restrict__ shift, const bf16_t* __restrict__ dv,
                                                            const float* __restrict__ att, bf16_t* __restrict__ datt,
                                                            int HW, int F, int vcb, const float* __restrict__ mean,
-                                                           const float* __restrict__ invstd, float* __restrict__ stats) {
+                                                           const float* __restrict__ invstd, float* __restrict__ stats,
+                                                           PoolGeom pg) {
   __shared__ float red[NT][9];
+  __shared__ float cfl[PG ? 4 * 256 : 1];
   const int vcols = F >> 3;
   const int vcl = threadIdx.x % vcb, rl = threadIdx.x / vcb, nrl = NT / vcb;
   const int vc = blockIdx.x * vcb + vcl;
@@ -217,11 +326,26 @@
   float acc[8], g0[8], x0[8], g1[8], x1[8];
 #pragma unroll
   for (int e = 0; e < 8; ++e) acc[e] = g0[e] = x0[e] = g1[e] = x1[e] = 0.f;
+  if (PG) {
+    if (rl == 0 && vc < vcols) {
+#pragma unroll
+      for (int e = 0; e < 8; ++e) {
+        cfl[vcl * 8 + e] = scale[vc * 8 + e];
+        cfl[256 + vcl * 8 + e] = shift[vc * 8 + e];
+        cfl[512 + vcl * 8 + e] = scale[F + vc * 8 + e];
+        cfl[768 + vcl * 8 + e] = shift[F + vc * 8 + e];
+      }
+    }
+    __syncthreads();
+  }
   if (vc < vcols && rl < nrl) {
-    Coef8 k0, k1;
-    load_coef(scale, shift, vc * 8, k0);
-    load_coef(scale, shift, F + vc * 8, k1);
-    auto consume = [&](const u32x4& v0, const u32x4& v1, const u32x4& vg) {
+    Coef8 r0, r1;
+    if (!PG) {
+      load_coef(scale, shift, vc * 8, r0);
+      load_coef(scale, shift, F + vc * 8, r1);
+    }
+    const CoefLds l0 = {cfl + vcl * 8, cfl + 256 + vcl * 8}, l1 = {cfl + 512 + vcl * 8, cfl + 768 + vcl * 8};
+    auto add_pixel = [&](const auto& k0, const auto& k1, const u32x4& v0, const u32x4& v1, const u32x4& vg) {
       float g[8];
       unpack8(vg, g);
       if (ST) {
@@ -240,6 +364,16 @@
         for (int e = 0; e < 8; ++e) acc[e] += (f0[e] - f1[e]) * g[e];
       }
     };
+    auto consume = [&](const u32x4& v0, const u32x4& v1, const u32x4& vg) {
+      if (PG) {
+        __asm__ volatile("" ::: "memory");
+        add_pixel(l0, l1, v0, v1, vg);
+      } else {
+        add_pixel(r0, r1, v0, v1, vg);
+      }
+    };
+    const bf16_t* gimg = PG ? dv + (size_t)n * pg.Hh * pg.Wh * F + vc * 8 : nullptr;
+    auto load_dv = [&](int rq) { return PG ? dv_from_pooled(gimg, pg, F, rq) : ldv(dv, ((size_t)n * HW + rq) * F + vc * 8); };
     constexpr int U = ST ? 1 : 2;
     int r = rl;
     for (; r + (U - 1) * nrl < HW; r += U * nrl) {
@@ -249,14 +383,14 @@
         const size_t m = (size_t)n * HW + r + u * nrl;
         v0[u] = ldv(y, m * 2 * F + vc * 8);
         v1[u] = ldv(y, m * 2 * F + F + vc * 8);
-        vg[u] = ldv(dv, m * F + vc * 8);
+        vg[u] = load_dv(r + u * nrl);
       }
 #pragma unroll
       for (int u = 0; u < U; ++u) consume(v0[u], v1[u], vg[u]);
     }
     for (; r < HW; r += nrl) {
       const size_t m = (size_t)n * HW + r;
-      consume(ldv(y, m * 2 * F + vc * 8), ldv(y, m * 2 * F + F + vc * 8), ldv(dv, m * F + vc * 8));
+      consume(ldv(y, m * 2 * F + vc * 8), ldv(y, m * 2 * F + F + vc * 8), load_dv(r));
     }
   }
   const bool leader = rl == 0 && vc < vcols;
@@ -408,12 +542,13 @@
   }
 }
 
+template <bool PG>
 __global__ __launch_bounds__(256) void sk_bn_bwd_apply_kernel(const bf16_t* __restrict__ dv, const float* __restrict__ att,
                                                               const bf16_t* __restrict__ ds, const bf16_t* __restrict__ y,
                                                               const float* __restrict__ scale,
                                                               const float* __restrict__ shift, const float* __restrict__ cA,
                                                               const float* __restrict__ cB, const float* __restrict__ cC,
-                                                              bf16_t* __restrict__ dy, SkBnGeom g) {
+                                                              bf16_t* __restrict__ dy, SkBnGeom g, PoolGeom pg) {
   const int tid = threadIdx.x;
   const int vc = tid % g.vcols;
   const int rr = tid / g.vcols;
@@ -432,6 +567,7 @@
     kC[e] = cC[vc * 8 + e];
   }
   sk_thread_setup(g, n, vc, att, ds, ab, u);
+  const bf16_t* gimg = PG ? dv + (size_t)n * pg.Hh * pg.Wh * g.F + cv * 8 : nullptr;
   const int r_begin = blockIdx.x * g.rows_per_chunk;
   const int r_end = min(g.HW, r_begin + g.rows_per_chunk);
   constexpr int U = 2;
@@ -440,9 +576,10 @@
 #pragma unroll
     for (int q = 0; q < U; ++q) {
       const int rq = r + q * g.rpb;
-      const size_t m = (size_t)n * g.HW + (rq < r_end ? rq : r);
+      const int rc = rq < r_end ? rq : r;
+      const size_t m = (size_t)n * g.HW + rc;
       vy[q] = __builtin_nontemporal_load(reinterpret_cast<const u32x4*>(y + m * C2 + vc * 8));
-      vg[q] = ldv(dv, m * g.F + cv * 8);
+      vg[q] = PG ? dv_from_pooled(gimg, pg, g.F, rc) : ldv(dv, m * g.F + cv * 8);
     }
 #pragma unroll
     for (int q = 0; q < U; ++q) {
@@ -537,18 +674,55 @@
   return ASM_OK;
 }
 
+#define SKB_OK(name)                                                                                                    \
+  ASM_REQUIRE(k == 3 && stride == 2, name ": blur filter size %d / stride %d not supported (3 / 2 only)", k, stride);    \
+  ASM_REQUIRE(H > 0 && W > 0 && H % 2 == 0 && W % 2 == 0, name ": H=%d W=%d must be even", H, W);                        \
+  const int HW = H * W;                                                                                                 \
+  SKF_OK(name)
+
+static PoolGeom make_pool_geom(int H, int W) {
+  const BlurCoef cf = blur_coef(3);
+  return PoolGeom{W, H / 2, W / 2, make_fastdiv((unsigned)W), cf.a[0], cf.a[1], cf.a[2]};
+}
+
+constexpr int SKB_BAND = 2;
+constexpr int SKB_MAX_W = 512;
+constexpr size_t SKB_LDS = 40 * 1024;
+
+extern "C" int asm_sk_select_bn_blur_fwd(const void* y, const float* scale, const float* shift, const float* att, void* out,
+                                         int N, int H, int W, int F, int k, int stride, void* stream) {
+  SKB_OK("sk_select_bn_blur_fwd");
+  ASM_REQUIRE(y && scale && shift && att && out, "sk_select_bn_blur_fwd: null pointer");
+  ASM_REQUIRE(W <= SKB_MAX_W, "sk_select_bn_blur_fwd: W=%d above %d", W, SKB_MAX_W);
+  const int fv = F / 8, rows = 2 * SKB_BAND + 1;
+  int fvb = fv < 32 ? fv : 32;
+  while (fvb > 1 && (size_t)rows * W * fvb * 16 > SKB_LDS) fvb = cdiv(fvb, 2);
+  const int groups = cdiv(fv, fvb);
+  ASM_REQUIRE(groups <= 65535, "sk_select_bn_blur_fwd: too many column groups");
+  const BlurCoef cf = blur_coef(3);
+  const unsigned lds = (unsigned)((size_t)rows * W * fvb * 16);
+  ASM_LAUNCH(sk_select_blur_fwd_kernel, dim3(cdiv(H / 2, SKB_BAND), N, groups), dim3(256), lds, (hipStream_t)stream,
+                     (const bf16_t*)y, scale, shift, att, (bf16_t*)out, H, W, F, fvb, 256 / fvb, SKB_BAND,
+                     make_fastdiv((unsigned)(W / 2)), cf.a[0], cf.a[1], cf.a[2]);
+  ASM_CHECK_LAUNCH("sk_select_bn_blur_fwd");
+  return ASM_OK;
+}
+
 static int sk_att_impl(const void* y, const float* scale, const float* shift, const void* dv, const float* att, void* datt,
-                       int N, int HW, int F, const float* mean, const float* invstd, float* stats, void* stream) {
+                       int N, int HW, int F, const float* mean, const float* invstd, float* stats, void* stream,
+                       const PoolGeom* pooled = nullptr) {
   SKF_OK("sk_select_bn_bwd_att");
   ASM_REQUIRE(y && scale && shift && dv && att && datt, "sk_select_bn_bwd_att: null pointer");
   const int vcb = image_pass_vcb(N, F);
   const dim3 grid(cdiv(F / 8, vcb), N);
   hipStream_t st = (hipStream_t)stream;
-#define LAUNCH_ATT(NT, ST)                                                                                          \
-  ASM_LAUNCH((sk_bn_bwd_att_kernel<NT, ST>), grid, dim3(NT), 0, st, (const bf16_t*)y, scale, shift, (const bf16_t*)dv, \
-                     att, (bf16_t*)datt, HW, F, vcb, mean, invstd, stats)
-  if (stats) { if (HW >= 512) LAUNCH_ATT(1024, true); else LAUNCH_ATT(256, true); }
-  else { if (HW >= 512) LAUNCH_ATT(1024, false); else LAUNCH_ATT(256, false); }
+  const PoolGeom pg = pooled ? *pooled : PoolGeom{};
+#define LAUNCH_ATT(NT, ST, PG)                                                                                          \
+  ASM_LAUNCH((sk_bn_bwd_att_kernel<NT, ST, PG>), grid, dim3(NT), 0, st, (const bf16_t*)y, scale, shift, (const bf16_t*)dv, \
+                     att, (bf16_t*)datt, HW, F, vcb, mean, invstd, stats, pg)
+  if (pooled) { if (HW >= 512) LAUNCH_ATT(1024, true, true); else LAUNCH_ATT(256, true, true); }
+  else if (stats) { if (HW >= 512) LAUNCH_ATT(1024, true, false); else LAUNCH_ATT(256, true, false); }
+  else { if (HW >= 512) LAUNCH_ATT(1024, false, false); else LAUNCH_ATT(256, false, false); }
 #undef LAUNCH_ATT
   ASM_CHECK_LAUNCH("sk_select_bn_bwd_att");
   return ASM_OK;
@@ -564,6 +738,16 @@
                                               float* grad_stats, int N, int HW, int F, void* stream) {
   ASM_REQUIRE(mean && invstd && grad_stats, "sk_select_bn_bwd_att_stats: null pointer");
   return sk_att_impl(y, scale, shift, dv, att, datt, N, HW, F, mean, invstd, grad_stats, stream);
+}
+
+extern "C" int asm_sk_select_bn_bwd_att_stats_blur(const void* y, const float* scale, const float* shift, const float* mean,
+                                                   const float* invstd, const void* dpool, const float* att, void* datt,
+                                                   float* grad_stats, int N, int H, int W, int F, int k, int stride,
+                                                   void* stream) {
+  SKB_OK("sk_select_bn_bwd_att_stats_blur");
+  ASM_REQUIRE(mean && invstd && grad_stats, "sk_select_bn_bwd_att_stats_blur: null pointer");
+  const PoolGeom pg = make_pool_geom(H, W);
+  return sk_att_impl(y, scale, shift, dpool, att, datt, N, HW, F, mean, invstd, grad_stats, stream, &pg);
 }
 
 extern "C" int asm_sk_bn_bwd_finalize(const float* grad_stats, const float* mask_stats, const float* att, const void* ds,
@@ -601,9 +785,23 @@
   SKF_OK("sk_bn_bwd_apply");
   ASM_REQUIRE(dv && att && ds && y && scale && shift && coefA && coefB && coefC && dy, "sk_bn_bwd_apply: null pointer");
   const SkBnGeom g = make_geom(N, HW, F);
-  ASM_LAUNCH(sk_bn_bwd_apply_kernel, dim3(g.chunks, N), dim3(256), 0, (hipStream_t)stream,
+  ASM_LAUNCH(sk_bn_bwd_apply_kernel<false>, dim3(g.chunks, N), dim3(256), 0, (hipStream_t)stream,
                      (const bf16_t*)dv, att, (const bf16_t*)ds, (const bf16_t*)y, scale, shift, coefA, coefB, coefC,
-                     (bf16_t*)dy, g);
+                     (bf16_t*)dy, g, PoolGeom{});
   ASM_CHECK_LAUNCH("sk_bn_bwd_apply");
   return ASM_OK;
 }
+
+extern "C" int asm_sk_bn_bwd_apply_blur(const void* dpool, const float* att, const void* ds, const void* y,
+                                        const float* scale, const float* shift, const float* coefA, const float* coefB,
+                                        const float* coefC, void* dy, int N, int H, int W, int F, int k, int stride,
+                                        void* stream) {
+  SKB_OK("sk_bn_bwd_apply_blur");
+  ASM_REQUIRE(dpool && att && ds && y && scale && shift && coefA && coefB && coefC && dy, "sk_bn_bwd_apply_blur: null pointer");
+  const SkBnGeom g = make_geom(N, HW, F);
+  ASM_LAUNCH(sk_bn_bwd_apply_kernel<true>, dim3(g.chunks, N), dim3(256), 0, (hipStream_t)stream,
+                     (const bf16_t*)dpool, att, (const bf16_t*)ds, (const bf16_t*)y, scale, shift, coefA, coefB, coefC,
+                     (bf16_t*)dy, g, make_pool_geom(H, W));
+  ASM_CHECK_LAUNCH("sk_bn_bwd_apply_blur");
+  return ASM_OK;
+}
diff --git a/assembled_cnn_amd/lib.py b/assembled_cnn_amd/lib.py
--- a/assembled_cnn_amd/lib.py
+++ b/assembled_cnn_amd/lib.py
@@ -172,6 +172,7 @@
     'asm_bn_bwd_finalize': (_I, [_P, _I, _I, _I, _P, _P, _P, _P, _P, _P, _P, _P, _P]),
     'asm_bn_bwd_finalize_raw': (_I, [_P, _I, _I, _I, _P, _P, _P, _P, _P, _P, _P, _P, _P]),
     'asm_bn_bwd_apply': (_I, [_P, _P, _P, _I, _I, _I, _P, _P, _P, _P, _P, _P]),
+    'asm_bn_bwd_apply_blocksum': (_I, [_P, _P, _P, _I, _I, _I, _I, _P, _P, _P, _P, _P, _P]),
     'asm_maxpool3x3s2_fwd': (_I, [_P, _P, _P, _I, _I, _I, _I, _P]),
     'asm_maxpool3x3s2_bwd': (_I, [_P, _P, _P, _I, _I, _I, _I, _P]),
     'asm_avgpool_fwd': (_I, [_P, _P, _I, _I, _I, _I, _I, _I, _I, _I, _I, _I, _P]),
@@ -188,12 +189,15 @@
     'asm_sk_select_bwd_f': (_I, [_P, _P, _P, _P, _I, _I, _I, _P]),
     'asm_sk_gap_bn': (_I, [_P, _P, _P, _P, _I, _I, _I, _P]),
     'asm_sk_select_bn_fwd': (_I, [_P, _P, _P, _P, _P, _I, _I, _I, _P]),
+    'asm_sk_select_bn_blur_fwd': (_I, [_P, _P, _P, _P, _P, _I, _I, _I, _I, _I, _I, _P]),
     'asm_sk_select_bn_bwd_att': (_I, [_P, _P, _P, _P, _P, _P, _I, _I, _I, _P]),
     'asm_sk_bn_bwd_blocks': (_I, [_I, _I, _I]),
     'asm_sk_bn_bwd_reduce': (_I, [_P, _P, _P, _P, _P, _P, _P, _P, _I, _I, _I, _P, _P]),
     'asm_sk_bn_bwd_apply': (_I, [_P, _P, _P, _P, _P, _P, _P, _P, _P, _P, _I, _I, _I, _P]),
+    'asm_sk_bn_bwd_apply_blur': (_I, [_P, _P, _P, _P, _P, _P, _P, _P, _P, _P, _I, _I, _I, _I, _I, _I, _P]),
     'asm_sk_gap_bn_stats': (_I, [_P, _P, _P, _P, _P, _P, _P, _I, _I, _I, _P]),
     'asm_sk_select_bn_bwd_att_stats': (_I, [_P, _P, _P, _P, _P, _P, _P, _P, _P, _I, _I, _I, _P]),
+    'asm_sk_select_bn_bwd_att_stats_blur': (_I, [_P, _P, _P, _P, _P, _P, _P, _P, _P, _I, _I, _I, _I, _I, _I, _P]),
     'asm_sk_bn_bwd_finalize': (_I, [_P, _P, _P, _P, _I, _I, _I, _P, _P, _P, _P, _P, _P, _P, _P, _P]),
     'asm_se_scale_fwd': (_I, [_P, _P, _P, _I, _I, _I, _P]),
     'asm_se_scale_bwd_e': (_I, [_P, _P, _P, _P, _I, _I, _I, _P]),
diff --git a/assembled_cnn_amd/nn.py b/assembled_cnn_amd/nn.py
--- a/assembled_cnn_amd/nn.py
+++ b/assembled_cnn_amd/nn.py
@@ -278,6 +278,14 @@
   shift: torch.Tensor
 
 
+class LazyV(NamedTuple):
+  y: torch.Tensor
+  scale: torch.Tensor
+  shift: torch.Tensor
+  att: torch.Tensor
+  F: int
+
+
 class RedCtx(NamedTuple):
   y: torch.Tensor
   mask: Optional[torch.Tensor]
@@ -285,13 +293,13 @@
 
 class Var(object):
   __slots__ = ('_data', 'shape', '_grad', 'grad_mask', 'grad_owned', 'needs_grad', 'deferred', 'bn_ctx', 'red_ctx', 'red',
-               'pre_dy', 'pool_grad')
+               'pre_dy', 'pool_grad', 'lazy_v', 'blur_grad')
 
   def __init__(self, data, shape=None, needs_grad=True):
     self._data = data
     self.shape = tuple(data.shape) if data is not None else tuple(shape)
     self.needs_grad = needs_grad
-    self._grad = self.grad_mask = self.pool_grad = self.red = self.pre_dy = None
+    self._grad = self.grad_mask = self.pool_grad = self.red = self.pre_dy = self.lazy_v = self.blur_grad = None
     self.grad_owned = False
     self.deferred = self.bn_ctx = self.red_ctx = None
 
@@ -300,7 +308,17 @@
     if self.bn_pending():
       s = self.deferred
       self._data = ops.bn_apply(s.y, s.M, s.C, s.scale, s.shift, None, 0, False)
+    elif self._data is None and self.lazy_v is not None:
+      s, self.lazy_v = self.lazy_v, None
+      self._data = ops.sk_select_bn_fwd(s.y, s.scale, s.shift, s.att, s.F)
     return self._data
+
+  def take_lazy_v(self, k: int, stride: int):
+    s = self.lazy_v
+    if self._data is not None or s is None or not ops.sk_blur_ok(self.shape[1], self.shape[2], k, stride):
+      return None
+    self.lazy_v = None
+    return s
 
   def bn_pending(self) -> bool:
     return self._data is None and self.deferred is not None
@@ -311,6 +329,7 @@
 
   @property
   def grad(self):
+    self._scatter_blur_grad()
     if self.grad_mask is not None:
       self.set_grad(ops.mask_apply(self._grad, self.grad_mask), True)
     if self.pool_grad is not None:
@@ -328,6 +347,7 @@
 
   def add_grad(self, g, owned: bool, mask=None):
     self.red = None
+    self._scatter_blur_grad()
     if mask is not None:
       if self._grad is None:
         self._grad, self.grad_mask, self.grad_owned = g, mask, False
@@ -359,7 +379,24 @@
       self._grad = ops.add_bf16(self._grad, ops.avgpool_bwd(dp, self.shape, k, stride, pad, count_valid))
     self.grad_owned = True
 
+  def add_blur_grad(self, dp, k, stride):
+    self.red = None
+    if self._grad is None and self.pool_grad is None and self.blur_grad is None:
+      self.blur_grad = (dp, k, stride)
+    else:
+      self.add_grad(ops.blurpool_bwd(dp, self.shape, k, stride), True)
+
+  def take_blur_grad(self):
+    bg, self.blur_grad = self.blur_grad, None
+    return bg
+
+  def _scatter_blur_grad(self):
+    if self.blur_grad is not None:
+      (dp, k, stride), self.blur_grad = self.blur_grad, None
+      self.set_grad(ops.blurpool_bwd(dp, self.shape, k, stride), True)
+
   def take_masked_grad(self):
+    self._scatter_blur_grad()
     if self.pool_grad is not None:
       self.grad
     return self._grad, self.grad_mask
@@ -383,9 +420,10 @@
     return dy
 
   def no_grad_yet(self) -> bool:
-    return self._grad is None and self.pre_dy is None
+    return self._grad is None and self.pre_dy is None and self.blur_grad is None
 
   def held(self):
+    self._scatter_blur_grad()
     return self._grad, self.grad_mask, self.pre_dy, self.pool_grad
 
 
@@ -713,12 +751,16 @@
                                     (sc.gamma, sc.mean, sc.invstd, a.g(sc.bn.gamma), a.g(sc.bn.beta)))
         residual.park_dy(dy_sc)
       else:
-        dy, dz = ops.bn_bwd(dout, y, bmask, brelu, M, Cn, gamma, mean, invstd, a.g(bn.gamma), a.g(bn.beta),
-                            route == 'dz', raw_part=out.take_red(dout, bmask))
+        bsum_hw = ((d.Ho, d.Wo) if (route == 'lazy' and rm == 2 and bmask is mask_t
+                                    and ops.bn_blocksum_ok(bmask, brelu, False, d.Ho, d.Wo)) else None)
+        dy, dz, *bsum = ops.bn_bwd(dout, y, bmask, brelu, M, Cn, gamma, mean, invstd, a.g(bn.gamma), a.g(bn.beta),
+                                   route == 'dz', raw_part=out.take_red(dout, bmask), block_sum=bsum_hw)
       a.notify_grad(bn.gamma)
       if route in ('lazy', 'dz', 'dout'):
         g, g_mask, owned = (dout, mask_t, False) if route == 'lazy' else (dz, None, True) if route == 'dz' else (dout, None, False)
-        if rm == 2:
+        if rm == 2 and bsum:
+          g, g_mask, owned = bsum[0], None, True
+        elif rm == 2:
           g, g_mask, owned = ops.upsample2x_bwd(g, g_mask), None, True
         accum_grad(residual, g, owned, mask=g_mask)
       conv_input_grad(conv, d, x, x_t, dy)
@@ -814,23 +856,28 @@
       s = Var(ops.sk_gap_bn(y, scale, shift, F_))
     z = conv_bn(ctx, s, self.fc1, self.bn1, 1, relu=True)
     att, fc2_bwd, _ = conv_plain(ctx, z, self.fc2, out_f32=True)
-    v = Var(ops.sk_select_bn_fwd(y, scale, shift, att, F_))
+    if factor and ops.sk_blur_ok(d.Ho, d.Wo, 3, 2):
+      v = Var(None, (N, d.Ho, d.Wo, F_))
+      v.lazy_v = LazyV(y, scale, shift, att, F_)
+    else:
+      v = Var(ops.sk_select_bn_fwd(y, scale, shift, att, F_))
     if ctx.tape is not None:
       bwd_z = ctx.tape.pop()
       x_t = x.data
 
       def bwd():
-        dv = v.grad
+        blur = v.take_blur_grad() if factor else None
+        dv, blur = (blur[0], blur[1:]) if blur is not None else (v.grad, None)
         if dv is None:
           raise RuntimeError('sk unit backward: no gradient reached this layer')
         if factor:
-          datt, grad_stats = ops.sk_select_bn_bwd_att(y, scale, shift, dv, att, F_, mean, invstd)
+          datt, grad_stats = ops.sk_select_bn_bwd_att(y, scale, shift, dv, att, F_, mean, invstd, blur=blur)
         else:
           datt, grad_stats = ops.sk_select_bn_bwd_att(y, scale, shift, dv, att, F_), None
         fc2_bwd(datt)
         bwd_z()
         dy = ops.sk_bn_bwd(dv, att, s.grad, y, scale, shift, gamma, mean, invstd, a.g(bn.gamma), a.g(bn.beta), F_,
-                           grad_stats, mask_stats if factor else None)
+                           grad_stats, mask_stats if factor else None, blur=blur)
         s.grad = None
         a.notify_grad(bn.gamma)
         conv_input_grad(conv, d, x, x_t, dy)
@@ -911,6 +958,15 @@
     raise NotImplementedError('anti_alias_filter_size=1 hard-codes NCHW slicing in the reference (blocks.py:79-84)')
   if ctx.dry:
     return Var(None, (N, ops.blur_out_size(H, k, stride), ops.blur_out_size(W, k, stride), Cn))
+  lazy = x.take_lazy_v(k, stride) if ctx.tape is not None else None
+  if lazy is not None:
+    y = Var(ops.sk_select_bn_blur_fwd(lazy.y, lazy.scale, lazy.shift, lazy.att, lazy.F, k, stride))
+
+    def bwd_lazy():
+      x.add_blur_grad(y.grad, k, stride)
+      y.grad = None
+    ctx.record(bwd_lazy)
+    return y
   y = Var(ops.blurpool_fwd(x.data, k, stride))
   if ctx.tape is not None:
     def bwd():
diff --git a/assembled_cnn_amd/ops.py b/assembled_cnn_amd/ops.py
--- a/assembled_cnn_amd/ops.py
+++ b/assembled_cnn_amd/ops.py
@@ -407,10 +407,16 @@
             _ptr(co[0]), _ptr(co[1]), _ptr(co[2]), _stream()), what)
 
 
-def bn_bwd(dy, x, yout, relu, M, Cn, gamma, mean, invstd, dgamma, dbeta, want_dz, raw_part=None):
+def bn_blocksum_ok(yout, relu, want_dz, H, W) -> bool:
+  return (knob('ASM_BL_SUM', '1') != '0' and relu and not want_dz and yout is not None and yout.dtype == torch.uint8
+          and H > 0 and W > 0 and H % 2 == 0 and W % 2 == 0 and getattr(L(), 'asm_bn_bwd_apply_blocksum', None) is not None)
+
+
+def bn_bwd(dy, x, yout, relu, M, Cn, gamma, mean, invstd, dgamma, dbeta, want_dz, raw_part=None, block_sum=None):
   rk = 0 if not relu else (2 if yout.dtype == torch.uint8 else 1)
   red_bytes = 0.0 if raw_part is not None else (4.0 + (0.125 if rk == 2 else 2.0 if rk == 1 else 0.0))
-  ev = _bn_ev(M * Cn * (red_bytes + 4.0 + 2.0 + (2.0 if want_dz else 0.0) + (0.125 if rk == 2 else 2.0 if rk == 1 else 0.0)))
+  ev = _bn_ev(M * Cn * (red_bytes + 4.0 + 2.0 + (2.0 if want_dz else 0.0) + (0.125 if rk == 2 else 2.0 if rk == 1 else 0.0)
+                        + (0.5 if block_sum is not None else 0.0)))
   co = empty((3, Cn), F32, dy)
   part = raw_part
   if part is None:
@@ -419,6 +425,15 @@
                                 _ptr(mean), _ptr(invstd), _ptr(part), _stream()), 'bn_bwd_reduce')
   _bn_bwd_coeffs(part, M, Cn, gamma, mean, invstd, dgamma, dbeta, co, raw=raw_part is not None)
   dx = torch.empty_like(x)
+  if block_sum is not None:
+    H, W = block_sum
+    Nb = M // (H * W)
+    bsum = empty((Nb, H // 2, W // 2, Cn), BF16, dy)
+    check(L().asm_bn_bwd_apply_blocksum(_ptr(dy), _ptr(x), _ptr(yout), Nb, H, W, Cn, _ptr(co[0]), _ptr(co[1]), _ptr(co[2]),
+                                        _ptr(dx), _ptr(bsum), _stream()), 'bn_bwd_apply_blocksum')
+    if ev is not None:
+      ev.record()
+    return dx, None, bsum
   dz = torch.empty_like(x) if want_dz else None
   check(L().asm_bn_bwd_apply(_ptr(dy), _ptr(x), _ptr(yout if relu else None), rk, M, Cn,
                              _ptr(co[0]), _ptr(co[1]), _ptr(co[2]), _ptr(dx), _ptr(dz), _stream()), 'bn_bwd_apply')
@@ -605,9 +620,31 @@
   return v
 
 
-def sk_select_bn_bwd_att(y, scale, shift, dv, att, F_, mean=None, invstd=None):
+_SK_BLUR_ENTRIES = ('asm_sk_select_bn_blur_fwd', 'asm_sk_select_bn_bwd_att_stats_blur', 'asm_sk_bn_bwd_apply_blur')
+
+
+def sk_blur_ok(H, W, k, stride) -> bool:
+  return (knob('ASM_SK_BLUR', '1') != '0' and k == 3 and stride == 2 and H > 0 and W > 0 and H % 2 == 0 and W % 2 == 0
+          and W <= 512 and all(getattr(L(), e, None) is not None for e in _SK_BLUR_ENTRIES))
+
+
+def sk_select_bn_blur_fwd(y, scale, shift, att, F_, k, stride):
+  N, H, W, _ = y.shape
+  out = empty((N, H // 2, W // 2, F_), BF16, y)
+  check(L().asm_sk_select_bn_blur_fwd(_ptr(y), _ptr(scale), _ptr(shift), _ptr(att), _ptr(out), N, H, W, F_, k, stride,
+                                      _stream()), 'sk_select_bn_blur_fwd')
+  return out
+
+
+def sk_select_bn_bwd_att(y, scale, shift, dv, att, F_, mean=None, invstd=None, blur=None):
   N, H, W, _ = y.shape
   datt = empty((N, 1, 1, 2 * F_), BF16, y)
+  if blur is not None:
+    st = empty((N, 2, 2 * F_), F32, y)
+    check(L().asm_sk_select_bn_bwd_att_stats_blur(_ptr(y), _ptr(scale), _ptr(shift), _ptr(mean), _ptr(invstd), _ptr(dv),
+                                                  _ptr(att), _ptr(datt), _ptr(st), N, H, W, F_, blur[0], blur[1], _stream()),
+          'sk_select_bn_bwd_att_stats_blur')
+    return datt, st
   if mean is not None:
     st = empty((N, 2, 2 * F_), F32, y)
     check(L().asm_sk_select_bn_bwd_att_stats(_ptr(y), _ptr(scale), _ptr(shift), _ptr(mean), _ptr(invstd), _ptr(dv), _ptr(att),
@@ -618,12 +655,13 @@
   return datt
 
 
-def sk_bn_bwd(dv, att, ds, y, scale, shift, gamma, mean, invstd, dgamma, dbeta, F_, grad_stats=None, mask_stats=None):
+def sk_bn_bwd(dv, att, ds, y, scale, shift, gamma, mean, invstd, dgamma, dbeta, F_, grad_stats=None, mask_stats=None,
+              blur=None):
   N, H, W, C2 = y.shape
   HW, M = H * W, N * H * W
   co = empty((3, C2), F32, y)
   if grad_stats is not None and mask_stats is not None:
-    ev = _bn_ev(M * (2.0 * C2 + 2.0 * F_ + 2.0 * C2))
+    ev = _bn_ev(M * (2.0 * C2 + (0.5 if blur is not None else 2.0) * F_ + 2.0 * C2))
     check(L().asm_sk_bn_bwd_finalize(_ptr(grad_stats), _ptr(mask_stats), _ptr(att), _ptr(ds), N, HW, F_, _ptr(gamma),
                                      _ptr(mean), _ptr(invstd), _ptr(dgamma), _ptr(dbeta), _ptr(co[0]), _ptr(co[1]),
                                      _ptr(co[2]), _stream()), 'sk_bn_bwd_finalize')
@@ -637,6 +675,15 @@
                                    _ptr(invstd), N, HW, F_, _ptr(part), _stream()), 'sk_bn_bwd_reduce')
     _bn_bwd_coeffs(part, M, C2, gamma, mean, invstd, dgamma, dbeta, co)
   dy = torch.empty_like(y)
+  if blur is not None:
+    if grad_stats is None or mask_stats is None:
+      raise ValueError('sk_bn_bwd: the pooled-gradient form needs the per-image statistics')
+    check(L().asm_sk_bn_bwd_apply_blur(_ptr(dv), _ptr(att), _ptr(ds), _ptr(y), _ptr(scale), _ptr(shift), _ptr(co[0]),
+                                       _ptr(co[1]), _ptr(co[2]), _ptr(dy), N, H, W, F_, blur[0], blur[1], _stream()),
+          'sk_bn_bwd_apply_blur')
+    if ev is not None:
+      ev.record()
+    return dy
   check(L().asm_sk_bn_bwd_apply(_ptr(dv), _ptr(att), _ptr(ds), _ptr(y), _ptr(scale), _ptr(shift), _ptr(co[0]),
                                 _ptr(co[1]), _ptr(co[2]), _ptr(dy), N, HW, F_, _stream()), 'sk_bn_bwd_apply')
   if ev is not None:
diff --git a/include/asm_hip.h b/include/asm_hip.h
--- a/include/asm_hip.h
+++ b/include/asm_hip.h
@@ -125,6 +125,9 @@
 int asm_bn_bwd_apply(const void* dy, const void* x, const void* yout, int relu, int M, int C,
                      const float* coefA, const float* coefB, const float* coefC, void* dx,
                      void* dz_out, void* stream);
+int asm_bn_bwd_apply_blocksum(const void* dy, const void* x, const uint8_t* relu_mask, int N, int H, int W, int C,
+                              const float* coefA, const float* coefB, const float* coefC, void* dx, void* block_sum,
+                              void* stream);
 
 int asm_bn_apply2(const void* xa, const void* xb, void* y, int M, int C, const float* scale_a, const float* shift_a,
                   const float* scale_b, const float* shift_b, int relu, uint8_t* relu_mask_out, void* stream);
@@ -184,6 +187,14 @@
 int asm_sk_bn_bwd_finalize(const float* grad_stats, const float* mask_stats, const float* att, const void* ds, int N,
                            int HW, int F, const float* gamma, const float* mean, const float* invstd, float* dgamma,
                            float* dbeta, float* coefA, float* coefB, float* coefC, void* stream);
+int asm_sk_select_bn_blur_fwd(const void* y, const float* scale, const float* shift, const float* att, void* out, int N,
+                              int H, int W, int F, int k, int stride, void* stream);
+int asm_sk_select_bn_bwd_att_stats_blur(const void* y, const float* scale, const float* shift, const float* mean,
+                                        const float* invstd, const void* dpool, const float* att, void* datt,
+                                        float* grad_stats, int N, int H, int W, int F, int k, int stride, void* stream);
+int asm_sk_bn_bwd_apply_blur(const void* dpool, const float* att, const void* ds, const void* y, const float* scale,
+                             const float* shift, const float* coefA, const float* coefB, const float* coefC, void* dy,
+                             int N, int H, int W, int F, int k, int stride, void* stream);
 int asm_se_scale_fwd(const void* x, const float* e, void* y, int N, int HW, int C, void* stream);
 int asm_se_scale_bwd_e(const void* x, const void* dy, const float* e, void* de, int N, int HW, int C, void* stream);
 int asm_se_scale_bwd_x(const void* dy, const float* e, const void* dsq, void* dx, int N, int HW, int C, void* stream);
```

Result: faster. 10810 images/sec, median of 6 (+1.5%).
